# bibendovsky/oalsfxpp

Hardware: AMD Instinct MI355X
Metric: Msamples/sec EAX reverb, 256-frame buffers, batch=4096; % HBM roofline (higher is better)
Workload: dtype f32

## Files before the change

### include/oalsfx_hip.h

```cpp
#ifndef OALSFX_HIP_H
#define OALSFX_HIP_H

#include "oalsfx_desc.h"

#ifdef __cplusplus
extern "C" {
#endif

typedef struct oalsfx_batch oalsfx_batch;

typedef struct {
    int32_t type;
    unsigned char props[108];
} oalsfx_effect;

typedef struct { float gain, gain_hf, gain_lf; } oalsfx_send_props;

oalsfx_batch* oalsfx_batch_create(int n_instances, int channel_format, int sampling_rate, int effect_count, int device_id);
void oalsfx_batch_destroy(oalsfx_batch* b);
const char* oalsfx_batch_error(const oalsfx_batch* b);
const char* oalsfx_last_error(void);

int oalsfx_batch_instances(const oalsfx_batch* b);
int oalsfx_batch_channels(const oalsfx_batch* b);
int oalsfx_batch_sampling_rate(const oalsfx_batch* b);
int oalsfx_batch_effect_count(const oalsfx_batch* b);

int oalsfx_batch_set_effect(oalsfx_batch* b, int first, int count, int slot, const oalsfx_effect* effects, int stride_bytes);
int oalsfx_batch_set_effect_at(oalsfx_batch* b, const int* instances, int count, int slot, const oalsfx_effect* effects, int stride_bytes);
int oalsfx_batch_set_effect_type(oalsfx_batch* b, int first, int count, int slot, int effect_type);
int oalsfx_batch_set_effect_props(oalsfx_batch* b, int first, int count, int slot, const void* props, int stride_bytes);
int oalsfx_batch_set_send_props(oalsfx_batch* b, int first, int count, int slot, const oalsfx_send_props* props);
int oalsfx_batch_get_effect(const oalsfx_batch* b, int instance, int slot, int deferred, oalsfx_effect* out);
int oalsfx_batch_get_send_props(const oalsfx_batch* b, int instance, int slot, int deferred, oalsfx_send_props* out);
int oalsfx_batch_apply_changes(oalsfx_batch* b, int first, int count);

int oalsfx_batch_mix(oalsfx_batch* b, int frames, const float* src_host, float* dst_host);
int oalsfx_batch_mix_gather(oalsfx_batch* b, int frames, const float* const* src_per_instance, float* const* dst_per_instance);
int oalsfx_batch_mix_device(oalsfx_batch* b, int frames, const float* src_dev, float* dst_dev, void* hip_stream);
int oalsfx_batch_mix_device_multi(oalsfx_batch* b, int frames, int buffers, const float* const* src_dev, float* const* dst_dev, void* hip_stream);
int oalsfx_batch_synchronize(oalsfx_batch* b);
long long oalsfx_batch_chained_calls(const oalsfx_batch* b);
int oalsfx_batch_mix_async(oalsfx_batch* b, int frames, const float* src_host, float* dst_host);
int oalsfx_batch_wait(oalsfx_batch* b);
void* oalsfx_pinned_alloc(unsigned long long bytes);
void oalsfx_pinned_free(void* p);
void* oalsfx_batch_stream(oalsfx_batch* b);

typedef struct oalsfx_group oalsfx_group;
oalsfx_group* oalsfx_group_create(int n_total, const int* device_ids, int n_devices, int channel_format, int sampling_rate, int effect_count);
void oalsfx_group_destroy(oalsfx_group* g);
const char* oalsfx_group_error(const oalsfx_group* g);
const char* oalsfx_group_last_error(void);
int oalsfx_group_instances(const oalsfx_group* g);
int oalsfx_group_channels(const oalsfx_group* g);
int oalsfx_group_devices(const oalsfx_group* g);
int oalsfx_group_shard(const oalsfx_group* g, int k, int* device_id, int* first, int* count);
oalsfx_batch* oalsfx_group_batch(oalsfx_group* g, int k);
int oalsfx_group_set_effect(oalsfx_group* g, int first, int count, int slot, const oalsfx_effect* effects, int stride_bytes);
int oalsfx_group_set_effect_type(oalsfx_group* g, int first, int count, int slot, int effect_type);
int oalsfx_group_set_effect_props(oalsfx_group* g, int first, int count, int slot, const void* props, int stride_bytes);
int oalsfx_group_set_send_props(oalsfx_group* g, int first, int count, int slot, const oalsfx_send_props* props);
int oalsfx_group_apply_changes(oalsfx_group* g, int first, int count);
int oalsfx_group_mix(oalsfx_group* g, int frames, const float* src_host, float* dst_host);
int oalsfx_group_mix_device(oalsfx_group* g, int frames, const float* const* src_per_device, float* const* dst_per_device);
int oalsfx_group_mix_device_multi(oalsfx_group* g, int frames, int buffers, const float* const* src_dev, float* const* dst_dev);
int oalsfx_group_synchronize(oalsfx_group* g);
int oalsfx_group_set_routing(oalsfx_group* g, int first, int count, const int* bus, const float* gain);
int oalsfx_group_mix_downmix(oalsfx_group* g, int frames, const float* src_host, int n_buses, float* dst_bus_host);

unsigned long long oalsfx_trim_pools(void);
unsigned long long oalsfx_pools_waiting_bytes(void);

int oalsfx_batch_read_slot(oalsfx_batch* b, int instance, int slot, oalsfx_slot_params* params, oalsfx_slot_state* state);
int oalsfx_batch_read_ring(oalsfx_batch* b, int instance, int slot, float* out, int max_floats);
int oalsfx_batch_read_source(oalsfx_batch* b, int instance, oalsfx_source_params* params, oalsfx_source_state* state);

unsigned long long oalsfx_batch_snapshot_bytes(oalsfx_batch* b, const int* instances, int count);
int oalsfx_batch_snapshot(oalsfx_batch* b, const int* instances, int count, void* dst, unsigned long long bytes);
int oalsfx_batch_restore(oalsfx_batch* b, const int* instances, int count, const void* src, unsigned long long bytes);
int oalsfx_batch_reset(oalsfx_batch* b, const int* instances, int count);

#define OALSFX_DOWNMIX_CHUNK 32
int oalsfx_batch_set_routing(oalsfx_batch* b, int first, int count, const int* bus, const float* gain);
int oalsfx_batch_get_routing(const oalsfx_batch* b, int instance, int* bus, float* gain);
int oalsfx_batch_downmix_device(oalsfx_batch* b, int frames, const float* src_dev, int n_buses, float* dst_bus_dev, void* hip_stream);
int oalsfx_batch_mix_downmix(oalsfx_batch* b, int frames, const float* src_host, int n_buses, float* dst_bus_host);

#define OALSFX_METER_LANES 64
#define OALSFX_METER_CARRY 1
typedef struct {
    float    peak[OALSFX_MAX_CHANNELS];
    float    sumsq[OALSFX_MAX_CHANNELS];
    float    peak_hold;
    uint32_t quiet_run;
    uint32_t nonfinite;
    uint32_t frames;
} oalsfx_meter;
int oalsfx_batch_meter_device(oalsfx_batch* b, int rows, int frames, const float* src_dev, float threshold, int flags,
                              oalsfx_meter* meters_dev, void* hip_stream);
int oalsfx_batch_mix_downmix_meter(oalsfx_batch* b, int frames, const float* src_host, int n_buses, float* dst_bus_host,
                                   float threshold, int flags, oalsfx_meter* voice_meters_host, oalsfx_meter* bus_meters_host);
int oalsfx_group_mix_downmix_meter(oalsfx_group* g, int frames, const float* src_host, int n_buses, float* dst_bus_host,
                                   float threshold, int flags, oalsfx_meter* voice_meters_host);

#define OALSFX_SAMPLER_FRAC_BITS 12
#define OALSFX_PCM_U8  0
#define OALSFX_PCM_S16 1
#define OALSFX_PCM_F32 2
#define OALSFX_SAMPLER_PLAYING 1
#define OALSFX_SAMPLER_LOOP    2
#define OALSFX_SAMPLER_LINEAR  4
typedef struct {
    uint64_t data;
    uint64_t position;
    uint32_t frames;
    uint32_t loop_start;
    uint32_t loop_end;
    uint32_t step;
    uint32_t format;
    uint32_t channels;
    uint32_t flags;
// ... 32 lines not shown
```

### include/oalsfx_hip_debug.h

```cpp
#ifndef OALSFX_HIP_DEBUG_H
#define OALSFX_HIP_DEBUG_H

#include "oalsfx_hip.h"

#ifdef __cplusplus
extern "C" {
#endif

int oalsfx_batch_mix_timed(oalsfx_batch* b, int frames, const float* src_host, float* dst_host, double legs_us[3]);
long long oalsfx_debug_chain_same_cu(oalsfx_batch* b);
int oalsfx_batch_fill_synthetic(oalsfx_batch* b, int frames, unsigned buffer_index, float* dst_dev, void* hip_stream);

int oalsfx_batch_kernel_timing(oalsfx_batch* b, int enable);
int oalsfx_batch_kernel_timing_read(oalsfx_batch* b, int effect_type, int* launches, double* total_ms);
int oalsfx_batch_kernel_timing_samples(oalsfx_batch* b, int effect_type, double* out_us, int max_samples);
int oalsfx_batch_placement(const oalsfx_batch* b, int* chunks, int* candidates, double* best_us, double* worst_us);
int oalsfx_batch_event_overhead(oalsfx_batch* b, int repeats, double* avg_us);

int oalsfx_debug_hbm_sweep(int device_id, unsigned long long bytes, int write, int repeats);
void oalsfx_debug_set_flags(int flags);
unsigned long long oalsfx_debug_ring_address(oalsfx_batch* b, int instance, int slot);
int oalsfx_debug_move_rings(oalsfx_batch* b, int keep_old);
int oalsfx_debug_probe_rings(oalsfx_batch* b, int repeats, double* avg_us);
int oalsfx_debug_probe_pointer(void* slabs, int instances, int slab_floats, int repeats, double* avg_us);
int oalsfx_debug_stream_pattern(int device_id, int instances, int dwords_per_lane, int repeats, int slab_floats, int pos_skew, double* avg_us);

int oalsfx_debug_host_pipeline(oalsfx_batch* b, int* form, double* probe_us_three_streams, double* probe_us_one_stream);

void oalsfx_debug_gate_skew(oalsfx_batch* b, unsigned skew);
int oalsfx_debug_chain_given_up(const oalsfx_batch* b);
int oalsfx_debug_chain_started(oalsfx_batch* b, unsigned* host_total, unsigned* device_total);
int oalsfx_batch_multi_counts(const oalsfx_batch* b, long long* buffers_in_passes, long long* passes);

long long oalsfx_debug_downmix_uploads(const oalsfx_batch* b);
void oalsfx_debug_downmix_vector(int max_floats);

long long oalsfx_debug_sampler_uploads(const oalsfx_batch* b);

#ifdef __cplusplus
}
#endif

#endif
```

### oalsfxpp_amd/api.py

```python
import ctypes as C
import operator
import weakref

import numpy as np

from . import desc, lib

_fp = C.POINTER(C.c_float)
DOWNMIX_CHUNK = 32
METER_LANES = 64
METER_CARRY = 1
METER_DTYPE = np.dtype([("peak", np.float32, (desc.MAX_CHANNELS,)), ("sumsq", np.float32, (desc.MAX_CHANNELS,)), ("peak_hold", np.float32),
                        ("quiet_run", np.uint32), ("nonfinite", np.uint32), ("frames", np.uint32)])
assert METER_DTYPE.itemsize == C.sizeof(desc.Meter) == 80
SAMPLER_DTYPE = np.dtype([("data", np.uint64), ("position", np.uint64), ("frames", np.uint32), ("loop_start", np.uint32), ("loop_end", np.uint32),
                          ("step", np.uint32), ("format", np.uint32), ("channels", np.uint32), ("flags", np.uint32), ("reserved", np.uint32),
                          ("gain", np.float32, (desc.MAX_CHANNELS,))])
assert SAMPLER_DTYPE.itemsize == C.sizeof(desc.Sampler) == 80
SAMPLER_FRAC_BITS = desc.SAMPLER_FRAC_BITS
_PCM_BYTES = {desc.PCM_U8: 1, desc.PCM_S16: 2, desc.PCM_F32: 4}


class BatchError(RuntimeError):
    pass
# ... 48 lines not shown
    def _range(self, first, count):
        return first, (self.n - first if count is None else count)

    def set_effect(self, slot, effect, first=0, count=None):
        first, count = self._range(first, count)
        if isinstance(effect, desc.Effect):
            self._check(self._lib.oalsfx_batch_set_effect(self._h, first, count, slot, C.byref(effect), 0))
        else:
            arr = (desc.Effect * count)(*effect)
            self._check(self._lib.oalsfx_batch_set_effect(self._h, first, count, slot, arr, C.sizeof(desc.Effect)))

    def set_effect_at(self, slot, instances, effects):
        idx = (C.c_int * len(instances))(*instances)
        if isinstance(effects, desc.Effect):
            self._check(self._lib.oalsfx_batch_set_effect_at(self._h, idx, len(instances), slot, C.byref(effects), 0))
        else:
            arr = (desc.Effect * len(instances))(*effects)
            self._check(self._lib.oalsfx_batch_set_effect_at(self._h, idx, len(instances), slot, arr, C.sizeof(desc.Effect)))

    def set_effect_type(self, slot, effect_type, first=0, count=None):
        first, count = self._range(first, count)
        self._check(self._lib.oalsfx_batch_set_effect_type(self._h, first, count, slot, effect_type))

    def set_effect_props(self, slot, props, first=0, count=None):
        first, count = self._range(first, count)
        if isinstance(props, desc.EffectPropsU):
            self._check(self._lib.oalsfx_batch_set_effect_props(self._h, first, count, slot, C.byref(props), 0))
        else:
            arr = (desc.EffectPropsU * count)(*props)
            self._check(self._lib.oalsfx_batch_set_effect_props(self._h, first, count, slot, arr, C.sizeof(desc.EffectPropsU)))

    def set_send_props(self, slot, gain, gain_hf, gain_lf, first=0, count=None):
        first, count = self._range(first, count)
        p = desc.SendProps(gain, gain_hf, gain_lf)
        self._check(self._lib.oalsfx_batch_set_send_props(self._h, first, count, slot, C.byref(p)))

    def get_effect(self, instance, slot, deferred=False):
        e = desc.Effect()
        self._check(self._lib.oalsfx_batch_get_effect(self._h, instance, slot, 1 if deferred else 0, C.byref(e)))
        return e

    def get_send_props(self, instance, slot, deferred=False):
        p = desc.SendProps()
        self._check(self._lib.oalsfx_batch_get_send_props(self._h, instance, slot, 1 if deferred else 0, C.byref(p)))
        return p

    def apply_changes(self, first=0, count=None):
        first, count = self._range(first, count)
        self._check(self._lib.oalsfx_batch_apply_changes(self._h, first, count))

    def mix(self, src):
        src = np.ascontiguousarray(src, dtype=np.float32)
        assert src.ndim == 3 and src.shape[0] == self.n and src.shape[2] == self.channels, src.shape
        dst = np.empty_like(src)
        self._check(self._lib.oalsfx_batch_mix(self._h, src.shape[1], src.ctypes.data_as(_fp), dst.ctypes.data_as(_fp)))
        return dst

    def mix_async(self, src, dst):
        assert src.dtype == np.float32 and dst.dtype == np.float32 and src.flags.c_contiguous and dst.flags.c_contiguous and src.shape == dst.shape
        assert src.ndim == 3 and src.shape[0] == self.n and src.shape[2] == self.channels, src.shape
        self._check(self._lib.oalsfx_batch_mix_async(self._h, src.shape[1], src.ctypes.data_as(_fp), dst.ctypes.data_as(_fp)))

    def wait(self):
        self._check(self._lib.oalsfx_batch_wait(self._h))

    def pinned_array(self, frames):
        count = self.n * frames * self.channels
        p = self._lib.oalsfx_pinned_alloc(count * 4)
        if not p:
            raise BatchError("oalsfx_pinned_alloc failed")
        buf = (C.c_float * count).from_address(p)
        weakref.finalize(buf, self._lib.oalsfx_pinned_free, C.c_void_p(p))
        return np.frombuffer(buf, dtype=np.float32).reshape(self.n, frames, self.channels)

    def mix_device(self, frames, src_ptr, dst_ptr, stream=None):
        self._check(self._lib.oalsfx_batch_mix_device(self._h, frames, C.c_void_p(src_ptr), C.c_void_p(dst_ptr), C.c_void_p(stream or 0)))

    def mix_device_multi(self, frames, src_ptrs, dst_ptrs, stream=None):
        if len(src_ptrs) != len(dst_ptrs):
            raise BatchError("mix_device_multi: as many source as destination buffers")
        s = (C.c_void_p * max(1, len(src_ptrs)))(*src_ptrs)
        d = (C.c_void_p * max(1, len(dst_ptrs)))(*dst_ptrs)
        self._check(self._lib.oalsfx_batch_mix_device_multi(self._h, frames, len(src_ptrs), s, d, C.c_void_p(stream or 0)))

    def multi_counts(self):
        k, p = C.c_longlong(0), C.c_longlong(0)
        self._check(self._lib.oalsfx_batch_multi_counts(self._h, C.byref(k), C.byref(p)))
        return k.value, p.value

    def synchronize(self):
        self._check(self._lib.oalsfx_batch_synchronize(self._h))

    @property
    def stream(self):
        return self._lib.oalsfx_batch_stream(self._h)

    def fill_synthetic(self, frames, buffer_index, dst_ptr, stream=None):
        self._check(self._lib.oalsfx_batch_fill_synthetic(self._h, frames, buffer_index, C.c_void_p(dst_ptr), C.c_void_p(stream or 0)))

    def read_slot(self, instance, slot):
        p, s = desc.SlotParams(), desc.SlotState()
        self._check(self._lib.oalsfx_batch_read_slot(self._h, instance, slot, C.byref(p), C.byref(s)))
        return p, s

    def read_ring(self, instance, slot):
        n = self._lib.oalsfx_batch_read_ring(self._h, instance, slot, None, 0)
        out = np.zeros(n, dtype=np.float32)
        if n:
            self._lib.oalsfx_batch_read_ring(self._h, instance, slot, out.ctypes.data_as(_fp), n)
        return out

    def read_source(self, instance):
        p, s = desc.SourceParams(), desc.SourceState()
        self._check(self._lib.oalsfx_batch_read_source(self._h, instance, C.byref(p), C.byref(s)))
        return p, s

    def _instances(self, instances):
        if instances is None:
            return None, self.n
        try:
            idx = [operator.index(i) for i in instances]
        except TypeError:
            raise BatchError("Instances must be a sequence of integers.") from None
        bad = [i for i in idx if i < 0 or i >= self.n]
        if bad:
            raise BatchError(f"Instance range is out of bounds: {bad[:4]}")
        return (C.c_int * max(1, len(idx)))(*idx), len(idx)

    @staticmethod
    def _blob(ptr, nbytes):
        if not ptr:
            raise BatchError("No snapshot buffer.")
        if ptr % 16:
            raise BatchError("The snapshot buffer is not 16-byte aligned.")
        if operator.index(nbytes) < 0:
            raise BatchError("Snapshot bytes are negative.")

    def snapshot_bytes(self, instances=None):
        idx, count = self._instances(instances)
        nbytes = self._lib.oalsfx_batch_snapshot_bytes(self._h, idx, count)
        self._check(nbytes != 0)
        return nbytes

    def snapshot(self, instances, dst_ptr, nbytes):
        idx, count = self._instances(instances)
        self._blob(dst_ptr, nbytes)
        self._check(self._lib.oalsfx_batch_snapshot(self._h, idx, count, C.c_void_p(dst_ptr), nbytes))

    def restore(self, instances, src_ptr, nbytes):
        idx, count = self._instances(instances)
        if instances is not None and len(set(idx[:count])) != count:
            raise BatchError("An instance is listed twice as a restore target.")
        self._blob(src_ptr, nbytes)
        self._check(self._lib.oalsfx_batch_restore(self._h, idx, count, C.c_void_p(src_ptr), nbytes))

    def reset(self, instances=None):
        idx, count = self._instances(instances)
        self._check(self._lib.oalsfx_batch_reset(self._h, idx, count))

    @staticmethod
    def _routing(n, first, bus, gain):
        if bus is None and gain is None:
            raise BatchError("set_routing: give buses, gains or both.")
        try:
            buses = None if bus is None else [operator.index(v) for v in bus]
            gains = None if gain is None else [float(v) for v in gain]
# ... 428 lines not shown
```

### oalsfxpp_amd/csrc/hip/batch.cpp

```cpp
#include <hip/hip_runtime.h>

#include <algorithm>
#include <atomic>
#include <cstdio>
#include <chrono>
#include <cmath>
#include <cstdlib>
#include <cstring>
#include <map>
#include <mutex>
#include <new>
#include <string>
#include <type_traits>
#include <vector>

#include "../host/core.hpp"
#include "common.hpp"
#include "oalsfx_hip.h"
#include "state_io.hpp"
#include "downmix.hpp"
#include "meter.hpp"
#include "sampler.hpp"
#include "oalsfx_hip_debug.h"

// ... 75 lines not shown
    int* d_progress = nullptr;
    unsigned* d_hot = nullptr;
    unsigned* d_inst_epoch = nullptr;
    unsigned* d_exact = nullptr;
    unsigned* h_exact = nullptr;
    char fault_text[400] = {};
    long long host_prepare_ns = 0, host_stage_wait_ns = 0, host_derive_ns = 0, host_lists_ns = 0;
    unsigned* h_fault = nullptr;
    unsigned* d_fault = nullptr;
    bool chain_given_up = false;
    uint32_t gate_skew = 0;
    hipEvent_t ev_exact = nullptr;
    char* h_state_io = nullptr;
    char* d_state_io = nullptr;
    size_t state_io_capacity = 0;
    hipEvent_t ev_state_io = nullptr;
    bool state_io_pending = false;
    bool state_io_unordered = false;
    int list_offset[OALSFX_MAX_SLOTS][OALSFX_TYPE_COUNT] = {};
    int list_count[OALSFX_MAX_SLOTS][OALSFX_TYPE_COUNT] = {};
    int steady_offset[OALSFX_MAX_SLOTS] = {};
    int fast_count[OALSFX_MAX_SLOTS] = {};
    int kind_count[OALSFX_MAX_SLOTS][3] = {};
    int rest_tiles[OALSFX_MAX_SLOTS] = {};
    int fast_first[OALSFX_MAX_SLOTS] = {};
    int slow_count[OALSFX_MAX_SLOTS] = {};
    int general_offset[OALSFX_MAX_SLOTS] = {};
    int general_count[OALSFX_MAX_SLOTS] = {};
    std::map<size_t, RingPool> pools;
    std::vector<void*> chunks;
    struct RingChunk { char* base; size_t bytes; void* alloc; };
    std::vector<RingChunk> ring_chunks;
    int placed_chunks = 0, placement_candidates = 0;
    double placement_best_us = 0.0, placement_worst_us = 0.0;

    float* d_io_src = nullptr;
    float* d_io_dst = nullptr;
    size_t io_capacity = 0;
    float* h_io_src = nullptr;
    float* h_io_dst = nullptr;
    size_t h_io_capacity = 0;
    static constexpr int kPipeDepth = 3;
    struct PipeSlot { float* d_src = nullptr; float* d_dst = nullptr; hipEvent_t copied_in = nullptr, mixed = nullptr, copied_out = nullptr; bool busy = false; };
    PipeSlot pipe[kPipeDepth];
    size_t pipe_capacity = 0;
    long long pipe_turn = 0;
    hipStream_t h2d_stream = nullptr, d2h_stream = nullptr;
    int pipe_mode = 0;
    std::chrono::steady_clock::time_point pipe_probe_t0;
    double pipe_probe_us[2] = {0.0, 0.0};

    unsigned long long* d_timeline = nullptr;
    struct Stage { char* host = nullptr; char* dev = nullptr; size_t capacity = 0; hipEvent_t done = nullptr; bool pending = false; };
    Stage stage[4];
    int stage_turn = 0;
    hipEvent_t ev_uploaded = nullptr;
    hipEvent_t ev_mixed = nullptr;
    hipStream_t last_launch_stream = nullptr;
    const char* last_steady_kernel = "";

    hipStream_t stream = nullptr;
    hipStream_t chain_stream[kChainDepth] = {};
    hipEvent_t ev_chain[kChainDepth] = {};
    int chain_pos = 0;
    int chain_pos_last = -1, chain_pos_before = -1;
    bool chain_used[kChainDepth] = {};
    hipEvent_t ev_chain_start = nullptr;
    unsigned* d_turn = nullptr;
    uint32_t turn_counter = 0;
    uint32_t started_total = 0;
    int launched_groups = 0;
    uint32_t frames_total = 0;
    std::vector<uint32_t> started_at;
    bool off_grid_known = false;
    int off_grid[OALSFX_MAX_SLOTS] = {};
    bool poisoned = false;
    int chain_len = 0;
    std::vector<std::pair<const char*, const char*>> chain_dsts;
    bool uncached = false;
    bool chain_open = false;
    bool stream_handed_out = false;
    long long chained_calls = 0;
    long long multi_buffers = 0, multi_passes = 0;
    std::vector<int> route_bus;
    std::vector<float> route_gain;
    bool routing_dirty = true;
    int route_max = -1;
    int dm_buses = 0;
    oalsfx_hip::DownmixTable dm_table;
    oalsfx_hip::DownmixDevice dm_dev;
    char* h_dm_table = nullptr;
    char* d_dm_table = nullptr;
    size_t dm_table_capacity = 0;
    float* d_dm_partials = nullptr;
    size_t dm_partials_capacity = 0;
    float* d_dm_out = nullptr;
    size_t dm_out_capacity = 0;
    hipEvent_t ev_downmix = nullptr;
    hipEvent_t ev_dm_order = nullptr;
    hipStream_t dm_stream = nullptr;
    bool dm_pending = false;
    long long dm_uploads = 0;
    oalsfx_meter* d_meters = nullptr;
    size_t meters_capacity = 0;
    std::vector<oalsfx_sampler> h_samplers;
    std::vector<uint8_t> sampler_dirty;
    std::vector<int> sampler_dirty_list;
    bool samplers_ahead = false;
    oalsfx_sampler* d_samplers = nullptr;
    char* h_sampler_stage = nullptr;
    size_t sampler_stage_capacity = 0;
    hipEvent_t ev_sampler_staged = nullptr;
    bool sampler_stage_pending = false;
    hipEvent_t ev_sampler = nullptr;
    hipStream_t sampler_stream = nullptr;
    bool sampler_pending = false;
    long long sampler_uploads = 0;
    hipStream_t side_stream[kSideStreams] = {};
    hipEvent_t ev_fork = nullptr;
    hipEvent_t ev_join[kSideStreams] = {};
    const char* error = "";
    std::string error_store;

    bool timing = false;
    int timing_every = 0;
    long long mix_calls = 0;
    std::vector<TimedLaunch> timed;
    std::vector<hipEvent_t> event_pool;

    hipEvent_t take_event()
    {
        hipEvent_t e = nullptr;
        if (!event_pool.empty()) { e = event_pool.back(); event_pool.pop_back(); }
        else hipEventCreate(&e);
        return e;
    }
    bool fail(const char* msg) { error = msg; return false; }
    bool hip_ok(hipError_t e, const char* what)
    {
        if (e == hipSuccess) return true;
        error_store = std::string(what) + ": " + hipGetErrorString(e);
        error = error_store.c_str();
        return false;
    }
};

namespace {

constexpr const char* kErrRange = "Instance range is out of bounds.";
constexpr const char* kErrSlot = "Effect index is out of range.";
constexpr const char* kErrNoSrc = "No source samples.";
constexpr const char* kErrNoDst = "No destination samples.";

bool range_ok(oalsfx_batch* b, int first, int count)
{
    if (first < 0 || count < 0 || first + count > b->n) return b->fail(kErrRange);
    return true;
}

void mark_touched(oalsfx_batch* b, int first, int count)
{
    for (int i = first; i < first + count; ++i)
        if (!b->touched[i]) {
            b->touched[i] = 1;
            b->touched_list.push_back(i);
        }
}

void mark_dirty(oalsfx_batch* b, int i)
{
    if (!b->inst_dirty[i]) {
        b->inst_dirty[i] = 1;
        b->dirty_list.push_back(i);
    }
}

void release_slab(oalsfx_batch* b, size_t idx)
{
    if (b->h_rings[idx]) {
        b->pools[b->ring_floats[idx]].free_dirty.push_back(b->h_rings[idx]);
        b->h_rings[idx] = nullptr;
        b->ring_floats[idx] = 0;
    }
}

enum DebugFlag : int {
    kDbgAcquireAlways = 0x1,
    kDbgAcquireNever = 0x2,
    kDbgReadEarly = 0x4,
    kDbgGeneralOnly = 0x8,
    kDbgTapRound128 = 0x20,
    kDbgTapRound256 = 0x40,
    kDbgChainLight = 0x80,
    kDbgNoCuMajor = 0x100,
    kDbgNoChain = 0x400,
    kDbgGateSecondOnly = 0x800,
    kDbgChainAlways = 0x8000,
    kDbgForceProven = 0x2000000,
    kDbgHandOverBits = kDbgAcquireAlways | kDbgAcquireNever | kDbgReadEarly,
    kDbgKernelBits = 0xFF,
};
int debug_flags();

constexpr int kSettleFrames = OALSFX_RV_FADE_SAMPLES;

enum : uint8_t {
    kClassReverb = 1,
    kClassSteady = 2,
    kClassClose = 4,
    kClassShort = 8,
    kClassModulated = 16,
};

uint8_t classify_slot(const oalsfx_slot_params& sp)
{
    if (sp.type != OALSFX_REVERB && sp.type != OALSFX_EAX_REVERB) return 0;
    const oalsfx_reverb_params& p = sp.u.reverb;
    uint8_t cls = kClassReverb | kClassSteady;
    const int sway = p.mod_depth != 0.0F ? 1 + static_cast<int>(std::abs(p.mod_depth)) : 0;
    int lo = 1 << 30, lo_ahead = 1 << 30;
    for (int j = 0; j < 4; ++j) {
        if (p.early_tap[j] < 0 || p.early_ap_off[j] < 4 || p.early_line_off[j] < 0 || p.late_ap_off[j] < 4 ||
            p.late_line_off[j] < 64 + sway || p.late_tap[j] < p.late_feed_tap)
            cls &= static_cast<uint8_t>(~kClassSteady);
        lo = std::min({lo, p.early_tap[j], p.early_ap_off[j], p.early_line_off[j], p.late_tap[j] - p.late_feed_tap, p.late_ap_off[j], p.late_line_off[j]});
        lo_ahead = std::min({lo_ahead, p.early_tap[j], p.late_line_off[j]});
    }
    if (lo >= 64 && (lo < static_cast<int>(oalsfx_hip::kPlainMinTap) || lo_ahead < static_cast<int>(oalsfx_hip::kPlainMinTapAhead))) cls |= kClassClose;
    if (lo < 64) cls |= kClassShort;
    if (p.mod_depth != 0.0F) cls |= kClassModulated;
    return cls;
}

bool reverb_settled(const oalsfx_batch* b, size_t idx)
{
    return (b->slot_class[idx] & kClassSteady) != 0 && (b->since_update[idx] >= kSettleFrames || b->xf_ok[idx]);
}

bool crossfade_followable(const oalsfx_reverb_params& from, const oalsfx_reverb_params& to)
{
    const int sway = (from.mod_depth != 0.0F || to.mod_depth != 0.0F) ? 1 + static_cast<int>(std::max(std::abs(from.mod_depth), std::abs(to.mod_depth))) : 0;
    for (const oalsfx_reverb_params* p : {&from, &to})
        for (int j = 0; j < 4; ++j)
            if (p->early_tap[j] < 0 || p->early_ap_off[j] < 4 || p->early_line_off[j] < 0 || p->late_tap[j] < to.late_feed_tap ||
                p->late_ap_off[j] < 4 || p->late_line_off[j] < 64 + sway)
                return false;
    return true;
}

bool slot_in_transition(const oalsfx_batch* b, int slot)
{
    for (size_t idx : b->settling)
        if (static_cast<int>(idx % b->slots) == slot && b->xf_ok[idx]) return true;
    return false;
}

void reclassify_slot(oalsfx_batch* b, size_t idx, int slot)
{
    const uint8_t before = b->slot_class[idx], after = classify_slot(b->h_params[idx]);
    b->n_close[slot] += ((after & kClassClose) != 0) - ((before & kClassClose) != 0);
    b->n_short[slot] += ((after & kClassShort) != 0) - ((before & kClassShort) != 0);
    if (after & kClassModulated) b->modulated[slot] = true;
    b->slot_class[idx] = after;
}

void advance_settling(oalsfx_batch* b, int frames)
{
    size_t keep = 0;
    for (size_t k = 0; k < b->settling.size(); ++k) {
        const size_t idx = b->settling[k];
        b->since_update[idx] = std::min(b->since_update[idx] + frames, kSettleFrames);
        if (b->since_update[idx] < kSettleFrames) { b->settling[keep++] = idx; continue; }
        b->in_settling[idx] = 0;
        b->xf_ok[idx] = 0;
        if (b->slot_class[idx] & kClassSteady) { b->lists_dirty = true; b->exact_wanted = true; }
    }
    b->settling.resize(keep);
}

class UncachedPool {
public:
    static constexpr size_t kGranule = size_t(2) << 20;
// ... 868 lines not shown
            const char* lo = reinterpret_cast<const char*>(dsts[k]);
            bool known = false;
            for (const auto& d : b->chain_dsts) known |= d.first <= lo && lo < d.second;
            if (!known) return false;
        }
        const char* lo = reinterpret_cast<const char*>(srcs[k]);
        const char* hi = lo + buffer_bytes;
        if (b->chain_open)
            for (const auto& d : b->chain_dsts)
                if (lo < d.second && d.first < hi) return false;
    }
    if (stream != b->stream || b->stream_handed_out || (debug_flags() & (kDbgNoChain | kDbgGeneralOnly)) || b->timing_every > 0 || b->d_timeline) return false;
    if (!b->uncached) return false;
    for (const auto& kv : b->pools)
        if (kv.first % 32 != 0) return false;
    if (frames > OALSFX_MAX_CHUNK) return false;
    if (b->channels > 2) {
        const int last_block = frames - ((frames - 1) / OALSFX_RV_MAX_UPDATE) * OALSFX_RV_MAX_UPDATE;
        return b->slots == 1 && !uploading && (frames & 63) == 0 && b->n_filtered == 0 && b->general_count[0] == 0 && b->slow_count[0] == 0 &&
               b->fast_count[0] == b->n && last_block / 64 >= b->rest_tiles[0];
    }
    if (b->slots > 1) {
        const int last = b->slots - 1, run = reverb_free_run(b, 0);
        if (uploading || (frames & 63) != 0 || b->n_filtered > 0 || run < last) return false;
        if ((b->n + 3) / 4 < 1024 && !(debug_flags() & kDbgChainAlways)) return false;
        if (run == b->slots) return (debug_flags() & kDbgChainLight) != 0;
        if (b->fast_count[last] + b->slow_count[last] != b->n || b->general_count[last] != 0) return false;
        KernelCtx ctx{};
        ctx.frames = frames;
        const SlotPlan pl = plan_slot(b, ctx, last, frames, true);
        return pl.by_kind && !pl.mixed && pl.steady == b->n;
    }
    if ((b->n + 3) / 4 < 1024 && frames < 256 && !(debug_flags() & kDbgChainAlways)) return false;
    const int steady = b->fast_count[0] + b->slow_count[0];
    if (b->general_count[0] != 0) return false;
    if (steady != b->n) {
        if (uploading || (frames & 63) != 0 || b->n_filtered > 0) return false;
        KernelCtx ctx{};
        ctx.frames = frames;
        const SlotPlan pl = plan_slot(b, ctx, 0, frames, true);
        if (pl.light + pl.steady != b->n || pl.reverbs != pl.steady) return false;
        if (pl.steady == 0) return (debug_flags() & kDbgChainLight) != 0;
        if ((b->n + 3) / 4 <= 1024 && !(debug_flags() & kDbgChainAlways)) return false;
        return pl.mixed && mixed_grid_proven(b, 0, frames);
    }
    if ((frames & 63) != 0) {
        KernelCtx ctx{};
        ctx.frames = frames;
        if (!plan_slot(b, ctx, 0, frames, true).ragged_proven || b->n_filtered > 0) return false;
    }
    if (b->n_filtered > 0) {
        KernelCtx ctx{};
        ctx.frames = frames;
        const SlotPlan p0 = plan_slot(b, ctx, 0, frames, true);
        if (!p0.by_kind || p0.steady != b->n) return false;
        int counts[4];
        steady_kind_counts(b, 0, p0.proven_usable, counts);
        if (filters_inside_count(b, 0, counts) != b->n_filtered) return false;
    }
    return true;
}

bool chain_next_launch(oalsfx_batch* b, KernelCtx& ctx, int depth, PendingUpload* upload, hipStream_t* stream_out)
{
    b->chain_pos_before = b->chain_open ? b->chain_pos_last : -1;
    b->chain_pos_last = b->chain_open ? b->chain_pos : -1;
    b->chain_pos = b->chain_open ? (b->chain_pos + 1) % depth : 0;
    hipStream_t stream = b->chain_stream[b->chain_pos];
    const bool first_on_its_stream = b->chain_open && !b->chain_used[b->chain_pos];
    b->chain_used[b->chain_pos] = true;
    const size_t total = static_cast<size_t>(b->n) * b->slots;
    ctx.turn = b->d_turn;
    ctx.turn_cu = b->d_turn + total + 16;
    ctx.turn_cu2 = ctx.turn_cu + total;
    ctx.turn_slot = b->slots - 1;
    ctx.turn_two_back = (b->chain_pos_before >= 0 && b->chain_pos_before != b->chain_pos) ? 1u : 0u;
    ctx.turn_wait = b->chain_open ? b->turn_counter : 0u;
    if (++b->turn_counter == 0u) b->turn_counter = 1u;
    ctx.turn_set = b->turn_counter;
    unsigned* started = b->d_turn + total;
    if (!b->chain_open) {
        if (!b->hip_ok(hipEventRecord(b->ev_chain_start, b->stream), "hipEventRecord")) return false;
        b->chain_len = 1;
    } else {
        ++b->chain_len;
        if (first_on_its_stream && !b->hip_ok(hipStreamWaitEvent(stream, b->ev_chain_start, 0), "hipStreamWaitEvent")) return false;
        if (b->chain_len == 2 || !(debug_flags() & kDbgGateSecondOnly)) {
            const unsigned target = b->started_total - static_cast<uint32_t>(std::min(8, (b->n + 3) / 4 - 1));
            if (upload && upload->st) { upload->jobs.gate_started = started; upload->jobs.gate_target = target + b->gate_skew; }
            else oalsfx_hip::launch_chain_gate(started, target + b->gate_skew, b->d_fault + 1, stream);
        }
    }
    ctx.turn_started = started;
    b->chain_open = true;
    b->launched_groups = 0;
    *stream_out = stream;
    return true;
}

bool chain_launch_done(oalsfx_batch* b)
{
    if (b->launched_groups <= 0) return b->fail("Internal error: a chained call launched no grid that takes turns.");
    b->started_total += static_cast<uint32_t>(b->launched_groups);
    b->launched_groups = 0;
    return true;
}

bool pass_usable(oalsfx_batch* b, int frames, int total)
{
    if (total > OALSFX_MAX_CHUNK || frames > total) return false;
    if (b->slots != 1 || b->channels > 2 || (frames & 63) != 0 || b->n_filtered > 0 || b->d_timeline) return false;
    if (b->fast_count[0] != b->n || b->slow_count[0] != 0 || b->general_count[0] != 0) return false;
    for (const int n : {frames, total}) {
        KernelCtx ctx{};
        ctx.frames = n;
        const SlotPlan p = plan_slot(b, ctx, 0, n, true);
        if (!p.by_kind || p.mixed || p.steady != b->n || !p.proven_usable) return false;
    }
    return true;
}

bool buffers_apart(const oalsfx_batch* b, int frames, int buffers, const float* const* srcs, float* const* dsts)
{
    if (buffers < 2) return true;
    const uintptr_t bytes = static_cast<uintptr_t>(b->n) * frames * b->channels * sizeof(float);
    struct Range { uintptr_t lo; int call; bool out; };
    std::vector<Range> r;
    r.reserve(2 * static_cast<size_t>(buffers));
    for (int k = 0; k < buffers; ++k) {
        r.push_back({reinterpret_cast<uintptr_t>(srcs[k]), k, false});
        r.push_back({reinterpret_cast<uintptr_t>(dsts[k]), k, true});
    }
    std::sort(r.begin(), r.end(), [](const Range& x, const Range& y) { return x.lo < y.lo || (x.lo == y.lo && x.call < y.call); });
    const Range* last[2][2] = {};
    for (const Range& x : r) {
        for (int kind = 0; kind < 2; ++kind) {
            if (!x.out && kind == 0) continue;
            for (const Range* y : last[kind])
                if (y && y->call != x.call && y->lo + bytes > x.lo) return false;
        }
        const int kind = x.out ? 1 : 0;
        last[kind][1] = last[kind][0];
        last[kind][0] = &x;
    }
    return true;
}

bool mix_pass(oalsfx_batch* b, int frames, int buffers, const float* const* srcs, float* const* dsts, hipStream_t stream, bool may_chain,
              PendingUpload& upload, bool pass)
{
    const float* const src = srcs[0];
    float* const dst = dsts[0];
    const int total = frames * buffers;
    if (pass && total > OALSFX_MAX_CHUNK) return b->fail("Internal error: a multi-buffer pass longer than one chunk.");
    const bool chained = may_chain && (!upload.st || upload.chainable) && chain_eligible(b, total, buffers, srcs, dsts, stream, upload.st != nullptr);
    if (!chained && !chain_join(b)) return false;
    int depth = 2;
    if (chained) {
        const int rs = b->slots - 1;
        int populated = 0;
        for (int k = 0; k < 3; ++k) populated += b->kind_count[rs][k] > 0;
        depth = (populated > 1 || b->slow_count[rs] > 0 || upload.st) ? kChainDepth : 2;
    }
    if (!chained && !launch_params(b, upload, b->stream, stream)) return false;
    if (!ensure_mixbuf(b)) return false;
    b->timing = b->timing_every > 0 && (b->mix_calls % b->timing_every == 0 || b->mix_calls % b->timing_every + buffers > b->timing_every);
    b->mix_calls += buffers;
    const bool filtered = b->n_filtered > 0;
    const int chunk_max = std::min(total, OALSFX_MAX_CHUNK);
    const size_t plane = static_cast<size_t>(b->n) * chunk_max * b->channels;
    if (filtered && plane > b->filtered_capacity) {
        if (!b->hip_ok(hipStreamSynchronize(stream), "hipStreamSynchronize")) return false;
        for (int k = 1; k < kChainDepth && b->chain_open; ++k)
            if (!b->hip_ok(hipStreamSynchronize(b->chain_stream[k]), "hipStreamSynchronize")) return false;
        hipFree(b->d_filtered);
        b->d_filtered = nullptr;
        b->filtered_capacity = 0;
        if (!b->hip_ok(hipMalloc(reinterpret_cast<void**>(&b->d_filtered), plane * (1 + b->slots) * sizeof(float)), "hipMalloc(filtered sends)")) return false;
        b->filtered_capacity = plane;
    }
    KernelCtx ctx{};
    ctx.params = b->d_params;
    ctx.state = b->d_state;
    ctx.rings = b->d_rings;
    ctx.source = b->d_source;
    ctx.source_state = b->d_source_state;
    ctx.mixbuf = b->d_mixbuf;
    ctx.timeline = b->d_timeline;
    ctx.hot = b->d_hot;
    ctx.inst_epoch = b->d_inst_epoch;
    ctx.exact = b->d_exact;
    ctx.fault = b->d_fault;
    ctx.list_first = -1;
    ctx.no_follow_up = 0;
    if (chained) {
        if (!b->chain_open) b->chain_dsts.clear();
        for (int k = 0; k < buffers; ++k) {
            const char* lo = reinterpret_cast<const char*>(dsts[k]);
            const char* hi = lo + static_cast<size_t>(b->n) * frames * b->channels * sizeof(float);
            bool known = false;
            for (auto& d : b->chain_dsts) known |= d.first <= lo && hi <= d.second;
            if (!known) b->chain_dsts.push_back({lo, hi});
        }
        if (!chain_next_launch(b, ctx, depth, &upload, &stream)) return false;
        if (!launch_params(b, upload, stream, nullptr, b->d_turn, ctx.turn_wait)) return false;
        b->chained_calls += 1;
    }
    ctx.slots = b->slots;
    ctx.channels = b->channels;
    ctx.io_stride = static_cast<long long>(frames) * b->channels;
    struct EqualPlaces {
        bool on;
        explicit EqualPlaces(bool o) : on(o) { if (on) oalsfx_hip::set_lds_per_workgroup(40960); }
        ~EqualPlaces() { if (on) oalsfx_hip::set_lds_per_workgroup(0); }
    } equal_places(chained && b->slots > 1);
    oalsfx_hip::BufferTable table{};
    if (pass) {
        for (int k = 0; k < buffers; ++k) { table.src[k] = srcs[k]; table.dst[k] = dsts[k]; }
        table.frames = frames;
        table.buffers = buffers;
    }
    for (int done = 0; done < total;) {
        const int n = std::min(total - done, OALSFX_MAX_CHUNK);
        const float* chunk_src = src + static_cast<size_t>(done) * b->channels;
        ctx.raw_src = chunk_src;
        ctx.dst = dst + static_cast<size_t>(done) * b->channels;
        ctx.frames = n;
        bool planes = filtered;
        bool filters_inside = false;
        if (filtered && b->slots == 1) {
            const SlotPlan p0 = plan_slot(b, ctx, 0, n, true);
            if (p0.by_kind && p0.steady > 0) {
                int counts[4];
                steady_kind_counts(b, 0, p0.proven_usable, counts);
                const int inside = filters_inside_count(b, 0, counts);
                if (inside > 0) {
                    filters_inside = true;
                    ctx.src_stride = static_cast<long long>(n) * b->channels;
                    planes = inside < b->n_filtered;
                    if (planes) {
                        const int before = b->steady_offset[0], behind = before + counts[0] + counts[1];
                        oalsfx_hip::launch_send_filters(ctx, chunk_src, ctx.io_stride, b->d_filtered, b->filtered_capacity, b->d_lists, before, stream);
                        oalsfx_hip::launch_send_filters(ctx, chunk_src, ctx.io_stride, b->d_filtered, b->filtered_capacity, b->d_lists + behind, b->n - behind, stream);
                    }
                }
            }
        }
        if (filters_inside) {
            ctx.src = planes ? b->d_filtered : chunk_src;
            if (!planes) ctx.src_stride = ctx.io_stride;
        } else if (filtered) {
            ctx.src_stride = static_cast<long long>(n) * b->channels;
            oalsfx_hip::launch_send_filters(ctx, chunk_src, ctx.io_stride, b->d_filtered, b->filtered_capacity, nullptr, b->n, stream);
            ctx.src = b->d_filtered;
        } else {
            ctx.src_stride = ctx.io_stride;
            ctx.src = chunk_src;
        }
        ctx.wet_plane = planes ? static_cast<long long>(b->filtered_capacity) : 0;
        for (int s = 0; s < b->slots; ++s) {
            ctx.wet_src = planes ? b->d_filtered + static_cast<size_t>(1 + s) * b->filtered_capacity : ctx.src;
            const int run = reverb_free_run(b, s);
            if (run >= 2) {
                const int run_flags = (s == 0 ? oalsfx_hip::kFirst : 0) | (s + run == b->slots ? oalsfx_hip::kLast : 0) |
                                      (planes ? oalsfx_hip::kFiltered : 0);
                {
                    ScopedTiming timing(b, kTimedWaveEffects, stream);
                    const bool grid_order = chained && s + run < b->slots;
                    const int* every = grid_order ? b->d_lists + b->steady_offset[b->slots - 1] : b->d_lists + b->list_offset[s][OALSFX_NULL];
                    oalsfx_hip::launch_wave_effects(ctx, s, run, every, b->n, nullptr,
                                                    run_flags | (chained ? ((debug_flags() & kDbgHandOverBits) | (grid_order ? 0 : 8)) << 8 : 0), stream);
                }
                if (chained) b->launched_groups = (b->n + 3) / 4;
                s += run - 1;
                continue;
            }
            if (chained && s > 0 && (!chain_launch_done(b) || !chain_next_launch(b, ctx, depth, nullptr, &stream))) return false;
            const int flags = (s == 0 ? oalsfx_hip::kFirst : 0) | (s == b->slots - 1 ? oalsfx_hip::kLast : 0) |
                              (planes ? oalsfx_hip::kFiltered : 0);
            const bool null_has_duty = (flags & (oalsfx_hip::kFirst | oalsfx_hip::kLast)) != 0;
            const SlotPlan sp = plan_slot(b, ctx, s, n, null_has_duty);
            const int light = sp.light, steady = sp.steady, reverbs = sp.reverbs;
            const bool use_steady = sp.use_steady, mixed = sp.mixed, by_kind = sp.by_kind, proven_usable = sp.proven_usable;
            bool part_on[4] = {light > 0 && !mixed, false, steady > 0, reverbs - steady > 0};
            int parts = 0;
            for (bool on : part_on) parts += on;
            const bool fork = parts > 1;
            if (fork && !b->hip_ok(hipEventRecord(b->ev_fork, stream), "hipEventRecord")) return false;
            int main_part = -1;
            for (int g = 0; g < 4; ++g)
                if (part_on[g]) main_part = (main_part < 0 || g == 3) ? g : main_part;
            int side = 0;
            for (int g = 0; g < 4; ++g) {
                if (!part_on[g]) continue;
                hipStream_t gs = stream;
                if (fork && g != main_part) {
                    gs = b->side_stream[side];
                    if (!b->hip_ok(hipStreamWaitEvent(gs, b->ev_fork, 0), "hipStreamWaitEvent")) return false;
                }
                if (g == 0) {
                    launch_wave_group(b, ctx, s, flags, gs);
                } else if (g == 2 && mixed) {
                    launch_mixed_part(b, ctx, s, flags, gs);
                } else if (g == 2 && pass) {
                    launch_reverb_pass_part(b, ctx, s, flags, table, gs);
                } else if (g == 2 && by_kind) {
                    launch_reverb_kinds_part(b, ctx, s, flags, proven_usable, filters_inside, gs);
                } else if (g == 2) {
                    launch_reverb_steady_part(b, ctx, s, flags, b->steady_offset[s], steady, sp.ragged_proven, gs);
                } else {
                    launch_reverb_general_part(b, !use_steady, ctx, s, flags, gs);
                }
                if (gs != stream) {
                    if (!b->hip_ok(hipEventRecord(b->ev_join[side], gs), "hipEventRecord")) return false;
                    ++side;
                }
            }
            for (int k = 0; k < side; ++k)
                if (!b->hip_ok(hipStreamWaitEvent(stream, b->ev_join[k], 0), "hipStreamWaitEvent")) return false;
        }
        done += n;
    }
    if (chained && !chain_launch_done(b)) return false;
    if (pass) { b->multi_buffers += buffers; b->multi_passes += 1; }
    if ((total % OALSFX_MAX_CHUNK) & 63) {
        for (size_t idx : b->settling)
            if (b->xf_ok[idx]) { b->xf_ok[idx] = 0; b->lists_dirty = true; }
    }
    advance_settling(b, total);
    b->frames_total += static_cast<uint32_t>(total);
    if (total & 31) b->off_grid_known = false;
    if (b->exact_wanted && !b->exact_pending) {
        const size_t total = static_cast<size_t>(b->n) * b->slots;
        if (!b->hip_ok(hipMemcpyAsync(b->h_exact, b->d_exact, total * sizeof(unsigned), hipMemcpyDeviceToHost, stream), "hipMemcpyAsync(exact)")) return false;
        if (!b->hip_ok(hipEventRecord(b->ev_exact, stream), "hipEventRecord")) return false;
        b->exact_pending = true;
        b->exact_wanted = false;
        b->exact_gen = b->upload_gen;
    }
    b->last_launch_stream = chained ? b->stream : stream;
    if (!chained && stream != b->stream && !b->hip_ok(hipEventRecord(b->ev_mixed, stream), "hipEventRecord")) return false;
    return b->hip_ok(hipGetLastError(), "kernel launch");
}

bool mix_device(oalsfx_batch* b, int frames, int buffers, const float* const* srcs, float* const* dsts, hipStream_t stream, bool may_chain,
                bool multi)
{
    if (b->state_io_unordered && stream != b->stream) {
        if (!b->hip_ok(hipStreamWaitEvent(stream, b->ev_state_io, 0), "hipStreamWaitEvent")) return false;
        b->state_io_unordered = false;
    }
    const int per_pass = std::max(1, OALSFX_MAX_CHUNK / std::max(frames, 1));
    const bool apart = multi && buffers_apart(b, frames, buffers, srcs, dsts);
    for (int k = 0; k < buffers;) {
        if (b->poisoned) return b->fail(b->fault_text);
        poll_exact(b);
        b->launched_groups = 0;
        PendingUpload upload;
        const auto hp0 = std::chrono::steady_clock::now();
        if (!prepare_params(b, upload)) return false;
        b->host_prepare_ns += std::chrono::duration_cast<std::chrono::nanoseconds>(std::chrono::steady_clock::now() - hp0).count();
        const int take = std::min(buffers - k, per_pass);
        const bool pass = apart && !(debug_flags() & kDbgGeneralOnly) && pass_usable(b, frames, take * frames);
        const int step = pass ? take : 1;
        if (!mix_pass(b, frames, step, srcs + k, dsts + k, stream, may_chain, upload, pass)) return false;
        k += step;
    }
    return true;
}

bool mix_device(oalsfx_batch* b, int frames, const float* src, float* dst, hipStream_t stream, bool may_chain = false)
{
    float* out = dst;
    return mix_device(b, frames, 1, &src, &out, stream, may_chain, false);
}

}

extern "C" {

const char* oalsfx_last_error(void) { return g_last_error.c_str(); }

oalsfx_batch* oalsfx_batch_create(int n_instances, int channel_format, int sampling_rate, int effect_count, int device_id)
{
    g_last_error.clear();
    const int channels = channel_count_of(static_cast<oalsfxpp::ChannelFormat>(channel_format));
    if (channels == 0) { g_last_error = "Invalid channel format."; return nullptr; }
    if (sampling_rate < min_sampling_rate) { g_last_error = "Sampling rate is out of range."; return nullptr; }
    if (effect_count <= 0 || effect_count > OALSFX_MAX_SLOTS) { g_last_error = "Effect count is out of range."; return nullptr; }
    if (n_instances <= 0) { g_last_error = "Instance count is out of range."; return nullptr; }

    int device_count = 0;
    if (hipGetDeviceCount(&device_count) != hipSuccess || device_count <= 0) {
        g_last_error = "No HIP device available: the effect process path has no CPU fallback.";
        return nullptr;
    }
    if (device_id < 0 || device_id >= device_count) { g_last_error = "HIP device ordinal is out of range."; return nullptr; }
    if (hipSetDevice(device_id) != hipSuccess) { g_last_error = "hipSetDevice failed."; return nullptr; }

    auto* b = new (std::nothrow) oalsfx_batch{};
    if (!b) { g_last_error = "Failed to allocate the batch."; return nullptr; }
    b->n = n_instances;
    b->slots = effect_count;
    b->channels = channels;
    b->rate = sampling_rate;
    b->format = channel_format;
    b->device = device_id;
    b->dev.init(static_cast<oalsfxpp::ChannelFormat>(channel_format), sampling_rate);
    b->channels = b->dev.channels;
    const size_t total = static_cast<size_t>(n_instances) * effect_count;
    b->inst.resize(n_instances);
    b->h_params.assign(total, oalsfx_slot_params{});
    b->h_state_init.assign(total, oalsfx_slot_state{});
    b->started_at.assign(total, 0);
    b->h_source.assign(n_instances, oalsfx_source_params{});
    b->seq.assign(total, 0);
    b->h_rings.assign(total, nullptr);
    b->ring_floats.assign(total, 0);
    b->inst_dirty.assign(n_instances, 0);
    b->inst_filtered.assign(n_instances, 0);
    b->touched.assign(n_instances, 0);
    b->aux_written.assign(n_instances, 0);
    b->route_bus.assign(n_instances, 0);
    b->route_gain.assign(n_instances, 1.0F);
    b->h_samplers.assign(n_instances, oalsfx_sampler{});
    b->sampler_dirty.assign(n_instances, 0);
    b->since_update.assign(total, 0);
    b->slot_class.assign(total, 0);
    b->in_settling.assign(total, 0);
    b->xf_ok.assign(total, 0);
    b->mod_ever.assign(total, 0);
    b->proven.assign(total, 0);
    b->updated_gen.assign(total, 0);
    b->inst_epoch.assign(n_instances, 1);
    for (int i = 0; i < n_instances; ++i) {
        b->inst[i].initialize(effect_count);
        mark_dirty(b, i);
    }
    mark_touched(b, 0, n_instances);

    bool ok = b->hip_ok(hipStreamCreateWithFlags(&b->stream, hipStreamNonBlocking), "hipStreamCreate");
    b->chain_stream[0] = b->stream;
    for (int k = 1; k < kChainDepth; ++k) {
        ok = ok && b->hip_ok(hipStreamCreateWithFlags(&b->chain_stream[k], hipStreamNonBlocking), "hipStreamCreate");
        ok = ok && b->hip_ok(hipEventCreateWithFlags(&b->ev_chain[k], hipEventDisableTiming), "hipEventCreate");
    }
    {
        const char* kind = std::getenv("OALSFX_RING_MEMORY");
        b->uncached = (!kind || std::strcmp(kind, "uncached") == 0) && uncached_memory_available(b->device);
    }
    ok = ok && b->hip_ok(hipEventCreateWithFlags(&b->ev_chain_start, hipEventDisableTiming), "hipEventCreate");
    for (int k = 0; k < kSideStreams; ++k) {
        ok = ok && b->hip_ok(hipStreamCreateWithFlags(&b->side_stream[k], hipStreamNonBlocking), "hipStreamCreate");
        ok = ok && b->hip_ok(hipEventCreateWithFlags(&b->ev_join[k], hipEventDisableTiming), "hipEventCreate");
    }
    ok = ok && b->hip_ok(hipEventCreateWithFlags(&b->ev_fork, hipEventDisableTiming), "hipEventCreate");
    ok = ok && b->hip_ok(hipEventCreateWithFlags(&b->ev_uploaded, hipEventDisableTiming), "hipEventCreate");
    ok = ok && b->hip_ok(hipEventCreateWithFlags(&b->ev_mixed, hipEventDisableTiming), "hipEventCreate");
    ok = ok && b->hip_ok(hipEventCreateWithFlags(&b->ev_downmix, hipEventDisableTiming), "hipEventCreate");
    ok = ok && b->hip_ok(hipEventCreateWithFlags(&b->ev_dm_order, hipEventDisableTiming), "hipEventCreate");
    ok = ok && b->hip_ok(hipEventCreateWithFlags(&b->ev_sampler, hipEventDisableTiming), "hipEventCreate");
    ok = ok && b->hip_ok(hipEventCreateWithFlags(&b->ev_sampler_staged, hipEventDisableTiming), "hipEventCreate");
    ok = ok && b->hip_ok(hipMalloc(reinterpret_cast<void**>(&b->d_samplers), n_instances * sizeof(oalsfx_sampler)), "hipMalloc(samplers)");
    ok = ok && b->hip_ok(hipMemsetAsync(b->d_samplers, 0, n_instances * sizeof(oalsfx_sampler), b->stream), "hipMemsetAsync(samplers)");
    ok = ok && b->hip_ok(hipMalloc(reinterpret_cast<void**>(&b->d_params), total * sizeof(oalsfx_slot_params)), "hipMalloc(params)");
    ok = ok && b->hip_ok(handed_on_malloc(b, reinterpret_cast<void**>(&b->d_state), total * sizeof(oalsfx_hip::SlotStateLines)), "hipMalloc(state)");
    ok = ok && b->hip_ok(hipMalloc(reinterpret_cast<void**>(&b->d_source), n_instances * sizeof(oalsfx_source_params)), "hipMalloc(source)");
    ok = ok && b->hip_ok(hipMalloc(reinterpret_cast<void**>(&b->d_rings), total * sizeof(float*)), "hipMalloc(ring table)");
    ok = ok && b->hip_ok(handed_on_malloc(b, reinterpret_cast<void**>(&b->d_source_state), n_instances * sizeof(oalsfx_source_state)), "hipMalloc(source state)");
    ok = ok && b->hip_ok(hipMalloc(reinterpret_cast<void**>(&b->d_lists_buf[0]), (kChainDepth + 1) * total * sizeof(int)), "hipMalloc(lists)");
    if (ok) {
        for (int k = 1; k <= kChainDepth; ++k) b->d_lists_buf[k] = b->d_lists_buf[0] + k * total;
        b->d_lists = b->d_lists_buf[0];
    }
    ok = ok && b->hip_ok(hipMalloc(reinterpret_cast<void**>(&b->d_progress), total * sizeof(int)), "hipMalloc(progress)");
    ok = ok && b->hip_ok(hipMemsetAsync(b->d_progress, 0, total * sizeof(int), b->stream), "hipMemsetAsync(progress)");
    ok = ok && b->hip_ok(handed_on_malloc(b, reinterpret_cast<void**>(&b->d_hot), total * oalsfx_hip::hot::SIZE * sizeof(unsigned)), "hipMalloc(hot records)");
    ok = ok && b->hip_ok(hipMemsetAsync(b->d_hot, 0, total * oalsfx_hip::hot::SIZE * sizeof(unsigned), b->stream), "hipMemsetAsync(hot records)");
    ok = ok && b->hip_ok(hipMalloc(reinterpret_cast<void**>(&b->d_inst_epoch), n_instances * sizeof(unsigned)), "hipMalloc(epochs)");
    ok = ok && b->hip_ok(hipMemsetAsync(b->d_inst_epoch, 0, n_instances * sizeof(unsigned), b->stream), "hipMemsetAsync(epochs)");
    ok = ok && b->hip_ok(handed_on_malloc(b, reinterpret_cast<void**>(&b->d_turn), (3 * total + 16) * sizeof(unsigned)), "hipMalloc(turns)");
    ok = ok && b->hip_ok(hipMemsetAsync(b->d_turn, 0, (3 * total + 16) * sizeof(unsigned), b->stream), "hipMemsetAsync(turns)");
    ok = ok && b->hip_ok(handed_on_malloc(b, reinterpret_cast<void**>(&b->d_exact), total * sizeof(unsigned)), "hipMalloc(exact)");
    ok = ok && b->hip_ok(hipMemsetAsync(b->d_exact, 0, total * sizeof(unsigned), b->stream), "hipMemsetAsync(exact)");
    ok = ok && b->hip_ok(hipHostMalloc(reinterpret_cast<void**>(&b->h_exact), total * sizeof(unsigned)), "hipHostMalloc(exact)");
    ok = ok && b->hip_ok(hipHostMalloc(reinterpret_cast<void**>(&b->h_fault), 2 * sizeof(unsigned), hipHostMallocMapped), "hipHostMalloc(fault)");
    if (ok) b->h_fault[0] = b->h_fault[1] = 0;
    ok = ok && b->hip_ok(hipHostGetDevicePointer(reinterpret_cast<void**>(&b->d_fault), b->h_fault, 0), "hipHostGetDevicePointer");
    ok = ok && b->hip_ok(hipEventCreateWithFlags(&b->ev_exact, hipEventDisableTiming), "hipEventCreate");
    ok = ok && b->hip_ok(hipEventCreateWithFlags(&b->ev_state_io, hipEventDisableTiming), "hipEventCreate");
    ok = ok && b->hip_ok(hipMemsetAsync(b->d_state, 0, total * sizeof(oalsfx_hip::SlotStateLines), b->stream), "hipMemsetAsync(state)");
    ok = ok && b->hip_ok(hipMemsetAsync(b->d_source_state, 0, n_instances * sizeof(oalsfx_source_state), b->stream), "hipMemsetAsync(source state)");
    if (ok && std::getenv("OALSFX_DEBUG_TIMELINE")) {
        ok = b->hip_ok(hipMalloc(reinterpret_cast<void**>(&b->d_timeline), kTimelineBytes), "hipMalloc(timeline)");
        ok = ok && b->hip_ok(hipMemsetAsync(b->d_timeline, 0, kTimelineBytes, b->stream), "hipMemsetAsync(timeline)");
    }
    if (!ok) {
        g_last_error = b->error;
        oalsfx_batch_destroy(b);
        return nullptr;
    }
    return b;
}

void oalsfx_batch_destroy(oalsfx_batch* b)
{
    if (!b) return;
    hipSetDevice(b->device);
    for (int k = 1; k < kChainDepth; ++k)
        if (b->chain_stream[k]) hipStreamSynchronize(b->chain_stream[k]);
    if (b->stream) hipStreamSynchronize(b->stream);
    for (int k = 0; k < kSideStreams; ++k)
        if (b->side_stream[k]) hipStreamSynchronize(b->side_stream[k]);
    if (b->exact_pending) hipEventSynchronize(b->ev_exact);
    if (b->d_timeline) {
        std::vector<unsigned long long> h(kTimelineBytes / sizeof(unsigned long long));
        if (hipMemcpy(h.data(), b->d_timeline, kTimelineBytes, hipMemcpyDeviceToHost) == hipSuccess)
            if (FILE* f = std::fopen(std::getenv("OALSFX_DEBUG_TIMELINE"), "wb")) { std::fwrite(h.data(), 1, kTimelineBytes, f); std::fclose(f); }
        hipFree(b->d_timeline);
    }
    for (auto& t : b->timed) { hipEventDestroy(t.start); hipEventDestroy(t.stop); }
    for (hipEvent_t e : b->event_pool) hipEventDestroy(e);
    if (std::getenv("OALSFX_HOST_PROFILE"))
        std::fprintf(stderr, "host profile: prepare_params %.1f ms (of which waiting for a staging buffer %.1f ms), %lld mix_device calls chained\n",
                     b->host_prepare_ns * 1e-6, b->host_stage_wait_ns * 1e-6, b->chained_calls);
    for (void* c : b->chunks) handed_on_free(c);
    hipFree(b->d_params); handed_on_free(b->d_state); hipFree(b->d_source); hipFree(b->d_rings); handed_on_free(b->d_source_state); hipFree(b->d_filtered);
    handed_on_free(b->d_mixbuf); hipFree(b->d_lists_buf[0]); hipFree(b->d_progress); hipFree(b->d_io_src); hipFree(b->d_io_dst);
    handed_on_free(b->d_hot); hipFree(b->d_inst_epoch); handed_on_free(b->d_exact); handed_on_free(b->d_turn);
    for (int k = 1; k < kChainDepth; ++k)
        if (b->ev_chain[k]) hipEventDestroy(b->ev_chain[k]);
    if (b->ev_chain_start) hipEventDestroy(b->ev_chain_start);
    for (int k = 1; k < kChainDepth; ++k)
        if (b->chain_stream[k]) hipStreamDestroy(b->chain_stream[k]);
    if (b->h2d_stream) hipStreamSynchronize(b->h2d_stream);
    if (b->d2h_stream) hipStreamSynchronize(b->d2h_stream);
    for (auto& ps : b->pipe) {
        hipFree(ps.d_src); hipFree(ps.d_dst);
        if (ps.copied_in) hipEventDestroy(ps.copied_in);
        if (ps.mixed) hipEventDestroy(ps.mixed);
        if (ps.copied_out) hipEventDestroy(ps.copied_out);
    }
    if (b->h2d_stream) hipStreamDestroy(b->h2d_stream);
    if (b->d2h_stream) hipStreamDestroy(b->d2h_stream);
    if (b->h_io_src) (void)hipHostFree(b->h_io_src);
    if (b->h_io_dst) (void)hipHostFree(b->h_io_dst);
    if (b->h_exact) (void)hipHostFree(b->h_exact);
    if (b->h_fault) (void)hipHostFree(b->h_fault);
    if (b->ev_exact) hipEventDestroy(b->ev_exact);
    if (b->h_state_io) (void)hipHostFree(b->h_state_io);
    hipFree(b->d_state_io);
    if (b->ev_state_io) hipEventDestroy(b->ev_state_io);
    if (b->dm_pending) hipEventSynchronize(b->ev_downmix);
    if (b->h_dm_table) (void)hipHostFree(b->h_dm_table);
    hipFree(b->d_dm_table); hipFree(b->d_dm_partials); hipFree(b->d_dm_out);
    hipFree(b->d_meters);
    if (b->sampler_pending) hipEventSynchronize(b->ev_sampler);
    if (b->h_sampler_stage) (void)hipHostFree(b->h_sampler_stage);
    hipFree(b->d_samplers);
    if (b->ev_sampler) hipEventDestroy(b->ev_sampler);
    if (b->ev_sampler_staged) hipEventDestroy(b->ev_sampler_staged);
    if (b->ev_downmix) hipEventDestroy(b->ev_downmix);
    if (b->ev_dm_order) hipEventDestroy(b->ev_dm_order);
    for (int k = 0; k < kSideStreams; ++k) {
        if (b->side_stream[k]) hipStreamDestroy(b->side_stream[k]);
        if (b->ev_join[k]) hipEventDestroy(b->ev_join[k]);
    }
    if (b->ev_fork) hipEventDestroy(b->ev_fork);
    if (b->ev_uploaded) hipEventDestroy(b->ev_uploaded);
    if (b->ev_mixed) hipEventDestroy(b->ev_mixed);
    for (auto& st : b->stage) {
        if (st.host) (void)hipHostFree(st.host);
        if (st.dev) (void)hipFree(st.dev);
        if (st.done) hipEventDestroy(st.done);
    }
    if (b->stream) hipStreamDestroy(b->stream);
    delete b;
}

const char* oalsfx_batch_error(const oalsfx_batch* b) { return b ? b->error : g_last_error.c_str(); }
int oalsfx_batch_instances(const oalsfx_batch* b) { return b->n; }
int oalsfx_batch_channels(const oalsfx_batch* b) { return b->channels; }
int oalsfx_batch_sampling_rate(const oalsfx_batch* b) { return b->rate; }
int oalsfx_batch_effect_count(const oalsfx_batch* b) { return b->slots; }

int oalsfx_batch_set_effect(oalsfx_batch* b, int first, int count, int slot, const oalsfx_effect* effects, int stride_bytes)
{
    if (!range_ok(b, first, count)) return 0;
    if (slot < 0 || slot >= b->slots) return b->fail(kErrSlot) ? 1 : 0;
    const auto* base = reinterpret_cast<const unsigned char*>(effects);
    for (int i = 0; i < count; ++i)
        std::memcpy(&b->inst[first + i].deferred[slot], base + static_cast<size_t>(i) * stride_bytes, sizeof(oalsfx_effect));
    mark_touched(b, first, count);
    return 1;
}

int oalsfx_batch_set_effect_at(oalsfx_batch* b, const int* instances, int count, int slot, const oalsfx_effect* effects, int stride_bytes)
{
    if (count < 0 || (count > 0 && (!instances || !effects))) return b->fail(kErrRange) ? 1 : 0;
    if (slot < 0 || slot >= b->slots) return b->fail(kErrSlot) ? 1 : 0;
    for (int k = 0; k < count; ++k)
        if (instances[k] < 0 || instances[k] >= b->n) return b->fail(kErrRange) ? 1 : 0;
    const auto* base = reinterpret_cast<const unsigned char*>(effects);
    for (int k = 0; k < count; ++k) {
        std::memcpy(&b->inst[instances[k]].deferred[slot], base + static_cast<size_t>(k) * stride_bytes, sizeof(oalsfx_effect));
        mark_touched(b, instances[k], 1);
    }
    return 1;
}

int oalsfx_batch_set_effect_type(oalsfx_batch* b, int first, int count, int slot, int effect_type)
{
    if (!range_ok(b, first, count)) return 0;
    if (slot < 0 || slot >= b->slots) return b->fail(kErrSlot) ? 1 : 0;
    for (int i = 0; i < count; ++i) b->inst[first + i].deferred[slot].set_type_and_defaults(static_cast<oalsfxpp::EffectType>(effect_type));
    mark_touched(b, first, count);
    return 1;
}

int oalsfx_batch_set_effect_props(oalsfx_batch* b, int first, int count, int slot, const void* props, int stride_bytes)
{
    if (!range_ok(b, first, count)) return 0;
    if (slot < 0 || slot >= b->slots) return b->fail(kErrSlot) ? 1 : 0;
    const auto* base = static_cast<const unsigned char*>(props);
    for (int i = 0; i < count; ++i)
        std::memcpy(&b->inst[first + i].deferred[slot].props_, base + static_cast<size_t>(i) * stride_bytes, sizeof(oalsfxpp::EffectProps));
    mark_touched(b, first, count);
    return 1;
}

int oalsfx_batch_set_send_props(oalsfx_batch* b, int first, int count, int slot, const oalsfx_send_props* props)
{
    if (!range_ok(b, first, count)) return 0;
    if (slot >= b->slots) return b->fail(kErrSlot) ? 1 : 0;
    oalsfxpp::SendProps p;
    p.gain_ = props->gain; p.gain_hf_ = props->gain_hf; p.gain_lf_ = props->gain_lf;
    for (int i = 0; i < count; ++i) {
        InstanceHost& h = b->inst[first + i];
        if (slot < 0) h.direct_deferred = p;
        else { h.aux_props[slot] = p; b->aux_written[first + i] = 1; }
    }
    mark_touched(b, first, count);
    return 1;
}

int oalsfx_batch_get_effect(const oalsfx_batch* b, int instance, int slot, int deferred, oalsfx_effect* out)
{
    if (instance < 0 || instance >= b->n || slot < 0 || slot >= b->slots) return 0;
    const InstanceHost& h = b->inst[instance];
    std::memcpy(out, deferred ? &h.deferred[slot] : &h.active[slot], sizeof(oalsfx_effect));
    return 1;
}

int oalsfx_batch_get_send_props(const oalsfx_batch* b, int instance, int slot, int deferred, oalsfx_send_props* out)
{
    if (instance < 0 || instance >= b->n || slot >= b->slots) return 0;
    const InstanceHost& h = b->inst[instance];
    const oalsfxpp::SendProps& p = slot < 0 ? (deferred ? h.direct_deferred : h.direct_props) : (deferred ? h.aux_deferred[slot] : h.aux_props[slot]);
    out->gain = p.gain_; out->gain_hf = p.gain_hf_; out->gain_lf = p.gain_lf_;
    return 1;
}

int oalsfx_batch_apply_changes(oalsfx_batch* b, int first, int count)
{
    if (!range_ok(b, first, count)) return 0;
    size_t kept = 0;
    for (size_t k = 0; k < b->touched_list.size(); ++k) {
        const int i = b->touched_list[k];
        if (i < first || i >= first + count) { b->touched_list[kept++] = i; continue; }
        InstanceHost& h = b->inst[i];
        h.apply_changes();
        bool dirty = h.source_changed;
        for (int s = 0; s < b->slots; ++s) dirty |= h.slot_changed[s];
        if (dirty) mark_dirty(b, i);
        bool sticky = false;
        for (int s = 0; s < b->slots; ++s) sticky |= !oalsfxpp::SendProps::are_equal(h.aux_props[s], h.aux_deferred[s]);
        if (sticky) b->touched_list[kept++] = i;
        else b->touched[i] = 0;
    }
    b->touched_list.resize(kept);
    return 1;
}

int oalsfx_batch_mix_device(oalsfx_batch* b, int frames, const float* src_dev, float* dst_dev, void* hip_stream)
{
    if (frames == 0) return 1;
    if (frames < 0) return b->fail("Frame count is negative.") ? 1 : 0;
    if (!src_dev) return b->fail(kErrNoSrc) ? 1 : 0;
    if (!dst_dev) return b->fail(kErrNoDst) ? 1 : 0;
    if (!b->hip_ok(hipSetDevice(b->device), "hipSetDevice")) return 0;
    return mix_device(b, frames, src_dev, dst_dev, hip_stream ? static_cast<hipStream_t>(hip_stream) : b->stream, hip_stream == nullptr) ? 1 : 0;
}

int oalsfx_batch_mix_device_multi(oalsfx_batch* b, int frames, int buffers, const float* const* src_dev, float* const* dst_dev, void* hip_stream)
{
    if (!b) { g_last_error = "Null batch."; return 0; }
    if (frames < 0) return b->fail("Frame count is negative.") ? 1 : 0;
    if (buffers < 0) return b->fail("Buffer count is negative.") ? 1 : 0;
    if (frames == 0 || buffers == 0) return 1;
    if (!src_dev) return b->fail("Null source buffer table.") ? 1 : 0;
    if (!dst_dev) return b->fail("Null destination buffer table.") ? 1 : 0;
    for (int k = 0; k < buffers; ++k) {
        if (!src_dev[k]) return b->fail(kErrNoSrc) ? 1 : 0;
        if (!dst_dev[k]) return b->fail(kErrNoDst) ? 1 : 0;
    }
    if (!b->hip_ok(hipSetDevice(b->device), "hipSetDevice")) return 0;
    return mix_device(b, frames, buffers, src_dev, dst_dev, hip_stream ? static_cast<hipStream_t>(hip_stream) : b->stream, hip_stream == nullptr, true) ? 1 : 0;
}

namespace {

bool grow_io(oalsfx_batch* b, size_t floats)
{
    if (floats <= b->io_capacity) return true;
    hipFree(b->d_io_src); hipFree(b->d_io_dst);
    b->d_io_src = b->d_io_dst = nullptr;
    b->io_capacity = 0;
    if (!b->hip_ok(hipMalloc(reinterpret_cast<void**>(&b->d_io_src), floats * sizeof(float)), "hipMalloc(io)")) return false;
    if (!b->hip_ok(hipMalloc(reinterpret_cast<void**>(&b->d_io_dst), floats * sizeof(float)), "hipMalloc(io)")) return false;
    b->io_capacity = floats;
    return true;
}

int mix_host(oalsfx_batch* b, int frames, const float* src_host, float* dst_host, double* legs_us)
{
    if (legs_us) legs_us[0] = legs_us[1] = legs_us[2] = 0.0;
    if (frames == 0) return 1;
    if (frames < 0) return b->fail("Frame count is negative.") ? 1 : 0;
    if (!src_host) return b->fail(kErrNoSrc) ? 1 : 0;
    if (!dst_host) return b->fail(kErrNoDst) ? 1 : 0;
    if (!b->hip_ok(hipSetDevice(b->device), "hipSetDevice") || !chain_join(b)) return 0;
    const size_t floats = static_cast<size_t>(b->n) * frames * b->channels;
    if (!grow_io(b, floats)) return 0;
    hipEvent_t ev[4] = {};
    if (legs_us)
        for (auto& e : ev) e = b->take_event();
    if (legs_us) hipEventRecord(ev[0], b->stream);
    if (!b->hip_ok(hipMemcpyAsync(b->d_io_src, src_host, floats * sizeof(float), hipMemcpyHostToDevice, b->stream), "hipMemcpyAsync(src)")) return 0;
    if (legs_us) hipEventRecord(ev[1], b->stream);
    if (!mix_device(b, frames, b->d_io_src, b->d_io_dst, b->stream)) return 0;
    if (legs_us) hipEventRecord(ev[2], b->stream);
    if (!b->hip_ok(hipMemcpyAsync(dst_host, b->d_io_dst, floats * sizeof(float), hipMemcpyDeviceToHost, b->stream), "hipMemcpyAsync(dst)")) return 0;
    if (legs_us) hipEventRecord(ev[3], b->stream);
    if (!b->hip_ok(hipStreamSynchronize(b->stream), "hipStreamSynchronize")) return 0;
    if (legs_us) {
        for (int k = 0; k < 3; ++k) {
            float ms = 0.0F;
            if (hipEventElapsedTime(&ms, ev[k], ev[k + 1]) == hipSuccess) legs_us[k] = ms * 1e3;
        }
        for (auto& e : ev) b->event_pool.push_back(e);
    }
    poll_exact(b);
    return check_fault(b) ? 1 : 0;
}

}

int oalsfx_batch_mix(oalsfx_batch* b, int frames, const float* src_host, float* dst_host) { return mix_host(b, frames, src_host, dst_host, nullptr); }

int oalsfx_batch_mix_gather(oalsfx_batch* b, int frames, const float* const* src_per_instance, float* const* dst_per_instance)
{
    if (frames == 0) return 1;
    if (frames < 0) return b->fail("Frame count is negative.") ? 1 : 0;
    if (!src_per_instance) return b->fail(kErrNoSrc) ? 1 : 0;
    if (!dst_per_instance) return b->fail(kErrNoDst) ? 1 : 0;
    const size_t per = static_cast<size_t>(frames) * b->channels, floats = per * b->n;
    for (int i = 0; i < b->n; ++i) {
        if (!src_per_instance[i]) return b->fail(kErrNoSrc) ? 1 : 0;
        if (!dst_per_instance[i]) return b->fail(kErrNoDst) ? 1 : 0;
    }
    if (!b->hip_ok(hipSetDevice(b->device), "hipSetDevice")) return 0;
    if (floats > b->h_io_capacity) {
        if (b->h_io_src) (void)hipHostFree(b->h_io_src);
        if (b->h_io_dst) (void)hipHostFree(b->h_io_dst);
        b->h_io_src = b->h_io_dst = nullptr;
        b->h_io_capacity = 0;
        if (!b->hip_ok(hipHostMalloc(reinterpret_cast<void**>(&b->h_io_src), floats * sizeof(float), hipHostMallocDefault), "hipHostMalloc(io)")) return 0;
        if (!b->hip_ok(hipHostMalloc(reinterpret_cast<void**>(&b->h_io_dst), floats * sizeof(float), hipHostMallocDefault), "hipHostMalloc(io)")) return 0;
        b->h_io_capacity = floats;
    }
    for (int i = 0; i < b->n; ++i) std::memcpy(b->h_io_src + per * i, src_per_instance[i], per * sizeof(float));
    if (!mix_host(b, frames, b->h_io_src, b->h_io_dst, nullptr)) return 0;
    for (int i = 0; i < b->n; ++i) std::memcpy(dst_per_instance[i], b->h_io_dst + per * i, per * sizeof(float));
    return 1;
}

int oalsfx_batch_mix_timed(oalsfx_batch* b, int frames, const float* src_host, float* dst_host, double legs_us[3])
{
    return mix_host(b, frames, src_host, dst_host, legs_us);
}

namespace {

std::mutex g_pipe_mutex;
std::map<int, int> g_pipe_mode;

int pipe_form(oalsfx_batch* b)
{
    if (b->pipe_mode) return b->pipe_mode;
    if (const char* e = std::getenv("OALSFX_HOST_PIPELINE")) {
        const int m = std::atoi(e);
        if (m == 1 || m == 3) return b->pipe_mode = m;
    }
    {
        std::lock_guard<std::mutex> lock(g_pipe_mutex);
        auto it = g_pipe_mode.find(b->device);
        if (it != g_pipe_mode.end()) return b->pipe_mode = it->second;
    }
    const long long k = b->pipe_turn;
    const auto now = std::chrono::steady_clock::now();
    if ((k & 15) == 4) b->pipe_probe_t0 = now;
    if (k == 32 || k == 48) b->pipe_probe_us[k == 48 ? 0 : 1] = std::chrono::duration<double, std::micro>(now - b->pipe_probe_t0).count() / 12.0;
    if (k < 48) return (k >= 16 && k < 32) ? 1 : 3;
    b->pipe_mode = b->pipe_probe_us[1] < b->pipe_probe_us[0] * 0.9 ? 1 : 3;
    std::lock_guard<std::mutex> lock(g_pipe_mutex);
    g_pipe_mode[b->device] = b->pipe_mode;
    return b->pipe_mode;
}

}

int oalsfx_batch_mix_async(oalsfx_batch* b, int frames, const float* src_host, float* dst_host)
{
    if (frames == 0) return 1;
    if (frames < 0) return b->fail("Frame count is negative.") ? 1 : 0;
    if (!src_host) return b->fail(kErrNoSrc) ? 1 : 0;
    if (!dst_host) return b->fail(kErrNoDst) ? 1 : 0;
    if (!b->hip_ok(hipSetDevice(b->device), "hipSetDevice") || !chain_join(b)) return 0;
    const size_t floats = static_cast<size_t>(b->n) * frames * b->channels;
    if (!b->h2d_stream) {
        if (!b->hip_ok(hipStreamCreateWithFlags(&b->h2d_stream, hipStreamNonBlocking), "hipStreamCreate")) return 0;
        if (!b->hip_ok(hipStreamCreateWithFlags(&b->d2h_stream, hipStreamNonBlocking), "hipStreamCreate")) return 0;
        for (auto& ps : b->pipe) {
            if (!b->hip_ok(hipEventCreateWithFlags(&ps.copied_in, hipEventDisableTiming), "hipEventCreate")) return 0;
            if (!b->hip_ok(hipEventCreateWithFlags(&ps.mixed, hipEventDisableTiming), "hipEventCreate")) return 0;
            if (!b->hip_ok(hipEventCreateWithFlags(&ps.copied_out, hipEventDisableTiming), "hipEventCreate")) return 0;
        }
    }
    if (floats > b->pipe_capacity) {
        if (!b->hip_ok(hipStreamSynchronize(b->d2h_stream), "hipStreamSynchronize") || !b->hip_ok(hipStreamSynchronize(b->stream), "hipStreamSynchronize")) return 0;
        for (auto& ps : b->pipe) {
            hipFree(ps.d_src); hipFree(ps.d_dst);
            ps.d_src = ps.d_dst = nullptr;
            ps.busy = false;
        }
        b->pipe_capacity = 0;
        for (auto& ps : b->pipe) {
            if (!b->hip_ok(hipMalloc(reinterpret_cast<void**>(&ps.d_src), floats * sizeof(float)), "hipMalloc(io)")) return 0;
            if (!b->hip_ok(hipMalloc(reinterpret_cast<void**>(&ps.d_dst), floats * sizeof(float)), "hipMalloc(io)")) return 0;
        }
        b->pipe_capacity = floats;
    }
    const int form = pipe_form(b);
    oalsfx_batch::PipeSlot& ps = b->pipe[b->pipe_turn++ % oalsfx_batch::kPipeDepth];
    if (ps.busy && !b->hip_ok(hipEventSynchronize(ps.copied_out), "hipEventSynchronize")) return 0;
    ps.busy = true;
    if (form == 1) {
        if (!b->hip_ok(hipMemcpyAsync(ps.d_src, src_host, floats * sizeof(float), hipMemcpyHostToDevice, b->stream), "hipMemcpyAsync(src)")) return 0;
        if (!mix_device(b, frames, ps.d_src, ps.d_dst, b->stream)) return 0;
        if (!b->hip_ok(hipMemcpyAsync(dst_host, ps.d_dst, floats * sizeof(float), hipMemcpyDeviceToHost, b->stream), "hipMemcpyAsync(dst)")) return 0;
        return b->hip_ok(hipEventRecord(ps.copied_out, b->stream), "hipEventRecord") ? 1 : 0;
    }
    if (!b->hip_ok(hipMemcpyAsync(ps.d_src, src_host, floats * sizeof(float), hipMemcpyHostToDevice, b->h2d_stream), "hipMemcpyAsync(src)")) return 0;
    if (!b->hip_ok(hipEventRecord(ps.copied_in, b->h2d_stream), "hipEventRecord")) return 0;
    if (!b->hip_ok(hipStreamWaitEvent(b->stream, ps.copied_in, 0), "hipStreamWaitEvent")) return 0;
    if (!mix_device(b, frames, ps.d_src, ps.d_dst, b->stream)) return 0;
    if (!b->hip_ok(hipEventRecord(ps.mixed, b->stream), "hipEventRecord")) return 0;
    if (!b->hip_ok(hipStreamWaitEvent(b->d2h_stream, ps.mixed, 0), "hipStreamWaitEvent")) return 0;
    if (!b->hip_ok(hipMemcpyAsync(dst_host, ps.d_dst, floats * sizeof(float), hipMemcpyDeviceToHost, b->d2h_stream), "hipMemcpyAsync(dst)")) return 0;
    return b->hip_ok(hipEventRecord(ps.copied_out, b->d2h_stream), "hipEventRecord") ? 1 : 0;
}

int oalsfx_batch_wait(oalsfx_batch* b)
{
    if (!b->hip_ok(hipSetDevice(b->device), "hipSetDevice") || !chain_join(b)) return 0;
    if (b->d2h_stream && !b->hip_ok(hipStreamSynchronize(b->d2h_stream), "hipStreamSynchronize")) return 0;
    if (!b->hip_ok(hipStreamSynchronize(b->stream), "hipStreamSynchronize")) return 0;
    for (auto& ps : b->pipe) ps.busy = false;
    poll_exact(b);
    return check_fault(b) ? 1 : 0;
}

void* oalsfx_pinned_alloc(unsigned long long bytes)
{
    void* p = nullptr;
    return hipHostMalloc(&p, bytes, hipHostMallocDefault) == hipSuccess ? p : nullptr;
}

void oalsfx_pinned_free(void* p)
{
    if (p) (void)hipHostFree(p);
}

int oalsfx_batch_synchronize(oalsfx_batch* b)
{
    if (!b->hip_ok(hipSetDevice(b->device), "hipSetDevice") || !chain_join(b)) return 0;
    if (!b->hip_ok(hipStreamSynchronize(b->stream), "hipStreamSynchronize")) return 0;
    if (std::getenv("OALSFX_HOST_PROFILE")) {
        std::fprintf(stderr, "host profile since the last synchronize: prepare_params %.1f us, of which staging-buffer waits %.1f us, derive %.1f us, lists %.1f us; %lld calls chained so far\n",
                     b->host_prepare_ns * 1e-3, b->host_stage_wait_ns * 1e-3, b->host_derive_ns * 1e-3, b->host_lists_ns * 1e-3, b->chained_calls);
        b->host_prepare_ns = b->host_stage_wait_ns = b->host_derive_ns = b->host_lists_ns = 0;
    }
    poll_exact(b);
    return check_fault(b) ? 1 : 0;
}

void* oalsfx_batch_stream(oalsfx_batch* b)
{
    b->stream_handed_out = true;
    if (hipSetDevice(b->device) == hipSuccess) (void)chain_join(b);
    return b->stream;
}

int oalsfx_batch_read_slot(oalsfx_batch* b, int instance, int slot, oalsfx_slot_params* params, oalsfx_slot_state* state)
{
    if (instance < 0 || instance >= b->n || slot < 0 || slot >= b->slots) return b->fail(kErrRange) ? 1 : 0;
    if (!b->hip_ok(hipSetDevice(b->device), "hipSetDevice") || !chain_join(b)) return 0;
    if (!sync_params(b, nullptr)) return 0;
    const size_t idx = static_cast<size_t>(instance) * b->slots + slot;
    if (params) *params = b->h_params[idx];
    if (state) {
        if (!b->hip_ok(hipStreamSynchronize(b->stream), "hipStreamSynchronize")) return 0;
        if (!b->hip_ok(hipMemcpy(state, static_cast<const oalsfx_slot_state*>(b->d_state + idx), sizeof(*state), hipMemcpyDeviceToHost), "hipMemcpy(state)")) return 0;
    }
    return 1;
}

int oalsfx_batch_read_ring(oalsfx_batch* b, int instance, int slot, float* out, int max_floats)
{
    if (instance < 0 || instance >= b->n || slot < 0 || slot >= b->slots) return 0;
    if (hipSetDevice(b->device) != hipSuccess || !chain_join(b) || !sync_params(b, nullptr)) return 0;
    const size_t idx = static_cast<size_t>(instance) * b->slots + slot;
    const int floats = static_cast<int>(b->ring_floats[idx]);
    if (out && floats) {
        hipStreamSynchronize(b->stream);
        const int n = std::min(floats, max_floats);
        if (!b->hip_ok(hipMemcpy(out, b->h_rings[idx], static_cast<size_t>(n) * sizeof(float), hipMemcpyDeviceToHost), "hipMemcpy(ring)")) return 0;
    }
    return floats;
}

int oalsfx_batch_read_source(oalsfx_batch* b, int instance, oalsfx_source_params* params, oalsfx_source_state* state)
{
    if (instance < 0 || instance >= b->n) return b->fail(kErrRange) ? 1 : 0;
    if (!b->hip_ok(hipSetDevice(b->device), "hipSetDevice") || !chain_join(b)) return 0;
    if (!sync_params(b, nullptr)) return 0;
    if (params) *params = b->h_source[instance];
    if (state) {
        if (!b->hip_ok(hipStreamSynchronize(b->stream), "hipStreamSynchronize")) return 0;
        if (!b->hip_ok(hipMemcpy(state, b->d_source_state + instance, sizeof(*state), hipMemcpyDeviceToHost), "hipMemcpy(source state)")) return 0;
    }
    return 1;
}

namespace {

constexpr uint32_t kBlobMagic = 0x58465342u;
constexpr uint32_t kBlobVersion = 1;
constexpr size_t kBlobAlign = 256;

size_t blob_round(size_t v) { return (v + kBlobAlign - 1) / kBlobAlign * kBlobAlign; }

struct BlobHeader {
    uint32_t magic, version;
    int32_t format, rate, slots, count;
    uint64_t total_bytes;
    uint64_t table_offset;
    uint64_t prefix_bytes;
    uint64_t device_stride;
    uint64_t host_stride;
};
static_assert(sizeof(BlobHeader) <= kBlobAlign, "the header fits its section");

struct BlobEntry { uint64_t host, device, ring[OALSFX_MAX_SLOTS]; };

struct BlobSlot {
    int32_t type;
    uint32_t ring_floats;
    uint32_t update_seq;
    uint32_t frames_since_start;
    uint32_t mod_ever;
    uint32_t reserved[3];
};

struct BlobHost {
    oalsfxpp::Effect active[OALSFX_MAX_SLOTS], deferred[OALSFX_MAX_SLOTS];
    oalsfxpp::SendProps direct_props, direct_deferred, aux_props[OALSFX_MAX_SLOTS], aux_deferred[OALSFX_MAX_SLOTS];
    BlobSlot slot[OALSFX_MAX_SLOTS];
    uint32_t touched;
    uint32_t aux_written;
};
static_assert(std::is_trivially_copyable<oalsfxpp::Effect>::value && std::is_trivially_copyable<oalsfxpp::SendProps>::value, "records are bytes");

constexpr size_t kStateBytes = sizeof(oalsfx_hip::SlotStateLines);
constexpr size_t kSourceStateBytes = sizeof(oalsfx_source_state);
constexpr size_t kSourceParamsBytes = sizeof(oalsfx_source_params);
static_assert(kStateBytes % 16 == 0 && kSourceStateBytes % 16 == 0 && kSourceParamsBytes % 16 == 0, "records copy in 16-byte pieces");
size_t source_state_at(int slots) { return slots * kStateBytes; }
size_t source_params_at(int slots) { return source_state_at(slots) + kSourceStateBytes; }
size_t device_stride(int slots) { return blob_round(source_params_at(slots) + kSourceParamsBytes); }

int instance_at(const int* instances, int k) { return instances ? instances[k] : k; }

bool instances_ok(oalsfx_batch* b, const int* instances, int count)
{
    if (count < 0 || (!instances && count > b->n)) return b->fail(kErrRange);
    if (instances)
        for (int k = 0; k < count; ++k)
            if (instances[k] < 0 || instances[k] >= b->n) return b->fail(kErrRange);
    return true;
}

uint64_t blob_layout(const oalsfx_batch* b, const int* instances, int count, std::vector<BlobEntry>& entries, BlobHeader& h)
{
    h = BlobHeader{};
    h.magic = kBlobMagic;
    h.version = kBlobVersion;
    h.format = b->format;
    h.rate = b->rate;
    h.slots = b->slots;
    h.count = count;
    h.table_offset = kBlobAlign;
    h.host_stride = blob_round(sizeof(BlobHost));
    h.device_stride = device_stride(b->slots);
    const uint64_t host0 = h.table_offset + blob_round(static_cast<size_t>(count) * sizeof(BlobEntry));
    h.prefix_bytes = host0 + static_cast<uint64_t>(count) * h.host_stride;
// ... 95 lines not shown
            if (b->ring_floats[idx] == recs[k].slot[s].ring_floats) continue;
            release_slab(b, idx);
            b->rings_table_dirty = true;
            if (recs[k].slot[s].ring_floats) taking.push_back(idx);
        }
    for (int k = 0, t = 0; k < count; ++k)
        for (int s = 0; s < b->slots; ++s) {
            const size_t idx = static_cast<size_t>(instances[k]) * b->slots + s;
            if (t >= static_cast<int>(taking.size()) || taking[t] != idx) continue;
            ++t;
            const size_t floats = recs[k].slot[s].ring_floats;
            RingPool& pool = b->pools[floats];
            std::vector<float*>& from = pool.free_clean.empty() ? pool.free_dirty : pool.free_clean;
            b->h_rings[idx] = from.back();
            from.pop_back();
            b->ring_floats[idx] = floats;
        }
    for (int k = 0; k < count; ++k) {
        const int i = instances[k];
        const BlobHost& r = recs[k];
        InstanceHost& h = b->inst[i];
        h.effect_count = b->slots;
        for (int s = 0; s < OALSFX_MAX_SLOTS; ++s) {
            h.active[s] = r.active[s];
            h.deferred[s] = r.deferred[s];
            h.aux_props[s] = r.aux_props[s];
            h.aux_deferred[s] = r.aux_deferred[s];
            h.slot_changed[s] = s < b->slots;
            h.slot_retyped[s] = false;
        }
        h.direct_props = r.direct_props;
        h.direct_deferred = r.direct_deferred;
        h.source_changed = true;
        for (int s = 0; s < b->slots; ++s) b->started_at[static_cast<size_t>(i) * b->slots + s] = b->frames_total - r.slot[s].frames_since_start;
        mark_dirty(b, i);
    }
    b->off_grid_known = false;
    if (!sync_params(b, nullptr)) return false;
    std::vector<oalsfx_hip::StateSegment> segs;
    std::vector<oalsfx_hip::StateSeenFix> fixes;
    for (int k = 0; k < count; ++k) {
        const int i = instances[k];
        const BlobHost& r = recs[k];
        const char* dev = blob ? blob + entries[k].device : nullptr;
        for (int s = 0; s < b->slots; ++s) {
            const size_t idx = static_cast<size_t>(i) * b->slots + s;
            b->xf_ok[idx] = 0;
            b->mod_ever[idx] = r.slot[s].mod_ever ? 1 : 0;
            if (b->mod_ever[idx]) b->modulated[s] = true;
            segs.push_back({dev ? dev + s * kStateBytes : nullptr, b->d_state + idx, kStateBytes, 0});
            fixes.push_back({&b->d_state[idx].seen_seq, dev ? reinterpret_cast<const unsigned*>(dev + s * kStateBytes) : nullptr, r.slot[s].update_seq,
                             b->h_params[idx].update_seq});
            if (b->h_rings[idx]) segs.push_back({blob ? blob + entries[k].ring[s] : nullptr, b->h_rings[idx], b->ring_floats[idx] * sizeof(float), 0});
        }
        segs.push_back({dev ? dev + source_state_at(b->slots) : nullptr, b->d_source_state + i, kSourceStateBytes, 0});
        b->aux_written[i] = r.aux_written ? 1 : 0;
        if (r.aux_written && dev) {
            const oalsfx_source_params& sp = sends[k];
            auto has_filter = [&](const oalsfx_source_params& x) {
                int any = x.direct.filter_type;
                for (int s = 0; s < b->slots; ++s)
                    if (x.aux[s].out_channels != 0) any |= x.aux[s].filter_type;
                return any != OALSFX_AF_NONE;
            };
            b->n_filtered += static_cast<int>(has_filter(sp)) - static_cast<int>(has_filter(b->h_source[i]));
            b->inst_filtered[i] = has_filter(sp) ? 1 : 0;
            b->inside_version = ~0u;
            b->h_source[i] = sp;
            segs.push_back({dev + source_params_at(b->slots), b->d_source + i, kSourceParamsBytes, 0});
            b->lists_dirty = true;
        }
        if (r.touched && !b->touched[i]) { b->touched[i] = 1; b->touched_list.push_back(i); }
        if (!r.touched) b->touched[i] = 0;
    }
    b->lists_dirty = true;
    b->touched_list.erase(std::remove_if(b->touched_list.begin(), b->touched_list.end(), [&](int i) { return !b->touched[i]; }), b->touched_list.end());
    return state_io_launch(b, segs, fixes, {}, 0, false);
}

}

unsigned long long oalsfx_batch_snapshot_bytes(oalsfx_batch* b, const int* instances, int count)
{
    if (!b) { g_last_error = "Null batch."; return 0; }
    if (!instances_ok(b, instances, count)) return 0;
    std::vector<BlobEntry> entries;
    BlobHeader h;
    return blob_layout(b, instances, count, entries, h);
}

int oalsfx_batch_snapshot(oalsfx_batch* b, const int* instances, int count, void* dst, unsigned long long bytes)
{
    if (!b) { g_last_error = "Null batch."; return 0; }
    if (!instances_ok(b, instances, count)) return 0;
    if (!dst) return b->fail("No snapshot buffer.") ? 1 : 0;
    if (reinterpret_cast<uintptr_t>(dst) % 16 != 0) return b->fail("The snapshot buffer is not 16-byte aligned.") ? 1 : 0;
    if (b->poisoned) return b->fail(b->fault_text) ? 1 : 0;
    std::vector<BlobEntry> entries;
    BlobHeader h;
    if (blob_layout(b, instances, count, entries, h) > bytes) return b->fail("The snapshot buffer is too small (oalsfx_batch_snapshot_bytes).") ? 1 : 0;
    if (!state_io_begin(b) || !sync_params(b, nullptr)) return 0;
    std::vector<char> prefix(h.prefix_bytes, 0);
    std::memcpy(prefix.data(), &h, sizeof(h));
    std::memcpy(prefix.data() + h.table_offset, entries.data(), entries.size() * sizeof(BlobEntry));
    char* const out = static_cast<char*>(dst);
    std::vector<oalsfx_hip::StateSegment> segs;
    segs.push_back({nullptr, out, h.prefix_bytes, 0});
    for (int k = 0; k < count; ++k) {
        const int i = instance_at(instances, k);
        const InstanceHost& ih = b->inst[i];
        BlobHost r{};
        for (int s = 0; s < OALSFX_MAX_SLOTS; ++s) {
            r.active[s] = ih.active[s];
            r.deferred[s] = ih.deferred[s];
            r.aux_props[s] = ih.aux_props[s];
            r.aux_deferred[s] = ih.aux_deferred[s];
        }
        r.direct_props = ih.direct_props;
        r.direct_deferred = ih.direct_deferred;
        r.touched = b->touched[i];
        r.aux_written = b->aux_written[i];
        char* const dev = out + entries[k].device;
        for (int s = 0; s < b->slots; ++s) {
            const size_t idx = static_cast<size_t>(i) * b->slots + s;
            BlobSlot& sl = r.slot[s];
            sl.type = b->h_params[idx].type;
            sl.ring_floats = static_cast<uint32_t>(b->ring_floats[idx]);
            sl.update_seq = b->h_params[idx].update_seq;
            sl.frames_since_start = b->frames_total - b->started_at[idx];
            sl.mod_ever = b->mod_ever[idx];
            if (sl.ring_floats != static_cast<uint32_t>(ring_floats_for(sl.type, b->rate)) || (sl.ring_floats && !entries[k].ring[s]))
                return b->fail("Internal error: a slot's delay lines do not match its effect type.") ? 1 : 0;
            segs.push_back({b->d_state + idx, dev + s * kStateBytes, kStateBytes, 0});
            if (sl.ring_floats) segs.push_back({b->h_rings[idx], out + entries[k].ring[s], sl.ring_floats * sizeof(float), 0});
        }
        segs.push_back({b->d_source_state + i, dev + source_state_at(b->slots), kSourceStateBytes, 0});
        segs.push_back({b->d_source + i, dev + source_params_at(b->slots), kSourceParamsBytes, 0});
        std::memcpy(prefix.data() + entries[k].host, &r, sizeof(r));
    }
    return state_io_launch(b, segs, {}, prefix, 1, true) ? 1 : 0;
}

int oalsfx_batch_restore(oalsfx_batch* b, const int* instances, int count, const void* src, unsigned long long bytes)
{
    if (!b) { g_last_error = "Null batch."; return 0; }
    if (!instances_ok(b, instances, count)) return 0;
    if (!src) return b->fail("No snapshot buffer.") ? 1 : 0;
    if (reinterpret_cast<uintptr_t>(src) % 16 != 0) return b->fail("The snapshot buffer is not 16-byte aligned.") ? 1 : 0;
    if (b->poisoned) return b->fail(b->fault_text) ? 1 : 0;
    std::vector<int> targets(count);
    std::vector<uint8_t> taken(b->n, 0);
    for (int k = 0; k < count; ++k) {
        targets[k] = instance_at(instances, k);
        if (taken[targets[k]]) return b->fail("An instance is listed twice as a restore target.") ? 1 : 0;
        taken[targets[k]] = 1;
    }
    if (bytes < sizeof(BlobHeader)) return b->fail("The snapshot is shorter than its header.") ? 1 : 0;
    if (!state_io_begin(b) || !b->hip_ok(hipStreamSynchronize(b->stream), "hipStreamSynchronize")) return 0;
    const char* const blob = static_cast<const char*>(src);
    BlobHeader h;
    if (!b->hip_ok(hipMemcpy(&h, blob, sizeof(h), hipMemcpyDefault), "hipMemcpy(snapshot header)")) return 0;
    if (h.magic != kBlobMagic) return b->fail("Not a snapshot (bad magic value).") ? 1 : 0;
    if (h.version != kBlobVersion) return b->fail("Snapshot version is not supported.") ? 1 : 0;
    if (h.format != b->format || h.rate != b->rate || h.slots != b->slots)
        return b->fail("The snapshot's channel format, sampling rate or effect count differs from the batch's.") ? 1 : 0;
    if (h.count != count) return b->fail("The snapshot holds another number of instances than the target list.") ? 1 : 0;
    if (h.total_bytes > bytes) return b->fail("The snapshot is larger than the bytes given.") ? 1 : 0;
    if (h.table_offset != kBlobAlign || h.host_stride != blob_round(sizeof(BlobHost)) || h.device_stride != device_stride(b->slots) ||
        h.prefix_bytes > h.total_bytes || h.table_offset + static_cast<uint64_t>(count) * sizeof(BlobEntry) > h.prefix_bytes)
        return b->fail("The snapshot's layout is damaged.") ? 1 : 0;
    std::vector<char> prefix(h.prefix_bytes);
    if (!b->hip_ok(hipMemcpy(prefix.data(), blob, prefix.size(), hipMemcpyDefault), "hipMemcpy(snapshot records)")) return 0;
    std::vector<BlobEntry> entries(count);
    std::memcpy(entries.data(), prefix.data() + h.table_offset, count * sizeof(BlobEntry));
    std::vector<BlobHost> recs(count);
    auto within = [&](uint64_t off, uint64_t len, uint64_t lo, uint64_t hi) { return off % 16 == 0 && off >= lo && off <= hi && len <= hi - off; };
    for (int k = 0; k < count; ++k) {
        const BlobEntry& e = entries[k];
        if (!within(e.host, sizeof(BlobHost), h.table_offset, h.prefix_bytes) || !within(e.device, h.device_stride, h.prefix_bytes, h.total_bytes))
            return b->fail("The snapshot's layout is damaged.") ? 1 : 0;
        std::memcpy(&recs[k], prefix.data() + e.host, sizeof(BlobHost));
        for (int s = 0; s < b->slots; ++s) {
            const BlobSlot& sl = recs[k].slot[s];
            const bool type_ok = sl.type >= 0 && sl.type < OALSFX_TYPE_COUNT && static_cast<int>(recs[k].active[s].type_) == sl.type;
            if (!type_ok || sl.ring_floats != static_cast<uint32_t>(ring_floats_for(sl.type, b->rate)) ||
                (sl.ring_floats && !within(e.ring[s], sl.ring_floats * sizeof(float), h.prefix_bytes, h.total_bytes)))
                return b->fail("The snapshot's records are damaged.") ? 1 : 0;
        }
    }
    std::vector<oalsfx_source_params> sends(count);
    uint64_t lo = ~uint64_t(0), hi = 0;
    for (int k = 0; k < count; ++k)
        if (recs[k].aux_written) { lo = std::min(lo, entries[k].device); hi = std::max(hi, entries[k].device + h.device_stride); }
    if (hi > lo) {
        std::vector<char> span(hi - lo);
        if (!b->hip_ok(hipMemcpy(span.data(), blob + lo, span.size(), hipMemcpyDefault), "hipMemcpy(sends)")) return 0;
        for (int k = 0; k < count; ++k)
            if (recs[k].aux_written) std::memcpy(&sends[k], span.data() + (entries[k].device - lo) + source_params_at(b->slots), sizeof(oalsfx_source_params));
    }
    return put_images(b, targets.data(), count, recs, blob, entries, sends) ? 1 : 0;
}

int oalsfx_batch_reset(oalsfx_batch* b, const int* instances, int count)
{
    if (!b) { g_last_error = "Null batch."; return 0; }
    if (!instances_ok(b, instances, count)) return 0;
    if (b->poisoned) return b->fail(b->fault_text) ? 1 : 0;
    std::vector<int> targets(count);
    for (int k = 0; k < count; ++k) targets[k] = instance_at(instances, k);
    InstanceHost fresh;
    fresh.initialize(b->slots);
    BlobHost r{};
    for (int s = 0; s < OALSFX_MAX_SLOTS; ++s) {
        r.active[s] = fresh.active[s];
        r.deferred[s] = fresh.deferred[s];
        r.aux_props[s] = fresh.aux_props[s];
        r.aux_deferred[s] = fresh.aux_deferred[s];
        r.slot[s].type = static_cast<int32_t>(fresh.active[s].type_);
    }
    r.direct_props = fresh.direct_props;
    r.direct_deferred = fresh.direct_deferred;
    if (!state_io_begin(b)) return 0;
    return put_images(b, targets.data(), count, std::vector<BlobHost>(count, r), nullptr, std::vector<BlobEntry>(count, BlobEntry{}),
                      std::vector<oalsfx_source_params>()) ? 1 : 0;
}

namespace {

std::atomic<int> g_downmix_vector{4};

bool downmix_args_ok(oalsfx_batch* b, int frames, int n_buses)
{
    if (frames < 0) return b->fail("Frame count is negative.");
    if (n_buses < 1) return b->fail("Bus count is out of range.");
    if (b->poisoned) return b->fail(b->fault_text);
    if (static_cast<size_t>(frames) * b->channels > 0xFFFFFFFFull) return b->fail("Frame count is out of range.");
    if (b->routing_dirty) {
        b->route_max = -1;
        for (int v : b->route_bus) b->route_max = std::max(b->route_max, v);
    }
    if (b->route_max >= n_buses)
        for (int i = 0; i < b->n; ++i)
            if (b->route_bus[i] >= n_buses) {
                char text[96];
                std::snprintf(text, sizeof(text), "Instance %d is routed to bus %d; the call has %d.", i, b->route_bus[i], n_buses);
                b->error_store = text;
                return b->fail(b->error_store.c_str());
            }
    return true;
}

bool downmix_grow(oalsfx_batch* b, float** buffer, size_t* capacity, size_t floats, const char* what)
{
    if (floats <= *capacity) return true;
    hipFree(*buffer);
    *buffer = nullptr;
    *capacity = 0;
    if (!b->hip_ok(hipMalloc(reinterpret_cast<void**>(buffer), floats * sizeof(float)), what)) return false;
    *capacity = floats;
    return true;
}

bool queue_behind_batch(oalsfx_batch* b, hipStream_t stream)
{
    if (stream == b->stream) {
        if (b->last_launch_stream && b->last_launch_stream != b->stream && !b->hip_ok(hipStreamWaitEvent(b->stream, b->ev_mixed, 0), "hipStreamWaitEvent"))
            return false;
    } else {
        if (!b->hip_ok(hipEventRecord(b->ev_dm_order, b->stream), "hipEventRecord") || !b->hip_ok(hipStreamWaitEvent(stream, b->ev_dm_order, 0), "hipStreamWaitEvent"))
            return false;
        if (b->last_launch_stream && b->last_launch_stream != b->stream && b->last_launch_stream != stream &&
            !b->hip_ok(hipStreamWaitEvent(stream, b->ev_mixed, 0), "hipStreamWaitEvent"))
            return false;
    }
    return true;
}

bool downmix_queue(oalsfx_batch* b, size_t elements, const float* src, int n_buses, float* dst, hipStream_t stream)
{
    if (!queue_behind_batch(b, stream)) return false;
    if (b->dm_pending && b->dm_stream != stream && !b->hip_ok(hipStreamWaitEvent(stream, b->ev_downmix, 0), "hipStreamWaitEvent")) return false;
    if (b->routing_dirty || b->dm_buses != n_buses) {
        if (b->dm_pending && !b->hip_ok(hipEventSynchronize(b->ev_downmix), "hipEventSynchronize")) return false;
        b->dm_pending = false;
        b->dm_buses = 0;
        b->dm_table.build(b->route_bus.data(), b->route_gain.data(), b->n, n_buses);
        size_t at[4];
        const size_t bytes = std::max<size_t>(b->dm_table.packed_bytes(at), 16);
        if (bytes > b->dm_table_capacity) {
            if (b->h_dm_table) (void)hipHostFree(b->h_dm_table);
            hipFree(b->d_dm_table);
            b->h_dm_table = b->d_dm_table = nullptr;
            b->dm_table_capacity = 0;
            if (!b->hip_ok(hipHostMalloc(reinterpret_cast<void**>(&b->h_dm_table), bytes), "hipHostMalloc(downmix table)")) return false;
            if (!b->hip_ok(hipMalloc(reinterpret_cast<void**>(&b->d_dm_table), bytes), "hipMalloc(downmix table)")) return false;
            b->dm_table_capacity = bytes;
        }
        b->dm_table.pack(b->h_dm_table);
        if (!b->hip_ok(hipMemcpyAsync(b->d_dm_table, b->h_dm_table, bytes, hipMemcpyHostToDevice, stream), "hipMemcpyAsync(downmix table)")) return false;
        b->dm_dev.chunks = reinterpret_cast<const oalsfx_hip::DownmixChunk*>(b->d_dm_table + at[0]);
        b->dm_dev.sums = reinterpret_cast<const oalsfx_hip::DownmixSum*>(b->d_dm_table + at[1]);
        b->dm_dev.members = reinterpret_cast<const int*>(b->d_dm_table + at[2]);
        b->dm_dev.gains = reinterpret_cast<const float*>(b->d_dm_table + at[3]);
        b->dm_dev.n_chunks = static_cast<int>(b->dm_table.chunks.size());
        b->dm_dev.n_sums = static_cast<int>(b->dm_table.sums.size());
        b->dm_buses = n_buses;
        b->routing_dirty = false;
        ++b->dm_uploads;
        b->dm_pending = true;
        b->dm_stream = stream;
        if (!b->hip_ok(hipEventRecord(b->ev_downmix, stream), "hipEventRecord")) return false;
    }
    const int vector = oalsfx_hip::downmix_vector(src, dst, elements, g_downmix_vector.load(std::memory_order_relaxed));
    if (!oalsfx_hip::downmix_fits(b->dm_dev, elements, vector)) return b->fail("The downmix is too large for one launch.");
    if (!downmix_grow(b, &b->d_dm_partials, &b->dm_partials_capacity, static_cast<size_t>(b->dm_table.partial_rows) * elements, "hipMalloc(downmix partials)"))
        return false;
    oalsfx_hip::launch_downmix(b->dm_dev, src, dst, b->d_dm_partials, elements, vector, stream);
    if (!b->hip_ok(hipGetLastError(), "downmix launch")) return false;
    if (!b->hip_ok(hipEventRecord(b->ev_downmix, stream), "hipEventRecord")) return false;
    b->dm_pending = true;
    b->dm_stream = stream;
    return true;
}

}

int oalsfx_batch_set_routing(oalsfx_batch* b, int first, int count, const int* bus, const float* gain)
{
    if (!b) { g_last_error = "Null batch."; return 0; }
    if (!range_ok(b, first, count)) return 0;
    if (bus)
        for (int k = 0; k < count; ++k)
            if (bus[k] < -1) return b->fail("Bus number is out of range.") ? 1 : 0;
    if (!bus && !gain) return 1;
    for (int k = 0; k < count; ++k) {
        if (bus) b->route_bus[first + k] = bus[k];
        if (gain) b->route_gain[first + k] = gain[k];
    }
    if (count) b->routing_dirty = true;
    return 1;
}

int oalsfx_batch_get_routing(const oalsfx_batch* b, int instance, int* bus, float* gain)
{
    if (!b || instance < 0 || instance >= b->n) return 0;
    if (bus) *bus = b->route_bus[instance];
    if (gain) *gain = b->route_gain[instance];
    return 1;
}

int oalsfx_batch_downmix_device(oalsfx_batch* b, int frames, const float* src_dev, int n_buses, float* dst_bus_dev, void* hip_stream)
{
    if (!b) { g_last_error = "Null batch."; return 0; }
    if (!downmix_args_ok(b, frames, n_buses)) return 0;
    if (frames == 0) return 1;
    if (!src_dev) return b->fail(kErrNoSrc) ? 1 : 0;
    if (!dst_bus_dev) return b->fail(kErrNoDst) ? 1 : 0;
    const size_t elements = static_cast<size_t>(frames) * b->channels;
    if ((reinterpret_cast<uintptr_t>(src_dev) | reinterpret_cast<uintptr_t>(dst_bus_dev)) % sizeof(float) != 0)
        return b->fail("A downmix buffer is not 4-byte aligned.") ? 1 : 0;
    const char* const s0 = reinterpret_cast<const char*>(src_dev);
    const char* const d0 = reinterpret_cast<const char*>(dst_bus_dev);
    if (d0 < s0 + static_cast<size_t>(b->n) * elements * sizeof(float) && s0 < d0 + static_cast<size_t>(n_buses) * elements * sizeof(float))
        return b->fail("The bus buffer overlaps the source buffer.") ? 1 : 0;
    if (!b->hip_ok(hipSetDevice(b->device), "hipSetDevice") || !chain_join(b)) return 0;
    return downmix_queue(b, elements, src_dev, n_buses, dst_bus_dev, hip_stream ? static_cast<hipStream_t>(hip_stream) : b->stream) ? 1 : 0;
}

int oalsfx_batch_mix_downmix(oalsfx_batch* b, int frames, const float* src_host, int n_buses, float* dst_bus_host)
{
    if (!b) { g_last_error = "Null batch."; return 0; }
    if (!downmix_args_ok(b, frames, n_buses)) return 0;
    if (frames == 0) return 1;
    if (!src_host) return b->fail(kErrNoSrc) ? 1 : 0;
    if (!dst_bus_host) return b->fail(kErrNoDst) ? 1 : 0;
    if (!b->hip_ok(hipSetDevice(b->device), "hipSetDevice") || !chain_join(b)) return 0;
    const size_t elements = static_cast<size_t>(frames) * b->channels, floats = elements * b->n, bus_floats = elements * n_buses;
    if (!grow_io(b, floats) || !downmix_grow(b, &b->d_dm_out, &b->dm_out_capacity, bus_floats, "hipMalloc(bus output)")) return 0;
    if (!b->hip_ok(hipMemcpyAsync(b->d_io_src, src_host, floats * sizeof(float), hipMemcpyHostToDevice, b->stream), "hipMemcpyAsync(src)")) return 0;
    if (!mix_device(b, frames, b->d_io_src, b->d_io_dst, b->stream)) return 0;
    if (!downmix_queue(b, elements, b->d_io_dst, n_buses, b->d_dm_out, b->stream)) return 0;
    if (!b->hip_ok(hipMemcpyAsync(dst_bus_host, b->d_dm_out, bus_floats * sizeof(float), hipMemcpyDeviceToHost, b->stream), "hipMemcpyAsync(buses)")) return 0;
    if (!b->hip_ok(hipStreamSynchronize(b->stream), "hipStreamSynchronize")) return 0;
    b->dm_pending = false;
    poll_exact(b);
    return check_fault(b) ? 1 : 0;
}

namespace {

bool meter_args_ok(oalsfx_batch* b, int frames, float threshold, int flags)
{
    if (frames < 0) return b->fail("Frame count is negative.");
    if (!(threshold >= 0.0F)) return b->fail("The meter threshold is negative or not a number.");
    if (flags & ~OALSFX_METER_CARRY) return b->fail("Unknown meter flags.");
    if (b->poisoned) return b->fail(b->fault_text);
    if (static_cast<size_t>(frames) * b->channels > 0xFFFFFFFFull) return b->fail("Frame count is out of range.");
    return true;
}

bool meter_launch(oalsfx_batch* b, int rows, int frames, const float* src, float threshold, int flags, oalsfx_meter* meters, hipStream_t stream)
{
    if (!oalsfx_hip::meter_fits(rows)) return b->fail("The meter pass is too large for one launch.");
    if (!oalsfx_hip::launch_meter(src, rows, static_cast<unsigned>(frames), b->channels, threshold, (flags & OALSFX_METER_CARRY) != 0, meters, stream))
        return b->fail("No meter kernel for this channel count.");
    return b->hip_ok(hipGetLastError(), "meter launch");
}

}

int oalsfx_batch_meter_device(oalsfx_batch* b, int rows, int frames, const float* src_dev, float threshold, int flags, oalsfx_meter* meters_dev,
                              void* hip_stream)
{
    if (!b) { g_last_error = "Null batch."; return 0; }
    if (rows < 1) return b->fail("Row count is out of range.") ? 1 : 0;
    if (!meter_args_ok(b, frames, threshold, flags)) return 0;
    if (!oalsfx_hip::meter_fits(rows)) return b->fail("The meter pass is too large for one launch.") ? 1 : 0;
    if (frames == 0) return 1;
    if (!src_dev) return b->fail(kErrNoSrc) ? 1 : 0;
    if (!meters_dev) return b->fail("No meter records.") ? 1 : 0;
    if (reinterpret_cast<uintptr_t>(src_dev) % sizeof(float) != 0) return b->fail("The meter source is not 4-byte aligned.") ? 1 : 0;
    if (reinterpret_cast<uintptr_t>(meters_dev) % 16 != 0) return b->fail("The meter records are not 16-byte aligned.") ? 1 : 0;
    const char* const s0 = reinterpret_cast<const char*>(src_dev);
    const char* const m0 = reinterpret_cast<const char*>(meters_dev);
    if (m0 < s0 + static_cast<size_t>(rows) * frames * b->channels * sizeof(float) && s0 < m0 + static_cast<size_t>(rows) * sizeof(oalsfx_meter))
        return b->fail("The meter records overlap the source buffer.") ? 1 : 0;
    if (!b->hip_ok(hipSetDevice(b->device), "hipSetDevice") || !chain_join(b)) return 0;
    const hipStream_t stream = hip_stream ? static_cast<hipStream_t>(hip_stream) : b->stream;
    if (!queue_behind_batch(b, stream)) return 0;
    return meter_launch(b, rows, frames, src_dev, threshold, flags, meters_dev, stream) ? 1 : 0;
}

namespace {

bool sampler_queue(oalsfx_batch* b, int frames, float* dst, hipStream_t stream);

int downmix_meter_call(oalsfx_batch* b, int frames, const float* src_host, bool play, int n_buses, float* dst_bus_host, float threshold, int flags,
                       oalsfx_meter* voice_meters_host, oalsfx_meter* bus_meters_host)
{
    if (!meter_args_ok(b, frames, threshold, flags)) return 0;
    if (!play && !voice_meters_host && !bus_meters_host) return oalsfx_batch_mix_downmix(b, frames, src_host, n_buses, dst_bus_host);
    if (!downmix_args_ok(b, frames, n_buses)) return 0;
    if (!oalsfx_hip::meter_fits(std::max(b->n, n_buses))) return b->fail("The meter pass is too large for one launch.") ? 1 : 0;
    if (play && !oalsfx_hip::sampler_fits(b->n)) return b->fail("The sampler pass is too large for one launch.") ? 1 : 0;
    if (frames == 0) return 1;
    if (!play && !src_host) return b->fail(kErrNoSrc) ? 1 : 0;
    if (!dst_bus_host) return b->fail(kErrNoDst) ? 1 : 0;
    if (!b->hip_ok(hipSetDevice(b->device), "hipSetDevice") || !chain_join(b)) return 0;
    const size_t elements = static_cast<size_t>(frames) * b->channels, floats = elements * b->n, bus_floats = elements * n_buses;
    const size_t records = static_cast<size_t>(b->n) + n_buses;
    if (!grow_io(b, floats) || !downmix_grow(b, &b->d_dm_out, &b->dm_out_capacity, bus_floats, "hipMalloc(bus output)")) return 0;
    if ((voice_meters_host || bus_meters_host) && records > b->meters_capacity) {
        hipFree(b->d_meters);
        b->d_meters = nullptr;
        b->meters_capacity = 0;
        if (!b->hip_ok(hipMalloc(reinterpret_cast<void**>(&b->d_meters), records * sizeof(oalsfx_meter)), "hipMalloc(meters)")) return 0;
        b->meters_capacity = records;
    }
    oalsfx_meter* const d_voices = b->d_meters;
    oalsfx_meter* const d_buses = b->d_meters + b->n;
    if (flags & OALSFX_METER_CARRY) {
        if (voice_meters_host &&
            !b->hip_ok(hipMemcpyAsync(d_voices, voice_meters_host, b->n * sizeof(oalsfx_meter), hipMemcpyHostToDevice, b->stream), "hipMemcpyAsync(meters)"))
            return 0;
        if (bus_meters_host &&
            !b->hip_ok(hipMemcpyAsync(d_buses, bus_meters_host, n_buses * sizeof(oalsfx_meter), hipMemcpyHostToDevice, b->stream), "hipMemcpyAsync(meters)"))
            return 0;
    }
    if (play) {
        if (!sampler_queue(b, frames, b->d_io_src, b->stream)) return 0;
    } else if (!b->hip_ok(hipMemcpyAsync(b->d_io_src, src_host, floats * sizeof(float), hipMemcpyHostToDevice, b->stream), "hipMemcpyAsync(src)")) return 0;
    if (!mix_device(b, frames, b->d_io_src, b->d_io_dst, b->stream)) return 0;
    if (!downmix_queue(b, elements, b->d_io_dst, n_buses, b->d_dm_out, b->stream)) return 0;
    if (voice_meters_host && !meter_launch(b, b->n, frames, b->d_io_dst, threshold, flags, d_voices, b->stream)) return 0;
    if (bus_meters_host && !meter_launch(b, n_buses, frames, b->d_dm_out, threshold, flags, d_buses, b->stream)) return 0;
    if (!b->hip_ok(hipMemcpyAsync(dst_bus_host, b->d_dm_out, bus_floats * sizeof(float), hipMemcpyDeviceToHost, b->stream), "hipMemcpyAsync(buses)")) return 0;
    if (voice_meters_host && bus_meters_host && bus_meters_host == voice_meters_host + b->n) {
        if (!b->hip_ok(hipMemcpyAsync(voice_meters_host, d_voices, records * sizeof(oalsfx_meter), hipMemcpyDeviceToHost, b->stream), "hipMemcpyAsync(meters)"))
            return 0;
    } else {
        if (voice_meters_host &&
            !b->hip_ok(hipMemcpyAsync(voice_meters_host, d_voices, b->n * sizeof(oalsfx_meter), hipMemcpyDeviceToHost, b->stream), "hipMemcpyAsync(meters)"))
            return 0;
        if (bus_meters_host &&
            !b->hip_ok(hipMemcpyAsync(bus_meters_host, d_buses, n_buses * sizeof(oalsfx_meter), hipMemcpyDeviceToHost, b->stream), "hipMemcpyAsync(meters)"))
            return 0;
    }
    if (!b->hip_ok(hipStreamSynchronize(b->stream), "hipStreamSynchronize")) return 0;
    b->dm_pending = false;
    poll_exact(b);
    return check_fault(b) ? 1 : 0;
}

}

int oalsfx_batch_mix_downmix_meter(oalsfx_batch* b, int frames, const float* src_host, int n_buses, float* dst_bus_host, float threshold, int flags,
                                   oalsfx_meter* voice_meters_host, oalsfx_meter* bus_meters_host)
{
    if (!b) { g_last_error = "Null batch."; return 0; }
    return downmix_meter_call(b, frames, src_host, false, n_buses, dst_bus_host, threshold, flags, voice_meters_host, bus_meters_host);
}

long long oalsfx_debug_downmix_uploads(const oalsfx_batch* b) { return b ? b->dm_uploads : 0; }
void oalsfx_debug_downmix_vector(int max_floats) { g_downmix_vector.store(max_floats, std::memory_order_relaxed); }

namespace {

constexpr uint32_t kSamplerFlags = OALSFX_SAMPLER_PLAYING | OALSFX_SAMPLER_LOOP | OALSFX_SAMPLER_LINEAR;

size_t pcm_bytes(uint32_t format) { return format == OALSFX_PCM_F32 ? 4 : format == OALSFX_PCM_S16 ? 2 : 1; }

struct AssetRange { uintptr_t lo = 0, hi = 0; };

bool asset_resident(oalsfx_batch* b, uintptr_t data, uint64_t bytes, AssetRange& known)
{
    if (data >= known.lo && data <= known.hi && bytes <= known.hi - data) return true;
    hipPointerAttribute_t attr{};
    void* base = nullptr;
    size_t size = 0;
    if (hipPointerGetAttributes(&attr, reinterpret_cast<const void*>(data)) != hipSuccess || attr.type != hipMemoryTypeDevice || attr.device != b->device ||
        hipMemGetAddressRange(reinterpret_cast<hipDeviceptr_t*>(&base), &size, reinterpret_cast<hipDeviceptr_t>(data)) != hipSuccess) {
        (void)hipGetLastError();
// ... 2 lines not shown
    const uintptr_t lo = reinterpret_cast<uintptr_t>(base);
    if (data < lo || data - lo > size || bytes > size - (data - lo)) return false;
    known.lo = lo;
    known.hi = lo + size;
    return true;
}

bool sampler_ok(oalsfx_batch* b, const oalsfx_sampler& s, AssetRange& known)
{
    if (s.flags & ~kSamplerFlags) return b->fail("Unknown sampler flags.");
    if (s.format != OALSFX_PCM_U8 && s.format != OALSFX_PCM_S16 && s.format != OALSFX_PCM_F32) return b->fail("Unknown sampler format.");
    if (s.reserved != 0) return b->fail("The sampler's reserved field is not 0.");
    if (s.channels != 1 && s.channels != static_cast<uint32_t>(b->channels)) return b->fail("The sampler's channel count is neither 1 nor the batch's.");
    if (!(s.flags & OALSFX_SAMPLER_PLAYING)) return true;
    if (s.data == 0) return b->fail("A playing sampler has no data.");
    if (s.frames == 0 || s.frames >= 0x80000000U) return b->fail("The sampler's frame count is out of range.");
    if (s.data % pcm_bytes(s.format) != 0) return b->fail("The sampler's data is not aligned to its element size.");
    uint64_t end = static_cast<uint64_t>(s.frames) << OALSFX_SAMPLER_FRAC_BITS;
    if (s.flags & OALSFX_SAMPLER_LOOP) {
        if (s.loop_start >= s.loop_end || s.loop_end > s.frames) return b->fail("The sampler's loop region is out of range.");
        end = static_cast<uint64_t>(s.loop_end) << OALSFX_SAMPLER_FRAC_BITS;
    }
    if (s.position >= end) return b->fail("The sampler's position is past its end.");
    if (!asset_resident(b, static_cast<uintptr_t>(s.data), static_cast<uint64_t>(s.frames) * s.channels * pcm_bytes(s.format), known))
        return b->fail("The sampler's data does not lie inside one allocation on the batch's device.");
    return true;
}

bool sampler_args_ok(oalsfx_batch* b, int frames)
{
    if (frames < 0) return b->fail("Frame count is negative.");
    if (b->poisoned) return b->fail(b->fault_text);
    if (static_cast<size_t>(frames) * b->channels > 0xFFFFFFFFull) return b->fail("Frame count is out of range.");
    if (!oalsfx_hip::sampler_fits(b->n)) return b->fail("The sampler pass is too large for one launch.");
    return true;
}

bool sampler_queue(oalsfx_batch* b, int frames, float* dst, hipStream_t stream)
{
    if (!queue_behind_batch(b, stream)) return false;
    if (b->sampler_pending && b->sampler_stream != stream && !b->hip_ok(hipStreamWaitEvent(stream, b->ev_sampler, 0), "hipStreamWaitEvent")) return false;
    if (!b->sampler_dirty_list.empty()) {
        const size_t count = b->sampler_dirty_list.size();
        if (b->sampler_stage_pending && !b->hip_ok(hipEventSynchronize(b->ev_sampler_staged), "hipEventSynchronize")) return false;
        b->sampler_stage_pending = false;
        if (count > b->sampler_stage_capacity) {
            if (b->h_sampler_stage) (void)hipHostFree(b->h_sampler_stage);
            b->h_sampler_stage = nullptr;
            b->sampler_stage_capacity = 0;
            const size_t capacity = std::min<size_t>(b->n, std::max<size_t>(2 * count, 64));
            if (!b->hip_ok(hipHostMalloc(reinterpret_cast<void**>(&b->h_sampler_stage), capacity * (sizeof(oalsfx_sampler) + sizeof(int))), "hipHostMalloc(samplers)"))
                return false;
            b->sampler_stage_capacity = capacity;
        }
        oalsfx_sampler* const changed = reinterpret_cast<oalsfx_sampler*>(b->h_sampler_stage);
        int* const index = reinterpret_cast<int*>(changed + b->sampler_stage_capacity);
        for (size_t k = 0; k < count; ++k) {
            const int i = b->sampler_dirty_list[k];
            index[k] = i;
            changed[k] = b->h_samplers[i];
            b->sampler_dirty[i] = 0;
        }
        b->sampler_dirty_list.clear();
        oalsfx_hip::launch_sampler_upload(b->d_samplers, index, changed, static_cast<int>(count), stream);
        b->sampler_stage_pending = true;
        ++b->sampler_uploads;
        if (!b->hip_ok(hipGetLastError(), "sampler upload") || !b->hip_ok(hipEventRecord(b->ev_sampler_staged, stream), "hipEventRecord")) return false;
        b->sampler_pending = true;
        b->sampler_stream = stream;
        if (!b->hip_ok(hipEventRecord(b->ev_sampler, stream), "hipEventRecord")) return false;
    }
    if (!oalsfx_hip::launch_sampler(b->d_samplers, b->n, static_cast<unsigned>(frames), b->channels, dst, stream)) return b->fail("No sampler kernel for this channel count.");
    b->samplers_ahead = true;
    b->sampler_pending = true;
    b->sampler_stream = stream;
    if (!b->hip_ok(hipGetLastError(), "sampler launch")) return false;
    return b->hip_ok(hipEventRecord(b->ev_sampler, stream), "hipEventRecord");
}

}

int oalsfx_batch_set_samplers(oalsfx_batch* b, const int* instances, int count, const oalsfx_sampler* samplers)
{
    if (!b) { g_last_error = "Null batch."; return 0; }
    if (!instances_ok(b, instances, count)) return 0;
    if (b->poisoned) return b->fail(b->fault_text) ? 1 : 0;
    if (count == 0) return 1;
    if (!samplers) return b->fail("No sampler records.") ? 1 : 0;
    if (instances) {
        std::vector<uint8_t> taken(b->n, 0);
        for (int k = 0; k < count; ++k) {
            if (taken[instances[k]]) return b->fail("An instance is listed twice as a sampler target.") ? 1 : 0;
            taken[instances[k]] = 1;
        }
    }
    if (!b->hip_ok(hipSetDevice(b->device), "hipSetDevice")) return 0;
    AssetRange known;
    for (int k = 0; k < count; ++k)
        if (!sampler_ok(b, samplers[k], known)) return 0;
    for (int k = 0; k < count; ++k) {
        const int i = instance_at(instances, k);
        b->h_samplers[i] = samplers[k];
        if (!b->sampler_dirty[i]) {
            b->sampler_dirty[i] = 1;
            b->sampler_dirty_list.push_back(i);
        }
    }
    return 1;
}

int oalsfx_batch_get_samplers(oalsfx_batch* b, const int* instances, int count, oalsfx_sampler* out)
{
    if (!b) { g_last_error = "Null batch."; return 0; }
    if (!instances_ok(b, instances, count)) return 0;
    if (count == 0) return 1;
    if (!out) return b->fail("No sampler records.") ? 1 : 0;
    if (b->samplers_ahead) {
        std::vector<oalsfx_sampler> now(b->n);
        if (!b->hip_ok(hipSetDevice(b->device), "hipSetDevice")) return 0;
        if (b->sampler_pending && !b->hip_ok(hipEventSynchronize(b->ev_sampler), "hipEventSynchronize")) return 0;
        if (!b->hip_ok(hipMemcpy(now.data(), b->d_samplers, now.size() * sizeof(oalsfx_sampler), hipMemcpyDeviceToHost), "hipMemcpy(samplers)")) return 0;
        b->sampler_pending = false;
        for (int i = 0; i < b->n; ++i)
            if (!b->sampler_dirty[i]) b->h_samplers[i] = now[i];
        b->samplers_ahead = false;
    }
    for (int k = 0; k < count; ++k) out[k] = b->h_samplers[instance_at(instances, k)];
    return 1;
}

int oalsfx_batch_sample_device(oalsfx_batch* b, int frames, float* dst_dev, void* hip_stream)
{
    if (!b) { g_last_error = "Null batch."; return 0; }
    if (!sampler_args_ok(b, frames)) return 0;
    if (frames == 0) return 1;
    if (!dst_dev) return b->fail(kErrNoDst) ? 1 : 0;
    if (reinterpret_cast<uintptr_t>(dst_dev) % sizeof(float) != 0) return b->fail("The sampler destination is not 4-byte aligned.") ? 1 : 0;
    if (!b->hip_ok(hipSetDevice(b->device), "hipSetDevice") || !chain_join(b)) return 0;
    return sampler_queue(b, frames, dst_dev, hip_stream ? static_cast<hipStream_t>(hip_stream) : b->stream) ? 1 : 0;
}

int oalsfx_batch_play_downmix_meter(oalsfx_batch* b, int frames, int n_buses, float* dst_bus_host, float threshold, int flags,
                                    oalsfx_meter* voice_meters_host, oalsfx_meter* bus_meters_host)
{
    if (!b) { g_last_error = "Null batch."; return 0; }
    return downmix_meter_call(b, frames, nullptr, true, n_buses, dst_bus_host, threshold, flags, voice_meters_host, bus_meters_host);
}

long long oalsfx_debug_sampler_uploads(const oalsfx_batch* b) { return b ? b->sampler_uploads : 0; }

int oalsfx_batch_fill_synthetic(oalsfx_batch* b, int frames, unsigned buffer_index, float* dst_dev, void* hip_stream)
{
    if (!b->hip_ok(hipSetDevice(b->device), "hipSetDevice") || !chain_join(b)) return 0;
    oalsfx_hip::launch_fill_synthetic(dst_dev, b->n, frames * b->channels, buffer_index, hip_stream ? static_cast<hipStream_t>(hip_stream) : b->stream);
    return b->hip_ok(hipGetLastError(), "fill_synthetic") ? 1 : 0;
}

int oalsfx_batch_kernel_timing(oalsfx_batch* b, int enable)
{
    if (!b->hip_ok(hipSetDevice(b->device), "hipSetDevice") || !chain_join(b)) return 0;
    for (auto& t : b->timed) { b->event_pool.push_back(t.start); b->event_pool.push_back(t.stop); }
    b->timed.clear();
    b->timing_every = enable > 0 ? enable : 0;
    b->timing = false;
    b->mix_calls = 0;
    while (b->timing_every && b->event_pool.size() < 2048) {
        hipEvent_t e = nullptr;
        if (!b->hip_ok(hipEventCreate(&e), "hipEventCreate")) return 0;
        b->event_pool.push_back(e);
    }
    return 1;
}

int oalsfx_batch_kernel_timing_read(oalsfx_batch* b, int effect_type, int* launches, double* total_ms)
{
    if (!b->hip_ok(hipSetDevice(b->device), "hipSetDevice") || !chain_join(b)) return 0;
    int n = 0;
    double ms = 0.0;
    int key = (effect_type >= 0 && effect_type < OALSFX_REVERB) ? kTimedWaveEffects : effect_type;
    if (key == OALSFX_REVERB) key = OALSFX_EAX_REVERB;
    if (key == OALSFX_EAX_REVERB + kTimedGeneralOffset) key = OALSFX_REVERB + kTimedGeneralOffset;
    if (effect_type == 32) key = kTimedMixed;
    for (auto& t : b->timed) {
        if (t.type != key) continue;
        if (!b->hip_ok(hipEventSynchronize(t.stop), "hipEventSynchronize")) return 0;
        float e = 0.0F;
        if (!b->hip_ok(hipEventElapsedTime(&e, t.start, t.stop), "hipEventElapsedTime")) return 0;
        ms += e;
        ++n;
    }
    if (launches) *launches = n;
    if (total_ms) *total_ms = ms;
    return 1;
}

int oalsfx_batch_kernel_timing_samples(oalsfx_batch* b, int effect_type, double* out_us, int max_samples)
{
    if (!b->hip_ok(hipSetDevice(b->device), "hipSetDevice") || !chain_join(b)) return -1;
    int key = (effect_type >= 0 && effect_type < OALSFX_REVERB) ? kTimedWaveEffects : effect_type;
    if (key == OALSFX_REVERB) key = OALSFX_EAX_REVERB;
    if (key == OALSFX_EAX_REVERB + kTimedGeneralOffset) key = OALSFX_REVERB + kTimedGeneralOffset;
    if (effect_type == 32) key = kTimedMixed;
    int n = 0;
    for (auto& t : b->timed) {
        if (t.type != key) continue;
        if (out_us && n < max_samples) {
            if (!b->hip_ok(hipEventSynchronize(t.stop), "hipEventSynchronize")) return -1;
            float e = 0.0F;
            if (!b->hip_ok(hipEventElapsedTime(&e, t.start, t.stop), "hipEventElapsedTime")) return -1;
            out_us[n] = e * 1e3;
        }
        ++n;
    }
    return n;
}

int oalsfx_batch_plan(oalsfx_batch* b, int slot, int counts[4])
{
    if (slot < 0 || slot >= b->slots) return b->fail(kErrSlot) ? 1 : 0;
    if (!b->hip_ok(hipSetDevice(b->device), "hipSetDevice") || !chain_join(b)) return 0;
    poll_exact(b);
    if (!sync_params(b, nullptr)) return 0;
    int light = 0;
    for (int t = 0; t < OALSFX_REVERB; ++t) light += b->list_count[slot][t];
    counts[0] = light;
    counts[1] = b->fast_count[slot];
    counts[2] = b->slow_count[slot];
    counts[3] = b->general_count[slot];
    return 1;
}

const char* oalsfx_batch_last_reverb_kernel(const oalsfx_batch* b) { return b->last_steady_kernel; }

long long oalsfx_batch_chained_calls(const oalsfx_batch* b) { return b->chained_calls; }

int oalsfx_batch_multi_counts(const oalsfx_batch* b, long long* buffers_in_passes, long long* passes)
{
    if (!b) { g_last_error = "Null batch."; return 0; }
    if (buffers_in_passes) *buffers_in_passes = b->multi_buffers;
    if (passes) *passes = b->multi_passes;
    return 1;
}

long long oalsfx_debug_chain_same_cu(oalsfx_batch* b)
{
    unsigned v = 0;
    if (hipSetDevice(b->device) != hipSuccess || !chain_join(b) || hipStreamSynchronize(b->stream) != hipSuccess) return -1;
    if (hipMemcpy(&v, b->d_turn + static_cast<size_t>(b->n) * b->slots + 1, sizeof(v), hipMemcpyDeviceToHost) != hipSuccess) return -1;
    return v;
}

int oalsfx_debug_host_pipeline(oalsfx_batch* b, int* form, double* probe_us_three_streams, double* probe_us_one_stream)
{
    if (form) *form = b->pipe_mode;
    if (probe_us_three_streams) *probe_us_three_streams = b->pipe_probe_us[0];
    if (probe_us_one_stream) *probe_us_one_stream = b->pipe_probe_us[1];
    return 1;
}

unsigned long long oalsfx_trim_pools(void)
{
    return uncached_pool().trim(0);
}

unsigned long long oalsfx_pools_waiting_bytes(void) { return uncached_pool().bytes_waiting(); }

void oalsfx_debug_gate_skew(oalsfx_batch* b, unsigned skew) { if (b) b->gate_skew = skew; }
int oalsfx_debug_chain_given_up(const oalsfx_batch* b) { return b && b->chain_given_up ? 1 : 0; }

int oalsfx_debug_chain_started(oalsfx_batch* b, unsigned* host_total, unsigned* device_total)
{
    unsigned v = 0;
    if (!b->hip_ok(hipSetDevice(b->device), "hipSetDevice") || !chain_join(b) || !b->hip_ok(hipStreamSynchronize(b->stream), "hipStreamSynchronize")) return 0;
    if (b->d_turn && !b->hip_ok(hipMemcpy(&v, b->d_turn + static_cast<size_t>(b->n) * b->slots, sizeof(v), hipMemcpyDeviceToHost), "hipMemcpy")) return 0;
    if (host_total) *host_total = b->started_total;
    if (device_total) *device_total = v;
    return 1;
}

int oalsfx_device_pci_bus_id(int device_id, char* out, int len)
{
    if (!out || len < 16) return 0;
    return hipDeviceGetPCIBusId(out, len, device_id) == hipSuccess ? 1 : 0;
}

int oalsfx_batch_event_overhead(oalsfx_batch* b, int repeats, double* avg_us)
{
    if (repeats <= 0 || !b->hip_ok(hipSetDevice(b->device), "hipSetDevice") || !chain_join(b)) return 0;
    hipEvent_t e0 = b->take_event(), e1 = b->take_event();
    double total = 0.0;
    bool ok = true;
    for (int r = 0; r < repeats && ok; ++r) {
        oalsfx_hip::launch_null(b->stream);
        hipEventRecord(e0, b->stream);
        hipEventRecord(e1, b->stream);
        ok = hipEventSynchronize(e1) == hipSuccess;
        float ms = 0.0F;
        ok = ok && hipEventElapsedTime(&ms, e0, e1) == hipSuccess;
        total += ms;
    }
    b->event_pool.push_back(e0);
    b->event_pool.push_back(e1);
    if (avg_us) *avg_us = total * 1e3 / repeats;
    return ok ? 1 : 0;
}

int oalsfx_batch_placement(const oalsfx_batch* b, int* chunks, int* candidates, double* best_us, double* worst_us)
{
    if (chunks) *chunks = b->placed_chunks;
    if (candidates) *candidates = b->placement_candidates;
    if (best_us) *best_us = b->placement_best_us;
    if (worst_us) *worst_us = b->placement_worst_us;
    return 1;
}

int oalsfx_debug_probe_pointer(void* slabs, int instances, int slab_floats, int repeats, double* avg_us)
{
    if (!slabs || instances <= 0 || repeats <= 0 || slab_floats < 65536) return 0;
    const int wps = std::max(1, 4096 / instances);
    hipEvent_t e0, e1;
    hipEventCreate(&e0); hipEventCreate(&e1);
    for (int r = 0; r < 2; ++r) oalsfx_hip::launch_ring_probe(static_cast<float*>(slabs), instances, slab_floats, 256u * r, wps, nullptr);
    hipEventRecord(e0, nullptr);
    for (int r = 0; r < repeats; ++r) oalsfx_hip::launch_ring_probe(static_cast<float*>(slabs), instances, slab_floats, 256u * (2 + r), wps, nullptr);
    hipEventRecord(e1, nullptr);
    bool ok = hipEventSynchronize(e1) == hipSuccess;
    float ms = 0.0F;
    ok = ok && hipEventElapsedTime(&ms, e0, e1) == hipSuccess;
    if (avg_us) *avg_us = ms * 1e3 / repeats;
    hipEventDestroy(e0); hipEventDestroy(e1);
    return ok ? 1 : 0;
}

int oalsfx_debug_probe_rings(oalsfx_batch* b, int repeats, double* avg_us)
{
    if (hipSetDevice(b->device) != hipSuccess || !chain_join(b) || !sync_params(b, nullptr) || b->ring_chunks.empty() || repeats <= 0) return 0;
    if (!b->hip_ok(hipStreamSynchronize(b->stream), "hipStreamSynchronize")) return 0;
    const auto& rc = b->ring_chunks.front();
    const size_t slab_floats = static_cast<size_t>(ring_floats_for(OALSFX_EAX_REVERB, b->rate));
    const int instances = static_cast<int>(rc.bytes / (slab_floats * sizeof(float)));
    hipEvent_t e0, e1;
    hipEventCreate(&e0); hipEventCreate(&e1);
    for (int r = 0; r < 4; ++r) oalsfx_hip::launch_stream_pattern(reinterpret_cast<float*>(rc.base), instances, 1, 256u * r, slab_floats, 0, b->stream);
    hipEventRecord(e0, b->stream);
    for (int r = 0; r < repeats; ++r) oalsfx_hip::launch_stream_pattern(reinterpret_cast<float*>(rc.base), instances, 1, 256u * (4 + r), slab_floats, 0, b->stream);
    hipEventRecord(e1, b->stream);
    bool ok = hipEventSynchronize(e1) == hipSuccess;
    float ms = 0.0F;
    ok = ok && hipEventElapsedTime(&ms, e0, e1) == hipSuccess;
    if (avg_us) *avg_us = ms * 1e3 / repeats;
    hipEventDestroy(e0); hipEventDestroy(e1);
    return ok ? 1 : 0;
}

int oalsfx_debug_move_rings(oalsfx_batch* b, int keep_old)
{
    if (hipSetDevice(b->device) != hipSuccess || !chain_join(b) || !sync_params(b, nullptr)) return 0;
    if (!b->hip_ok(hipStreamSynchronize(b->stream), "hipStreamSynchronize")) return 0;
    const size_t total = static_cast<size_t>(b->n) * b->slots;
    for (auto& rc : b->ring_chunks) {
        void* fresh = nullptr;
        if (!b->hip_ok(handed_on_malloc(b, &fresh, rc.bytes), "hipMalloc(rings)")) return 0;
        if (!b->hip_ok(hipMemcpy(fresh, rc.base, rc.bytes, hipMemcpyDeviceToDevice), "hipMemcpy(rings)")) return 0;
        const ptrdiff_t delta = static_cast<char*>(fresh) - rc.base;
        auto inside = [&](float* p) { return reinterpret_cast<char*>(p) >= rc.base && reinterpret_cast<char*>(p) < rc.base + rc.bytes; };
        auto moved = [&](float* p) { return reinterpret_cast<float*>(reinterpret_cast<char*>(p) + delta); };
        for (size_t idx = 0; idx < total; ++idx)
            if (b->h_rings[idx] && inside(b->h_rings[idx])) b->h_rings[idx] = moved(b->h_rings[idx]);
        for (auto& kv : b->pools) {
            for (auto& p : kv.second.free_clean) if (inside(p)) p = moved(p);
            for (auto& p : kv.second.free_dirty) if (inside(p)) p = moved(p);
        }
        if (keep_old) {
        } else {
            for (auto& c : b->chunks) if (c == rc.alloc) c = nullptr;
            handed_on_free(rc.alloc);
        }
        b->chunks.push_back(fresh);
        rc.base = static_cast<char*>(fresh);
        rc.alloc = fresh;
    }
    return b->hip_ok(hipMemcpy(b->d_rings, b->h_rings.data(), total * sizeof(float*), hipMemcpyHostToDevice), "hipMemcpy(ring table)") ? 1 : 0;
}

unsigned long long oalsfx_debug_ring_address(oalsfx_batch* b, int instance, int slot)
{
    if (instance < 0 || instance >= b->n || slot < 0 || slot >= b->slots) return 0;
    if (hipSetDevice(b->device) != hipSuccess || !chain_join(b) || !sync_params(b, nullptr)) return 0;
    return reinterpret_cast<unsigned long long>(b->h_rings[static_cast<size_t>(instance) * b->slots + slot]);
}

void oalsfx_debug_set_flags(int flags) { g_debug_flags.store(flags < 0 ? 0 : flags, std::memory_order_relaxed); }

int oalsfx_debug_hbm_sweep(int device_id, unsigned long long bytes, int write, int repeats)
{
    if (hipSetDevice(device_id) != hipSuccess) return 0;
    float* buf = nullptr;
    float* sink = nullptr;
    if (hipMalloc(reinterpret_cast<void**>(&buf), bytes) != hipSuccess) return 0;
    if (hipMalloc(reinterpret_cast<void**>(&sink), 256) != hipSuccess) { (void)hipFree(buf); return 0; }
    (void)hipMemset(buf, 0, bytes);
    for (int r = 0; r < repeats; ++r) oalsfx_hip::launch_hbm_sweep(buf, bytes / sizeof(float), write, sink, nullptr);
    const bool ok = hipDeviceSynchronize() == hipSuccess;
    (void)hipFree(buf);
    (void)hipFree(sink);
    return ok ? 1 : 0;
}

int oalsfx_debug_stream_pattern(int device_id, int instances, int dwords_per_lane, int repeats, int slab_floats, int pos_skew, double* avg_us)
{
    if (hipSetDevice(device_id) != hipSuccess || instances <= 0 || repeats <= 0) return 0;
    if (dwords_per_lane != 1 && dwords_per_lane != 2 && dwords_per_lane != 4) return 0;
    float* slabs = nullptr;
    if (slab_floats < 235520) return 0;
    const size_t bytes = static_cast<size_t>(instances) * slab_floats * sizeof(float);
    if (hipMalloc(reinterpret_cast<void**>(&slabs), bytes) != hipSuccess) return 0;
    (void)hipMemset(slabs, 0, bytes);
    hipEvent_t e0, e1;
    hipEventCreate(&e0); hipEventCreate(&e1);
    for (int r = 0; r < 8; ++r) oalsfx_hip::launch_stream_pattern(slabs, instances, dwords_per_lane, 256u * r, slab_floats, pos_skew, nullptr);
    hipEventRecord(e0, nullptr);
    for (int r = 0; r < repeats; ++r) oalsfx_hip::launch_stream_pattern(slabs, instances, dwords_per_lane, 256u * (8 + r), slab_floats, pos_skew, nullptr);
    hipEventRecord(e1, nullptr);
    bool ok = hipEventSynchronize(e1) == hipSuccess;
    float ms = 0.0F;
    ok = ok && hipEventElapsedTime(&ms, e0, e1) == hipSuccess;
    if (avg_us) *avg_us = ms * 1e3 / repeats;
    hipEventDestroy(e0); hipEventDestroy(e1);
    (void)hipFree(slabs);
    return ok ? 1 : 0;
}

}
```

### oalsfxpp_amd/csrc/host/group.cpp

```cpp
#include <condition_variable>
#include <cstdio>
#include <cstring>
#include <functional>
#include <mutex>
#include <string>
#include <thread>
#include <vector>

#include "oalsfx_hip.h"

namespace {

struct Worker {
    std::thread thread;
    std::mutex m;
    std::condition_variable cv;
    std::function<int()> task;
    bool has_task = false, done = false, quit = false;
    int result = 1;

    void loop()
    {
        std::unique_lock<std::mutex> lock(m);
        for (;;) {
// ... 5 lines not shown
            const int r = t();
            lock.lock();
            result = r;
            done = true;
            cv.notify_all();
        }
    }
    void post(std::function<int()> t)
    {
        std::lock_guard<std::mutex> lock(m);
        task = std::move(t);
        has_task = true;
        done = false;
        cv.notify_all();
    }
    int join()
    {
        std::unique_lock<std::mutex> lock(m);
        cv.wait(lock, [&] { return done; });
        return result;
    }
};

}

struct oalsfx_group {
    int n = 0, channels = 0;
    std::vector<int> device, first, count;
    std::vector<oalsfx_batch*> batch;
    std::vector<Worker*> worker;
    std::vector<std::vector<float>> bus_part;
    std::string error;

    bool fail(const std::string& msg) { error = msg; return false; }
    bool shard_failed(size_t k, const char* what)
    {
        char head[96];
        std::snprintf(head, sizeof(head), "device %d (instances %d .. %d), %s: ", device[k], first[k], first[k] + count[k] - 1, what);
        error = std::string(head) + oalsfx_batch_error(batch[k]);
        return false;
    }
    int overlap(size_t k, int f, int c, int* local_first) const
    {
        const int lo = f > first[k] ? f : first[k], hi = (f + c < first[k] + count[k]) ? f + c : first[k] + count[k];
        *local_first = lo - first[k];
        return hi > lo ? hi - lo : 0;
    }
};

namespace {
std::string g_group_error;

void shard_range(int n_total, int k, int shards, int* first, int* count)
{
    const int base = n_total / shards, extra = n_total % shards;
    *first = k * base + (k < extra ? k : extra);
    *count = base + (k < extra ? 1 : 0);
}
}

extern "C" {

const char* oalsfx_group_last_error(void) { return g_group_error.c_str(); }

oalsfx_group* oalsfx_group_create(int n_total, const int* device_ids, int n_devices, int channel_format, int sampling_rate, int effect_count)
{
    g_group_error.clear();
    if (n_devices <= 0 || !device_ids) { g_group_error = "A group needs at least one device."; return nullptr; }
    if (n_total < n_devices) { g_group_error = "Instance count is out of range (fewer instances than devices)."; return nullptr; }
    oalsfx_group* g = new oalsfx_group;
    g->n = n_total;
    for (int k = 0; k < n_devices; ++k) {
        int f = 0, c = 0;
        shard_range(n_total, k, n_devices, &f, &c);
        oalsfx_batch* b = oalsfx_batch_create(c, channel_format, sampling_rate, effect_count, device_ids[k]);
        if (!b) {
            char head[64];
            std::snprintf(head, sizeof(head), "device %d: ", device_ids[k]);
            g_group_error = std::string(head) + oalsfx_last_error();
            for (oalsfx_batch* made : g->batch) oalsfx_batch_destroy(made);
            delete g;
            return nullptr;
        }
        g->device.push_back(device_ids[k]);
        g->first.push_back(f);
        g->count.push_back(c);
        g->batch.push_back(b);
    }
    g->channels = oalsfx_batch_channels(g->batch[0]);
    for (int k = 0; k < n_devices; ++k) {
        Worker* w = new Worker;
        w->thread = std::thread([w] { w->loop(); });
        g->worker.push_back(w);
    }
    return g;
}

void oalsfx_group_destroy(oalsfx_group* g)
{
    if (!g) return;
    for (Worker* w : g->worker) {
        { std::lock_guard<std::mutex> lock(w->m); w->quit = true; w->cv.notify_all(); }
        w->thread.join();
        delete w;
    }
    for (oalsfx_batch* b : g->batch) oalsfx_batch_destroy(b);
    delete g;
}

const char* oalsfx_group_error(const oalsfx_group* g) { return g ? g->error.c_str() : g_group_error.c_str(); }
int oalsfx_group_instances(const oalsfx_group* g) { return g->n; }
int oalsfx_group_channels(const oalsfx_group* g) { return g->channels; }
int oalsfx_group_devices(const oalsfx_group* g) { return static_cast<int>(g->batch.size()); }

int oalsfx_group_shard(const oalsfx_group* g, int k, int* device_id, int* first, int* count)
{
    if (k < 0 || k >= static_cast<int>(g->batch.size())) return 0;
    if (device_id) *device_id = g->device[k];
    if (first) *first = g->first[k];
    if (count) *count = g->count[k];
    return 1;
}

oalsfx_batch* oalsfx_group_batch(oalsfx_group* g, int k) { return (k < 0 || k >= static_cast<int>(g->batch.size())) ? nullptr : g->batch[k]; }

#define OALSFX_GROUP_RANGE_CHECK()                                                                          \
    if (first < 0 || count < 0 || first + count > g->n) return g->fail("Instance range is out of range.") ? 1 : 0

int oalsfx_group_set_effect(oalsfx_group* g, int first, int count, int slot, const oalsfx_effect* effects, int stride_bytes)
{
    OALSFX_GROUP_RANGE_CHECK();
    for (size_t k = 0; k < g->batch.size(); ++k) {
        int lf = 0;
        const int c = g->overlap(k, first, count, &lf);
        if (!c) continue;
        const auto* e = reinterpret_cast<const oalsfx_effect*>(reinterpret_cast<const char*>(effects) + static_cast<size_t>(g->first[k] + lf - first) * stride_bytes);
        if (!oalsfx_batch_set_effect(g->batch[k], lf, c, slot, e, stride_bytes)) return g->shard_failed(k, "set_effect") ? 1 : 0;
    }
    return 1;
}

int oalsfx_group_set_effect_type(oalsfx_group* g, int first, int count, int slot, int effect_type)
{
    OALSFX_GROUP_RANGE_CHECK();
    for (size_t k = 0; k < g->batch.size(); ++k) {
        int lf = 0;
        const int c = g->overlap(k, first, count, &lf);
        if (c && !oalsfx_batch_set_effect_type(g->batch[k], lf, c, slot, effect_type)) return g->shard_failed(k, "set_effect_type") ? 1 : 0;
    }
    return 1;
}

int oalsfx_group_set_effect_props(oalsfx_group* g, int first, int count, int slot, const void* props, int stride_bytes)
{
    OALSFX_GROUP_RANGE_CHECK();
    for (size_t k = 0; k < g->batch.size(); ++k) {
        int lf = 0;
        const int c = g->overlap(k, first, count, &lf);
        if (!c) continue;
        const void* p = static_cast<const char*>(props) + static_cast<size_t>(g->first[k] + lf - first) * stride_bytes;
        if (!oalsfx_batch_set_effect_props(g->batch[k], lf, c, slot, p, stride_bytes)) return g->shard_failed(k, "set_effect_props") ? 1 : 0;
    }
    return 1;
}

int oalsfx_group_set_send_props(oalsfx_group* g, int first, int count, int slot, const oalsfx_send_props* props)
// ... 140 lines not shown
```

### oalsfxpp_amd/lib.py

```python
import ctypes as C
import os

from . import desc

_HERE = os.path.dirname(os.path.abspath(__file__))
LIB_PATH = os.path.join(_HERE, "csrc", "liboalsfx_hip.so")

_fp = C.POINTER(C.c_float)
_lib = None

SIGNATURES = {
    "oalsfx_batch_create": (C.c_void_p, [C.c_int, C.c_int, C.c_int, C.c_int, C.c_int]),
    "oalsfx_batch_destroy": (None, [C.c_void_p]),
    "oalsfx_batch_error": (C.c_char_p, [C.c_void_p]),
    "oalsfx_last_error": (C.c_char_p, []),
    "oalsfx_batch_instances": (C.c_int, [C.c_void_p]),
    "oalsfx_batch_channels": (C.c_int, [C.c_void_p]),
    "oalsfx_batch_sampling_rate": (C.c_int, [C.c_void_p]),
    "oalsfx_batch_effect_count": (C.c_int, [C.c_void_p]),
    "oalsfx_batch_set_effect": (C.c_int, [C.c_void_p, C.c_int, C.c_int, C.c_int, C.c_void_p, C.c_int]),
    "oalsfx_batch_set_effect_at": (C.c_int, [C.c_void_p, C.c_void_p, C.c_int, C.c_int, C.c_void_p, C.c_int]),
    "oalsfx_batch_set_effect_type": (C.c_int, [C.c_void_p, C.c_int, C.c_int, C.c_int, C.c_int]),
    "oalsfx_batch_set_effect_props": (C.c_int, [C.c_void_p, C.c_int, C.c_int, C.c_int, C.c_void_p, C.c_int]),
    "oalsfx_batch_set_send_props": (C.c_int, [C.c_void_p, C.c_int, C.c_int, C.c_int, C.POINTER(desc.SendProps)]),
    "oalsfx_batch_get_effect": (C.c_int, [C.c_void_p, C.c_int, C.c_int, C.c_int, C.POINTER(desc.Effect)]),
    "oalsfx_batch_get_send_props": (C.c_int, [C.c_void_p, C.c_int, C.c_int, C.c_int, C.POINTER(desc.SendProps)]),
    "oalsfx_batch_apply_changes": (C.c_int, [C.c_void_p, C.c_int, C.c_int]),
    "oalsfx_batch_mix": (C.c_int, [C.c_void_p, C.c_int, _fp, _fp]),
    "oalsfx_batch_mix_timed": (C.c_int, [C.c_void_p, C.c_int, _fp, _fp, C.POINTER(C.c_double)]),
    "oalsfx_batch_mix_device": (C.c_int, [C.c_void_p, C.c_int, C.c_void_p, C.c_void_p, C.c_void_p]),
    "oalsfx_batch_mix_device_multi": (C.c_int, [C.c_void_p, C.c_int, C.c_int, C.POINTER(C.c_void_p), C.POINTER(C.c_void_p), C.c_void_p]),
    "oalsfx_batch_synchronize": (C.c_int, [C.c_void_p]),
    "oalsfx_batch_mix_async": (C.c_int, [C.c_void_p, C.c_int, _fp, _fp]),
    "oalsfx_batch_wait": (C.c_int, [C.c_void_p]),
    "oalsfx_pinned_alloc": (C.c_void_p, [C.c_ulonglong]),
    "oalsfx_pinned_free": (None, [C.c_void_p]),
    "oalsfx_batch_stream": (C.c_void_p, [C.c_void_p]),
    "oalsfx_batch_read_slot": (C.c_int, [C.c_void_p, C.c_int, C.c_int, C.POINTER(desc.SlotParams), C.POINTER(desc.SlotState)]),
    "oalsfx_batch_read_ring": (C.c_int, [C.c_void_p, C.c_int, C.c_int, _fp, C.c_int]),
    "oalsfx_batch_read_source": (C.c_int, [C.c_void_p, C.c_int, C.POINTER(desc.SourceParams), C.POINTER(desc.SourceState)]),
    "oalsfx_batch_snapshot_bytes": (C.c_ulonglong, [C.c_void_p, C.POINTER(C.c_int), C.c_int]),
    "oalsfx_batch_snapshot": (C.c_int, [C.c_void_p, C.POINTER(C.c_int), C.c_int, C.c_void_p, C.c_ulonglong]),
    "oalsfx_batch_restore": (C.c_int, [C.c_void_p, C.POINTER(C.c_int), C.c_int, C.c_void_p, C.c_ulonglong]),
    "oalsfx_batch_reset": (C.c_int, [C.c_void_p, C.POINTER(C.c_int), C.c_int]),
    "oalsfx_batch_set_routing": (C.c_int, [C.c_void_p, C.c_int, C.c_int, C.POINTER(C.c_int), _fp]),
    "oalsfx_batch_get_routing": (C.c_int, [C.c_void_p, C.c_int, C.POINTER(C.c_int), _fp]),
    "oalsfx_batch_downmix_device": (C.c_int, [C.c_void_p, C.c_int, C.c_void_p, C.c_int, C.c_void_p, C.c_void_p]),
    "oalsfx_batch_mix_downmix": (C.c_int, [C.c_void_p, C.c_int, _fp, C.c_int, _fp]),
    "oalsfx_batch_meter_device": (C.c_int, [C.c_void_p, C.c_int, C.c_int, C.c_void_p, C.c_float, C.c_int, C.c_void_p, C.c_void_p]),
    "oalsfx_batch_mix_downmix_meter": (C.c_int, [C.c_void_p, C.c_int, _fp, C.c_int, _fp, C.c_float, C.c_int, C.c_void_p, C.c_void_p]),
    "oalsfx_batch_set_samplers": (C.c_int, [C.c_void_p, C.POINTER(C.c_int), C.c_int, C.c_void_p]),
    "oalsfx_batch_get_samplers": (C.c_int, [C.c_void_p, C.POINTER(C.c_int), C.c_int, C.c_void_p]),
    "oalsfx_batch_sample_device": (C.c_int, [C.c_void_p, C.c_int, C.c_void_p, C.c_void_p]),
    "oalsfx_batch_play_downmix_meter": (C.c_int, [C.c_void_p, C.c_int, C.c_int, _fp, C.c_float, C.c_int, C.c_void_p, C.c_void_p]),
    "oalsfx_batch_fill_synthetic": (C.c_int, [C.c_void_p, C.c_int, C.c_uint, C.c_void_p, C.c_void_p]),
    "oalsfx_batch_kernel_timing": (C.c_int, [C.c_void_p, C.c_int]),
    "oalsfx_batch_kernel_timing_read": (C.c_int, [C.c_void_p, C.c_int, C.POINTER(C.c_int), C.POINTER(C.c_double)]),
    "oalsfx_batch_event_overhead": (C.c_int, [C.c_void_p, C.c_int, C.POINTER(C.c_double)]),
    "oalsfx_batch_kernel_timing_samples": (C.c_int, [C.c_void_p, C.c_int, C.POINTER(C.c_double), C.c_int]),
    "oalsfx_batch_plan": (C.c_int, [C.c_void_p, C.c_int, C.POINTER(C.c_int)]),
    "oalsfx_batch_placement": (C.c_int, [C.c_void_p, C.POINTER(C.c_int), C.POINTER(C.c_int), C.POINTER(C.c_double), C.POINTER(C.c_double)]),
    "oalsfx_batch_last_reverb_kernel": (C.c_char_p, [C.c_void_p]),
    "oalsfx_batch_mix_gather": (C.c_int, [C.c_void_p, C.c_int, C.POINTER(C.c_void_p), C.POINTER(C.c_void_p)]),
    "oalsfx_batch_chained_calls": (C.c_longlong, [C.c_void_p]),
    "oalsfx_group_create": (C.c_void_p, [C.c_int, C.POINTER(C.c_int), C.c_int, C.c_int, C.c_int, C.c_int]),
    "oalsfx_group_destroy": (None, [C.c_void_p]),
    "oalsfx_group_error": (C.c_char_p, [C.c_void_p]),
    "oalsfx_group_last_error": (C.c_char_p, []),
    "oalsfx_group_instances": (C.c_int, [C.c_void_p]),
    "oalsfx_group_channels": (C.c_int, [C.c_void_p]),
    "oalsfx_group_devices": (C.c_int, [C.c_void_p]),
    "oalsfx_group_shard": (C.c_int, [C.c_void_p, C.c_int, C.POINTER(C.c_int), C.POINTER(C.c_int), C.POINTER(C.c_int)]),
    "oalsfx_group_batch": (C.c_void_p, [C.c_void_p, C.c_int]),
    "oalsfx_group_set_effect": (C.c_int, [C.c_void_p, C.c_int, C.c_int, C.c_int, C.c_void_p, C.c_int]),
    "oalsfx_group_set_effect_type": (C.c_int, [C.c_void_p, C.c_int, C.c_int, C.c_int, C.c_int]),
    "oalsfx_group_set_effect_props": (C.c_int, [C.c_void_p, C.c_int, C.c_int, C.c_int, C.c_void_p, C.c_int]),
    "oalsfx_group_set_send_props": (C.c_int, [C.c_void_p, C.c_int, C.c_int, C.c_int, C.POINTER(desc.SendProps)]),
    "oalsfx_group_apply_changes": (C.c_int, [C.c_void_p, C.c_int, C.c_int]),
    "oalsfx_group_mix": (C.c_int, [C.c_void_p, C.c_int, C.c_void_p, C.c_void_p]),
    "oalsfx_group_mix_device": (C.c_int, [C.c_void_p, C.c_int, C.POINTER(C.c_void_p), C.POINTER(C.c_void_p)]),
    "oalsfx_group_mix_device_multi": (C.c_int, [C.c_void_p, C.c_int, C.c_int, C.POINTER(C.c_void_p), C.POINTER(C.c_void_p)]),
    "oalsfx_group_set_routing": (C.c_int, [C.c_void_p, C.c_int, C.c_int, C.POINTER(C.c_int), _fp]),
    "oalsfx_group_mix_downmix": (C.c_int, [C.c_void_p, C.c_int, _fp, C.c_int, _fp]),
    "oalsfx_group_mix_downmix_meter": (C.c_int, [C.c_void_p, C.c_int, _fp, C.c_int, _fp, C.c_float, C.c_int, C.c_void_p]),
    "oalsfx_group_synchronize": (C.c_int, [C.c_void_p]),
    "oalsfx_trim_pools": (C.c_ulonglong, []),
    "oalsfx_pools_waiting_bytes": (C.c_ulonglong, []),
    "oalsfx_debug_chain_same_cu": (C.c_longlong, [C.c_void_p]),
    "oalsfx_debug_chain_started": (C.c_int, [C.c_void_p, C.POINTER(C.c_uint), C.POINTER(C.c_uint)]),
    "oalsfx_batch_multi_counts": (C.c_int, [C.c_void_p, C.POINTER(C.c_longlong), C.POINTER(C.c_longlong)]),
    "oalsfx_debug_downmix_uploads": (C.c_longlong, [C.c_void_p]),
    "oalsfx_debug_downmix_vector": (None, [C.c_int]),
    "oalsfx_debug_sampler_uploads": (C.c_longlong, [C.c_void_p]),
    "oalsfx_debug_gate_skew": (None, [C.c_void_p, C.c_uint]),
    "oalsfx_debug_chain_given_up": (C.c_int, [C.c_void_p]),
    "oalsfx_debug_host_pipeline": (C.c_int, [C.c_void_p, C.POINTER(C.c_int), C.POINTER(C.c_double), C.POINTER(C.c_double)]),
    "oalsfx_device_pci_bus_id": (C.c_int, [C.c_int, C.c_char_p, C.c_int]),
    "oalsfx_debug_set_flags": (None, [C.c_int]),
    "oalsfx_debug_ring_address": (C.c_ulonglong, [C.c_void_p, C.c_int, C.c_int]),
    "oalsfx_debug_move_rings": (C.c_int, [C.c_void_p, C.c_int]),
    "oalsfx_debug_probe_rings": (C.c_int, [C.c_void_p, C.c_int, C.POINTER(C.c_double)]),
    "oalsfx_debug_probe_pointer": (C.c_int, [C.c_void_p, C.c_int, C.c_int, C.c_int, C.POINTER(C.c_double)]),
    "oalsfx_debug_hbm_sweep": (C.c_int, [C.c_int, C.c_ulonglong, C.c_int, C.c_int]),
    "oalsfx_debug_stream_pattern": (C.c_int, [C.c_int, C.c_int, C.c_int, C.c_int, C.c_int, C.c_int, C.POINTER(C.c_double)]),
    "oalsfx_host_effect_defaults": (None, [C.c_int, C.POINTER(desc.Effect)]),
    "oalsfx_host_effect_normalize": (None, [C.POINTER(desc.Effect)]),
    "oalsfx_host_derive_slot": (C.c_int, [C.c_int, C.c_int, C.POINTER(desc.Effect), C.POINTER(desc.SlotParams)]),
    "oalsfx_host_derive_source": (C.c_int, [C.c_int, C.c_int, C.c_int, C.POINTER(desc.SendProps), C.POINTER(desc.SendProps),
                                            C.POINTER(C.c_int), C.POINTER(desc.SourceParams)]),
    "oalsfx_host_ring_floats": (C.c_int, [C.c_int, C.c_int]),
    "oalsfx_host_channel_count": (C.c_int, [C.c_int]),
    "oalsfx_host_preset_count": (C.c_int, []),
    "oalsfx_host_preset_name": (C.c_char_p, [C.c_int]),
    "oalsfx_host_preset": (C.c_int, [C.c_int, C.c_void_p]),
}


def load(path=None):
    global _lib
    if _lib is not None and path is None:
        return _lib
    path = path or os.environ.get("OALSFX_LIB") or LIB_PATH
    if not os.path.exists(path):
        raise FileNotFoundError(
            f"{path} is missing: build it with `python -c 'import __graft_entry__ as g; g.build()'` "
            "(hipcc --offload-arch=gfx950).  There is no CPU fallback for the process path.")
    lib = C.CDLL(path)
    for name, (restype, argtypes) in SIGNATURES.items():
        try:
            fn = getattr(lib, name)
        except AttributeError:
            if name.startswith("oalsfx_host_") or os.environ.get("OALSFX_LIB") is None:
                raise
            continue
        fn.restype = restype
        fn.argtypes = argtypes
    _lib = lib
    return lib


def effect_defaults(effect_type):
    e = desc.Effect()
    load().oalsfx_host_effect_defaults(effect_type, C.byref(e))
    return e


def effect_normalized(effect):
    e = desc.Effect.from_buffer_copy(bytes(effect))
    load().oalsfx_host_effect_normalize(C.byref(e))
    return e


def derive_slot(channel_format, rate, normalized_effect):
    p = desc.SlotParams()
    if not load().oalsfx_host_derive_slot(channel_format, rate, C.byref(normalized_effect), C.byref(p)):
        raise ValueError("bad channel format")
    return p


def derive_source(channel_format, rate, direct, aux, slot_types):
    n = len(slot_types)
    aux_arr = (desc.SendProps * n)(*aux)
    types = (C.c_int * n)(*slot_types)
    out = desc.SourceParams()
    if not load().oalsfx_host_derive_source(channel_format, rate, n, C.byref(direct), aux_arr, types, C.byref(out)):
        raise ValueError("bad arguments")
    return out


def preset(index):
    p = desc.ReverbProps()
    if not load().oalsfx_host_preset(index, C.byref(p)):
        raise IndexError(index)
    return load().oalsfx_host_preset_name(index).decode(), p


def preset_count():
    return load().oalsfx_host_preset_count()
```

Measured before the change: 25490.

## Coalesce back-to-back device mix calls into one multi-buffer pass while GPU is backlogged

Consecutive single-buffer device mix calls can now be held on the host instead of launched at once. While the chained run is still backlogged (an event recorded two launches back has not completed), later calls with compatible, non-overlapping buffers are queued and then launched together as one multi-buffer pass. The aim is to cut per-call launch and chain-setup overhead for small 256-frame buffers. Every other API entry point now flushes held calls first, and the overlap check is extended to allow a shared output buffer. The cost is extra host bookkeeping, event queries per call and more complex error and flush handling.

```diff
diff --git a/include/oalsfx_hip.h b/include/oalsfx_hip.h
--- a/include/oalsfx_hip.h
+++ b/include/oalsfx_hip.h
@@ -38,6 +38,7 @@
 int oalsfx_batch_mix(oalsfx_batch* b, int frames, const float* src_host, float* dst_host);
 int oalsfx_batch_mix_gather(oalsfx_batch* b, int frames, const float* const* src_per_instance, float* const* dst_per_instance);
 int oalsfx_batch_mix_device(oalsfx_batch* b, int frames, const float* src_dev, float* dst_dev, void* hip_stream);
+int oalsfx_batch_set_coalescing(oalsfx_batch* b, int enable);
 int oalsfx_batch_mix_device_multi(oalsfx_batch* b, int frames, int buffers, const float* const* src_dev, float* const* dst_dev, void* hip_stream);
 int oalsfx_batch_synchronize(oalsfx_batch* b);
 long long oalsfx_batch_chained_calls(const oalsfx_batch* b);
diff --git a/include/oalsfx_hip_debug.h b/include/oalsfx_hip_debug.h
--- a/include/oalsfx_hip_debug.h
+++ b/include/oalsfx_hip_debug.h
@@ -32,6 +32,10 @@
 int oalsfx_debug_chain_started(oalsfx_batch* b, unsigned* host_total, unsigned* device_total);
 int oalsfx_batch_multi_counts(const oalsfx_batch* b, long long* buffers_in_passes, long long* passes);
 
+int oalsfx_host_buffers_apart(unsigned long long bytes, int buffers, const unsigned long long* srcs, const unsigned long long* dsts, int shared_out_ok);
+int oalsfx_host_joins_held(unsigned long long bytes, int held, const unsigned long long* srcs, const unsigned long long* dsts, unsigned long long src,
+                           unsigned long long dst);
+
 long long oalsfx_debug_downmix_uploads(const oalsfx_batch* b);
 void oalsfx_debug_downmix_vector(int max_floats);
 
diff --git a/oalsfxpp_amd/api.py b/oalsfxpp_amd/api.py
--- a/oalsfxpp_amd/api.py
+++ b/oalsfxpp_amd/api.py
@@ -154,6 +154,9 @@
         s = (C.c_void_p * max(1, len(src_ptrs)))(*src_ptrs)
         d = (C.c_void_p * max(1, len(dst_ptrs)))(*dst_ptrs)
         self._check(self._lib.oalsfx_batch_mix_device_multi(self._h, frames, len(src_ptrs), s, d, C.c_void_p(stream or 0)))
+
+    def set_coalescing(self, enable):
+        self._check(self._lib.oalsfx_batch_set_coalescing(self._h, 1 if enable else 0))
 
     def multi_counts(self):
         k, p = C.c_longlong(0), C.c_longlong(0)
diff --git a/oalsfxpp_amd/csrc/hip/batch.cpp b/oalsfxpp_amd/csrc/hip/batch.cpp
--- a/oalsfxpp_amd/csrc/hip/batch.cpp
+++ b/oalsfxpp_amd/csrc/hip/batch.cpp
@@ -181,6 +181,12 @@
     bool stream_handed_out = false;
     long long chained_calls = 0;
     long long multi_buffers = 0, multi_passes = 0;
+    bool coalesce = true;
+    int held_frames = 0;
+    std::vector<const float*> held_srcs;
+    std::vector<float*> held_dsts;
+    hipEvent_t ev_launched[2] = {};
+    int launched_no[2] = {0, 0};
     std::vector<int> route_bus;
     std::vector<float> route_gain;
     bool routing_dirty = true;
@@ -294,9 +300,12 @@
     kDbgNoCuMajor = 0x100,
     kDbgNoChain = 0x400,
     kDbgGateSecondOnly = 0x800,
+    kDbgNoCoalesce = 0x1000,
+    kDbgMultiSharedDst = 0x2000,
     kDbgChainAlways = 0x8000,
     kDbgForceProven = 0x2000000,
     kDbgHandOverBits = kDbgAcquireAlways | kDbgAcquireNever | kDbgReadEarly,
+    kDbgLaunchPerCall = kDbgNoCoalesce | kDbgChainAlways | kDbgGateSecondOnly | kDbgHandOverBits,
     kDbgKernelBits = 0xFF,
 };
 int debug_flags();
@@ -1331,6 +1340,7 @@
     if (!b->chain_open) {
         if (!b->hip_ok(hipEventRecord(b->ev_chain_start, b->stream), "hipEventRecord")) return false;
         b->chain_len = 1;
+        b->launched_no[0] = b->launched_no[1] = 0;
     } else {
         ++b->chain_len;
         if (first_on_its_stream && !b->hip_ok(hipStreamWaitEvent(stream, b->ev_chain_start, 0), "hipStreamWaitEvent")) return false;
@@ -1369,10 +1379,9 @@
     return true;
 }
 
-bool buffers_apart(const oalsfx_batch* b, int frames, int buffers, const float* const* srcs, float* const* dsts)
+bool ranges_apart(uintptr_t bytes, int buffers, const float* const* srcs, float* const* dsts, bool shared_out_ok)
 {
     if (buffers < 2) return true;
-    const uintptr_t bytes = static_cast<uintptr_t>(b->n) * frames * b->channels * sizeof(float);
     struct Range { uintptr_t lo; int call; bool out; };
     std::vector<Range> r;
     r.reserve(2 * static_cast<size_t>(buffers));
@@ -1381,28 +1390,58 @@
         r.push_back({reinterpret_cast<uintptr_t>(dsts[k]), k, true});
     }
     std::sort(r.begin(), r.end(), [](const Range& x, const Range& y) { return x.lo < y.lo || (x.lo == y.lo && x.call < y.call); });
-    const Range* last[2][2] = {};
+    struct Seen { uintptr_t lo; int call; bool set; };
+    Seen last[2][2] = {};
     for (const Range& x : r) {
         for (int kind = 0; kind < 2; ++kind) {
             if (!x.out && kind == 0) continue;
-            for (const Range* y : last[kind])
-                if (y && y->call != x.call && y->lo + bytes > x.lo) return false;
+            for (const Seen& y : last[kind]) {
+                if (!y.set || y.call == x.call || y.lo + bytes <= x.lo) continue;
+                if (shared_out_ok && x.out && kind == 1 && y.lo == x.lo) continue;
+                return false;
+            }
         }
         const int kind = x.out ? 1 : 0;
+        if (shared_out_ok && x.out && last[1][0].set && last[1][0].lo == x.lo) {
+            if (last[1][0].call != x.call) last[1][0].call = -1;
+            continue;
+        }
         last[kind][1] = last[kind][0];
-        last[kind][0] = &x;
+        last[kind][0] = Seen{x.lo, x.call, true};
     }
     return true;
 }
 
+bool buffers_apart(const oalsfx_batch* b, int frames, int buffers, const float* const* srcs, float* const* dsts, bool shared_out_ok)
+{
+    return ranges_apart(static_cast<uintptr_t>(b->n) * frames * b->channels * sizeof(float), buffers, srcs, dsts, shared_out_ok);
+}
+
+bool may_hold_behind(oalsfx_batch* b, int frames)
+{
+    if (!b->coalesce || (debug_flags() & (kDbgLaunchPerCall | kDbgNoChain | kDbgGeneralOnly))) return false;
+    return pass_usable(b, frames, 2 * frames);
+}
+
+bool run_backlogged(oalsfx_batch* b)
+{
+    if (!b->chain_open || b->chain_len < 2) return false;
+    const int two_back = b->chain_len - 1;
+    if (b->launched_no[two_back & 1] != two_back) return false;
+    if (hipEventQuery(b->ev_launched[two_back & 1]) != hipErrorNotReady) return false;
+    (void)hipGetLastError();
+    return true;
+}
+
 bool mix_pass(oalsfx_batch* b, int frames, int buffers, const float* const* srcs, float* const* dsts, hipStream_t stream, bool may_chain,
-              PendingUpload& upload, bool pass)
+              PendingUpload& upload, bool pass, bool held = false)
 {
     const float* const src = srcs[0];
     float* const dst = dsts[0];
     const int total = frames * buffers;
     if (pass && total > OALSFX_MAX_CHUNK) return b->fail("Internal error: a multi-buffer pass longer than one chunk.");
     const bool chained = may_chain && (!upload.st || upload.chainable) && chain_eligible(b, total, buffers, srcs, dsts, stream, upload.st != nullptr);
+    if (held && !chained) b->chained_calls -= buffers;
     if (!chained && !chain_join(b)) return false;
     int depth = 2;
     if (chained) {
@@ -1453,7 +1492,7 @@
         }
         if (!chain_next_launch(b, ctx, depth, &upload, &stream)) return false;
         if (!launch_params(b, upload, stream, nullptr, b->d_turn, ctx.turn_wait)) return false;
-        b->chained_calls += 1;
+        if (!held) b->chained_calls += 1;
     }
     ctx.slots = b->slots;
     ctx.channels = b->channels;
@@ -1571,6 +1610,11 @@
         done += n;
     }
     if (chained && !chain_launch_done(b)) return false;
+    if (chained && may_hold_behind(b, frames)) {
+        const int at = b->chain_len & 1;
+        if (!b->hip_ok(hipEventRecord(b->ev_launched[at], stream), "hipEventRecord")) return false;
+        b->launched_no[at] = b->chain_len;
+    }
     if (pass) { b->multi_buffers += buffers; b->multi_passes += 1; }
     if ((total % OALSFX_MAX_CHUNK) & 63) {
         for (size_t idx : b->settling)
@@ -1593,14 +1637,14 @@
 }
 
 bool mix_device(oalsfx_batch* b, int frames, int buffers, const float* const* srcs, float* const* dsts, hipStream_t stream, bool may_chain,
-                bool multi)
+                bool multi, bool held = false)
 {
     if (b->state_io_unordered && stream != b->stream) {
         if (!b->hip_ok(hipStreamWaitEvent(stream, b->ev_state_io, 0), "hipStreamWaitEvent")) return false;
         b->state_io_unordered = false;
     }
     const int per_pass = std::max(1, OALSFX_MAX_CHUNK / std::max(frames, 1));
-    const bool apart = multi && buffers_apart(b, frames, buffers, srcs, dsts);
+    const bool apart = multi && buffers_apart(b, frames, buffers, srcs, dsts, held || (debug_flags() & kDbgMultiSharedDst) != 0);
     for (int k = 0; k < buffers;) {
         if (b->poisoned) return b->fail(b->fault_text);
         poll_exact(b);
@@ -1612,7 +1656,7 @@
         const int take = std::min(buffers - k, per_pass);
         const bool pass = apart && !(debug_flags() & kDbgGeneralOnly) && pass_usable(b, frames, take * frames);
         const int step = pass ? take : 1;
-        if (!mix_pass(b, frames, step, srcs + k, dsts + k, stream, may_chain, upload, pass)) return false;
+        if (!mix_pass(b, frames, step, srcs + k, dsts + k, stream, may_chain, upload, pass, held)) return false;
         k += step;
     }
     return true;
@@ -1624,11 +1668,105 @@
     return mix_device(b, frames, 1, &src, &out, stream, may_chain, false);
 }
 
+
+bool flush_held(oalsfx_batch* b)
+{
+    if (b->held_srcs.empty()) return true;
+    std::vector<const float*> srcs;
+    std::vector<float*> dsts;
+    srcs.swap(b->held_srcs);
+    dsts.swap(b->held_dsts);
+    const int held = static_cast<int>(srcs.size());
+    bool ok = b->hip_ok(hipSetDevice(b->device), "hipSetDevice");
+    if (ok) ok = mix_device(b, b->held_frames, held, srcs.data(), dsts.data(), b->stream, true, held > 1, true);
+    else b->chained_calls -= held;
+    srcs.clear();
+    dsts.clear();
+    srcs.swap(b->held_srcs);
+    dsts.swap(b->held_dsts);
+    if (!ok && !b->poisoned) {
+        char text[sizeof(b->fault_text)];
+        std::snprintf(text, sizeof(text), "Held calls could not be launched: %s", b->error);
+        std::memcpy(b->fault_text, text, sizeof(text));
+        b->poisoned = true;
+        return b->fail(b->fault_text);
+    }
+    return ok;
+}
+
+bool entered(oalsfx_batch* b) { return !b || b->held_srcs.empty() || flush_held(b); }
+
+bool holdable(oalsfx_batch* b, int frames, int held, const float* src, float* dst)
+{
+    if (!may_hold_behind(b, frames) || !pass_usable(b, frames, (held + 1) * frames)) return false;
+    poll_exact(b);
+    if (!b->dirty_list.empty() || b->lists_dirty || b->rings_table_dirty) return false;
+    return chain_eligible(b, frames, 1, &src, &dst, b->stream, false);
+}
+
+bool range_joins(uintptr_t bytes, int held, const float* const* held_srcs, float* const* held_dsts, const float* src, const float* dst)
+{
+    const auto overlap = [bytes](const void* x, const void* y) {
+        const uintptr_t a = reinterpret_cast<uintptr_t>(x), c = reinterpret_cast<uintptr_t>(y);
+        return a < c + bytes && c < a + bytes;
+    };
+    for (int k = 0; k < held; ++k) {
+        if (overlap(dst, held_dsts[k]) && dst != held_dsts[k]) return false;
+        if (overlap(dst, held_srcs[k]) || overlap(src, held_dsts[k])) return false;
+    }
+    return true;
+}
+
+bool joins_held(const oalsfx_batch* b, int frames, const float* src, const float* dst)
+{
+    return range_joins(static_cast<uintptr_t>(b->n) * frames * b->channels * sizeof(float), static_cast<int>(b->held_srcs.size()),
+                       b->held_srcs.data(), b->held_dsts.data(), src, dst);
+}
+
+bool hold_or_launch(oalsfx_batch* b, int frames, const float* src, float* dst)
+{
+    if (b->poisoned) return b->fail(b->fault_text);
+    int held = static_cast<int>(b->held_srcs.size());
+    bool joins = holdable(b, frames, held, src, dst);
+    if (held > 0 && !(joins && frames == b->held_frames && joins_held(b, frames, src, dst))) {
+        if (!flush_held(b)) return false;
+        held = 0;
+        joins = holdable(b, frames, 0, src, dst);
+    }
+    if (!joins) return mix_device(b, frames, src, dst, b->stream, true);
+    b->held_frames = frames;
+    b->held_srcs.push_back(src);
+    b->held_dsts.push_back(dst);
+    b->chained_calls += 1;
+    ++held;
+    const bool full = !pass_usable(b, frames, (held + 1) * frames);
+    if (full || !run_backlogged(b)) return flush_held(b);
+    return true;
+}
+
 }
 
 extern "C" {
 
 const char* oalsfx_last_error(void) { return g_last_error.c_str(); }
+
+int oalsfx_host_buffers_apart(unsigned long long bytes, int buffers, const unsigned long long* srcs, const unsigned long long* dsts, int shared_out_ok)
+{
+    std::vector<const float*> s(buffers);
+    std::vector<float*> d(buffers);
+    for (int k = 0; k < buffers; ++k) { s[k] = reinterpret_cast<const float*>(static_cast<uintptr_t>(srcs[k])); d[k] = reinterpret_cast<float*>(static_cast<uintptr_t>(dsts[k])); }
+    return ranges_apart(static_cast<uintptr_t>(bytes), buffers, s.data(), d.data(), shared_out_ok != 0) ? 1 : 0;
+}
+
+int oalsfx_host_joins_held(unsigned long long bytes, int held, const unsigned long long* srcs, const unsigned long long* dsts, unsigned long long src,
+                           unsigned long long dst)
+{
+    std::vector<const float*> s(held);
+    std::vector<float*> d(held);
+    for (int k = 0; k < held; ++k) { s[k] = reinterpret_cast<const float*>(static_cast<uintptr_t>(srcs[k])); d[k] = reinterpret_cast<float*>(static_cast<uintptr_t>(dsts[k])); }
+    return range_joins(static_cast<uintptr_t>(bytes), held, s.data(), d.data(), reinterpret_cast<const float*>(static_cast<uintptr_t>(src)),
+                       reinterpret_cast<const float*>(static_cast<uintptr_t>(dst))) ? 1 : 0;
+}
 
 oalsfx_batch* oalsfx_batch_create(int n_instances, int channel_format, int sampling_rate, int effect_count, int device_id)
 {
@@ -1699,6 +1837,7 @@
         b->uncached = (!kind || std::strcmp(kind, "uncached") == 0) && uncached_memory_available(b->device);
     }
     ok = ok && b->hip_ok(hipEventCreateWithFlags(&b->ev_chain_start, hipEventDisableTiming), "hipEventCreate");
+    for (auto& e : b->ev_launched) ok = ok && b->hip_ok(hipEventCreateWithFlags(&e, hipEventDisableTiming), "hipEventCreate");
     for (int k = 0; k < kSideStreams; ++k) {
         ok = ok && b->hip_ok(hipStreamCreateWithFlags(&b->side_stream[k], hipStreamNonBlocking), "hipStreamCreate");
         ok = ok && b->hip_ok(hipEventCreateWithFlags(&b->ev_join[k], hipEventDisableTiming), "hipEventCreate");
@@ -1756,6 +1895,7 @@
 {
     if (!b) return;
     hipSetDevice(b->device);
+    (void)entered(b);
     for (int k = 1; k < kChainDepth; ++k)
         if (b->chain_stream[k]) hipStreamSynchronize(b->chain_stream[k]);
     if (b->stream) hipStreamSynchronize(b->stream);
@@ -1780,6 +1920,8 @@
     for (int k = 1; k < kChainDepth; ++k)
         if (b->ev_chain[k]) hipEventDestroy(b->ev_chain[k]);
     if (b->ev_chain_start) hipEventDestroy(b->ev_chain_start);
+    for (hipEvent_t e : b->ev_launched)
+        if (e) hipEventDestroy(e);
     for (int k = 1; k < kChainDepth; ++k)
         if (b->chain_stream[k]) hipStreamDestroy(b->chain_stream[k]);
     if (b->h2d_stream) hipStreamSynchronize(b->h2d_stream);
@@ -1835,6 +1977,7 @@
 
 int oalsfx_batch_set_effect(oalsfx_batch* b, int first, int count, int slot, const oalsfx_effect* effects, int stride_bytes)
 {
+    if (!entered(b)) return 0;
     if (!range_ok(b, first, count)) return 0;
     if (slot < 0 || slot >= b->slots) return b->fail(kErrSlot) ? 1 : 0;
     const auto* base = reinterpret_cast<const unsigned char*>(effects);
@@ -1846,6 +1989,7 @@
 
 int oalsfx_batch_set_effect_at(oalsfx_batch* b, const int* instances, int count, int slot, const oalsfx_effect* effects, int stride_bytes)
 {
+    if (!entered(b)) return 0;
     if (count < 0 || (count > 0 && (!instances || !effects))) return b->fail(kErrRange) ? 1 : 0;
     if (slot < 0 || slot >= b->slots) return b->fail(kErrSlot) ? 1 : 0;
     for (int k = 0; k < count; ++k)
@@ -1860,6 +2004,7 @@
 
 int oalsfx_batch_set_effect_type(oalsfx_batch* b, int first, int count, int slot, int effect_type)
 {
+    if (!entered(b)) return 0;
     if (!range_ok(b, first, count)) return 0;
     if (slot < 0 || slot >= b->slots) return b->fail(kErrSlot) ? 1 : 0;
     for (int i = 0; i < count; ++i) b->inst[first + i].deferred[slot].set_type_and_defaults(static_cast<oalsfxpp::EffectType>(effect_type));
@@ -1869,6 +2014,7 @@
 
 int oalsfx_batch_set_effect_props(oalsfx_batch* b, int first, int count, int slot, const void* props, int stride_bytes)
 {
+    if (!entered(b)) return 0;
     if (!range_ok(b, first, count)) return 0;
     if (slot < 0 || slot >= b->slots) return b->fail(kErrSlot) ? 1 : 0;
     const auto* base = static_cast<const unsigned char*>(props);
@@ -1880,6 +2026,7 @@
 
 int oalsfx_batch_set_send_props(oalsfx_batch* b, int first, int count, int slot, const oalsfx_send_props* props)
 {
+    if (!entered(b)) return 0;
     if (!range_ok(b, first, count)) return 0;
     if (slot >= b->slots) return b->fail(kErrSlot) ? 1 : 0;
     oalsfxpp::SendProps p;
@@ -1912,6 +2059,7 @@
 
 int oalsfx_batch_apply_changes(oalsfx_batch* b, int first, int count)
 {
+    if (!entered(b)) return 0;
     if (!range_ok(b, first, count)) return 0;
     size_t kept = 0;
     for (size_t k = 0; k < b->touched_list.size(); ++k) {
@@ -1938,11 +2086,22 @@
     if (!src_dev) return b->fail(kErrNoSrc) ? 1 : 0;
     if (!dst_dev) return b->fail(kErrNoDst) ? 1 : 0;
     if (!b->hip_ok(hipSetDevice(b->device), "hipSetDevice")) return 0;
-    return mix_device(b, frames, src_dev, dst_dev, hip_stream ? static_cast<hipStream_t>(hip_stream) : b->stream, hip_stream == nullptr) ? 1 : 0;
+    if (!hip_stream) return hold_or_launch(b, frames, src_dev, dst_dev) ? 1 : 0;
+    if (!entered(b)) return 0;
+    return mix_device(b, frames, src_dev, dst_dev, static_cast<hipStream_t>(hip_stream), false) ? 1 : 0;
+}
+
+int oalsfx_batch_set_coalescing(oalsfx_batch* b, int enable)
+{
+    if (!b) { g_last_error = "Null batch."; return 0; }
+    if (!entered(b)) return 0;
+    b->coalesce = enable != 0;
+    return 1;
 }
 
 int oalsfx_batch_mix_device_multi(oalsfx_batch* b, int frames, int buffers, const float* const* src_dev, float* const* dst_dev, void* hip_stream)
 {
+    if (!entered(b)) return 0;
     if (!b) { g_last_error = "Null batch."; return 0; }
     if (frames < 0) return b->fail("Frame count is negative.") ? 1 : 0;
     if (buffers < 0) return b->fail("Buffer count is negative.") ? 1 : 0;
@@ -1973,6 +2132,7 @@
 
 int mix_host(oalsfx_batch* b, int frames, const float* src_host, float* dst_host, double* legs_us)
 {
+    if (!entered(b)) return 0;
     if (legs_us) legs_us[0] = legs_us[1] = legs_us[2] = 0.0;
     if (frames == 0) return 1;
     if (frames < 0) return b->fail("Frame count is negative.") ? 1 : 0;
@@ -2071,6 +2231,7 @@
 
 int oalsfx_batch_mix_async(oalsfx_batch* b, int frames, const float* src_host, float* dst_host)
 {
+    if (!entered(b)) return 0;
     if (frames == 0) return 1;
     if (frames < 0) return b->fail("Frame count is negative.") ? 1 : 0;
     if (!src_host) return b->fail(kErrNoSrc) ? 1 : 0;
@@ -2122,6 +2283,7 @@
 
 int oalsfx_batch_wait(oalsfx_batch* b)
 {
+    if (!entered(b)) return 0;
     if (!b->hip_ok(hipSetDevice(b->device), "hipSetDevice") || !chain_join(b)) return 0;
     if (b->d2h_stream && !b->hip_ok(hipStreamSynchronize(b->d2h_stream), "hipStreamSynchronize")) return 0;
     if (!b->hip_ok(hipStreamSynchronize(b->stream), "hipStreamSynchronize")) return 0;
@@ -2143,6 +2305,7 @@
 
 int oalsfx_batch_synchronize(oalsfx_batch* b)
 {
+    if (!entered(b)) return 0;
     if (!b->hip_ok(hipSetDevice(b->device), "hipSetDevice") || !chain_join(b)) return 0;
     if (!b->hip_ok(hipStreamSynchronize(b->stream), "hipStreamSynchronize")) return 0;
     if (std::getenv("OALSFX_HOST_PROFILE")) {
@@ -2156,6 +2319,7 @@
 
 void* oalsfx_batch_stream(oalsfx_batch* b)
 {
+    (void)entered(b);
     b->stream_handed_out = true;
     if (hipSetDevice(b->device) == hipSuccess) (void)chain_join(b);
     return b->stream;
@@ -2163,6 +2327,7 @@
 
 int oalsfx_batch_read_slot(oalsfx_batch* b, int instance, int slot, oalsfx_slot_params* params, oalsfx_slot_state* state)
 {
+    if (!entered(b)) return 0;
     if (instance < 0 || instance >= b->n || slot < 0 || slot >= b->slots) return b->fail(kErrRange) ? 1 : 0;
     if (!b->hip_ok(hipSetDevice(b->device), "hipSetDevice") || !chain_join(b)) return 0;
     if (!sync_params(b, nullptr)) return 0;
@@ -2177,6 +2342,7 @@
 
 int oalsfx_batch_read_ring(oalsfx_batch* b, int instance, int slot, float* out, int max_floats)
 {
+    if (!entered(b)) return 0;
     if (instance < 0 || instance >= b->n || slot < 0 || slot >= b->slots) return 0;
     if (hipSetDevice(b->device) != hipSuccess || !chain_join(b) || !sync_params(b, nullptr)) return 0;
     const size_t idx = static_cast<size_t>(instance) * b->slots + slot;
@@ -2191,6 +2357,7 @@
 
 int oalsfx_batch_read_source(oalsfx_batch* b, int instance, oalsfx_source_params* params, oalsfx_source_state* state)
 {
+    if (!entered(b)) return 0;
     if (instance < 0 || instance >= b->n) return b->fail(kErrRange) ? 1 : 0;
     if (!b->hip_ok(hipSetDevice(b->device), "hipSetDevice") || !chain_join(b)) return 0;
     if (!sync_params(b, nullptr)) return 0;
@@ -2452,6 +2619,7 @@
 
 unsigned long long oalsfx_batch_snapshot_bytes(oalsfx_batch* b, const int* instances, int count)
 {
+    if (!entered(b)) return 0;
     if (!b) { g_last_error = "Null batch."; return 0; }
     if (!instances_ok(b, instances, count)) return 0;
     std::vector<BlobEntry> entries;
@@ -2461,6 +2629,7 @@
 
 int oalsfx_batch_snapshot(oalsfx_batch* b, const int* instances, int count, void* dst, unsigned long long bytes)
 {
+    if (!entered(b)) return 0;
     if (!b) { g_last_error = "Null batch."; return 0; }
     if (!instances_ok(b, instances, count)) return 0;
     if (!dst) return b->fail("No snapshot buffer.") ? 1 : 0;
@@ -2513,6 +2682,7 @@
 
 int oalsfx_batch_restore(oalsfx_batch* b, const int* instances, int count, const void* src, unsigned long long bytes)
 {
+    if (!entered(b)) return 0;
     if (!b) { g_last_error = "Null batch."; return 0; }
     if (!instances_ok(b, instances, count)) return 0;
     if (!src) return b->fail("No snapshot buffer.") ? 1 : 0;
@@ -2573,6 +2743,7 @@
 
 int oalsfx_batch_reset(oalsfx_batch* b, const int* instances, int count)
 {
+    if (!entered(b)) return 0;
     if (!b) { g_last_error = "Null batch."; return 0; }
     if (!instances_ok(b, instances, count)) return 0;
     if (b->poisoned) return b->fail(b->fault_text) ? 1 : 0;
@@ -2697,6 +2868,7 @@
 
 int oalsfx_batch_set_routing(oalsfx_batch* b, int first, int count, const int* bus, const float* gain)
 {
+    if (!entered(b)) return 0;
     if (!b) { g_last_error = "Null batch."; return 0; }
     if (!range_ok(b, first, count)) return 0;
     if (bus)
@@ -2721,6 +2893,7 @@
 
 int oalsfx_batch_downmix_device(oalsfx_batch* b, int frames, const float* src_dev, int n_buses, float* dst_bus_dev, void* hip_stream)
 {
+    if (!entered(b)) return 0;
     if (!b) { g_last_error = "Null batch."; return 0; }
     if (!downmix_args_ok(b, frames, n_buses)) return 0;
     if (frames == 0) return 1;
@@ -2739,6 +2912,7 @@
 
 int oalsfx_batch_mix_downmix(oalsfx_batch* b, int frames, const float* src_host, int n_buses, float* dst_bus_host)
 {
+    if (!entered(b)) return 0;
     if (!b) { g_last_error = "Null batch."; return 0; }
     if (!downmix_args_ok(b, frames, n_buses)) return 0;
     if (frames == 0) return 1;
@@ -2782,6 +2956,7 @@
 int oalsfx_batch_meter_device(oalsfx_batch* b, int rows, int frames, const float* src_dev, float threshold, int flags, oalsfx_meter* meters_dev,
                               void* hip_stream)
 {
+    if (!entered(b)) return 0;
     if (!b) { g_last_error = "Null batch."; return 0; }
     if (rows < 1) return b->fail("Row count is out of range.") ? 1 : 0;
     if (!meter_args_ok(b, frames, threshold, flags)) return 0;
@@ -2808,6 +2983,7 @@
 int downmix_meter_call(oalsfx_batch* b, int frames, const float* src_host, bool play, int n_buses, float* dst_bus_host, float threshold, int flags,
                        oalsfx_meter* voice_meters_host, oalsfx_meter* bus_meters_host)
 {
+    if (!entered(b)) return 0;
     if (!meter_args_ok(b, frames, threshold, flags)) return 0;
     if (!play && !voice_meters_host && !bus_meters_host) return oalsfx_batch_mix_downmix(b, frames, src_host, n_buses, dst_bus_host);
     if (!downmix_args_ok(b, frames, n_buses)) return 0;
@@ -2976,6 +3152,7 @@
 
 int oalsfx_batch_set_samplers(oalsfx_batch* b, const int* instances, int count, const oalsfx_sampler* samplers)
 {
+    if (!entered(b)) return 0;
     if (!b) { g_last_error = "Null batch."; return 0; }
     if (!instances_ok(b, instances, count)) return 0;
     if (b->poisoned) return b->fail(b->fault_text) ? 1 : 0;
@@ -3005,6 +3182,7 @@
 
 int oalsfx_batch_get_samplers(oalsfx_batch* b, const int* instances, int count, oalsfx_sampler* out)
 {
+    if (!entered(b)) return 0;
     if (!b) { g_last_error = "Null batch."; return 0; }
     if (!instances_ok(b, instances, count)) return 0;
     if (count == 0) return 1;
@@ -3025,6 +3203,7 @@
 
 int oalsfx_batch_sample_device(oalsfx_batch* b, int frames, float* dst_dev, void* hip_stream)
 {
+    if (!entered(b)) return 0;
     if (!b) { g_last_error = "Null batch."; return 0; }
     if (!sampler_args_ok(b, frames)) return 0;
     if (frames == 0) return 1;
@@ -3045,6 +3224,7 @@
 
 int oalsfx_batch_fill_synthetic(oalsfx_batch* b, int frames, unsigned buffer_index, float* dst_dev, void* hip_stream)
 {
+    if (!entered(b)) return 0;
     if (!b->hip_ok(hipSetDevice(b->device), "hipSetDevice") || !chain_join(b)) return 0;
     oalsfx_hip::launch_fill_synthetic(dst_dev, b->n, frames * b->channels, buffer_index, hip_stream ? static_cast<hipStream_t>(hip_stream) : b->stream);
     return b->hip_ok(hipGetLastError(), "fill_synthetic") ? 1 : 0;
@@ -3052,6 +3232,7 @@
 
 int oalsfx_batch_kernel_timing(oalsfx_batch* b, int enable)
 {
+    if (!entered(b)) return 0;
     if (!b->hip_ok(hipSetDevice(b->device), "hipSetDevice") || !chain_join(b)) return 0;
     for (auto& t : b->timed) { b->event_pool.push_back(t.start); b->event_pool.push_back(t.stop); }
     b->timed.clear();
@@ -3068,6 +3249,7 @@
 
 int oalsfx_batch_kernel_timing_read(oalsfx_batch* b, int effect_type, int* launches, double* total_ms)
 {
+    if (!entered(b)) return 0;
     if (!b->hip_ok(hipSetDevice(b->device), "hipSetDevice") || !chain_join(b)) return 0;
     int n = 0;
     double ms = 0.0;
@@ -3090,6 +3272,7 @@
 
 int oalsfx_batch_kernel_timing_samples(oalsfx_batch* b, int effect_type, double* out_us, int max_samples)
 {
+    if (!entered(b)) return 0;
     if (!b->hip_ok(hipSetDevice(b->device), "hipSetDevice") || !chain_join(b)) return -1;
     int key = (effect_type >= 0 && effect_type < OALSFX_REVERB) ? kTimedWaveEffects : effect_type;
     if (key == OALSFX_REVERB) key = OALSFX_EAX_REVERB;
@@ -3111,6 +3294,7 @@
 
 int oalsfx_batch_plan(oalsfx_batch* b, int slot, int counts[4])
 {
+    if (!entered(b)) return 0;
     if (slot < 0 || slot >= b->slots) return b->fail(kErrSlot) ? 1 : 0;
     if (!b->hip_ok(hipSetDevice(b->device), "hipSetDevice") || !chain_join(b)) return 0;
     poll_exact(b);
@@ -3138,6 +3322,7 @@
 
 long long oalsfx_debug_chain_same_cu(oalsfx_batch* b)
 {
+    if (!entered(b)) return -1;
     unsigned v = 0;
     if (hipSetDevice(b->device) != hipSuccess || !chain_join(b) || hipStreamSynchronize(b->stream) != hipSuccess) return -1;
     if (hipMemcpy(&v, b->d_turn + static_cast<size_t>(b->n) * b->slots + 1, sizeof(v), hipMemcpyDeviceToHost) != hipSuccess) return -1;
@@ -3146,6 +3331,7 @@
 
 int oalsfx_debug_host_pipeline(oalsfx_batch* b, int* form, double* probe_us_three_streams, double* probe_us_one_stream)
 {
+    if (!entered(b)) return 0;
     if (form) *form = b->pipe_mode;
     if (probe_us_three_streams) *probe_us_three_streams = b->pipe_probe_us[0];
     if (probe_us_one_stream) *probe_us_one_stream = b->pipe_probe_us[1];
@@ -3159,11 +3345,12 @@
 
 unsigned long long oalsfx_pools_waiting_bytes(void) { return uncached_pool().bytes_waiting(); }
 
-void oalsfx_debug_gate_skew(oalsfx_batch* b, unsigned skew) { if (b) b->gate_skew = skew; }
+void oalsfx_debug_gate_skew(oalsfx_batch* b, unsigned skew) { if (b && entered(b)) b->gate_skew = skew; }
 int oalsfx_debug_chain_given_up(const oalsfx_batch* b) { return b && b->chain_given_up ? 1 : 0; }
 
 int oalsfx_debug_chain_started(oalsfx_batch* b, unsigned* host_total, unsigned* device_total)
 {
+    if (!entered(b)) return 0;
     unsigned v = 0;
     if (!b->hip_ok(hipSetDevice(b->device), "hipSetDevice") || !chain_join(b) || !b->hip_ok(hipStreamSynchronize(b->stream), "hipStreamSynchronize")) return 0;
     if (b->d_turn && !b->hip_ok(hipMemcpy(&v, b->d_turn + static_cast<size_t>(b->n) * b->slots, sizeof(v), hipMemcpyDeviceToHost), "hipMemcpy")) return 0;
@@ -3180,6 +3367,7 @@
 
 int oalsfx_batch_event_overhead(oalsfx_batch* b, int repeats, double* avg_us)
 {
+    if (!entered(b)) return 0;
     if (repeats <= 0 || !b->hip_ok(hipSetDevice(b->device), "hipSetDevice") || !chain_join(b)) return 0;
     hipEvent_t e0 = b->take_event(), e1 = b->take_event();
     double total = 0.0;
@@ -3228,6 +3416,7 @@
 
 int oalsfx_debug_probe_rings(oalsfx_batch* b, int repeats, double* avg_us)
 {
+    if (!entered(b)) return 0;
     if (hipSetDevice(b->device) != hipSuccess || !chain_join(b) || !sync_params(b, nullptr) || b->ring_chunks.empty() || repeats <= 0) return 0;
     if (!b->hip_ok(hipStreamSynchronize(b->stream), "hipStreamSynchronize")) return 0;
     const auto& rc = b->ring_chunks.front();
@@ -3249,6 +3438,7 @@
 
 int oalsfx_debug_move_rings(oalsfx_batch* b, int keep_old)
 {
+    if (!entered(b)) return 0;
     if (hipSetDevice(b->device) != hipSuccess || !chain_join(b) || !sync_params(b, nullptr)) return 0;
     if (!b->hip_ok(hipStreamSynchronize(b->stream), "hipStreamSynchronize")) return 0;
     const size_t total = static_cast<size_t>(b->n) * b->slots;
@@ -3279,6 +3469,7 @@
 
 unsigned long long oalsfx_debug_ring_address(oalsfx_batch* b, int instance, int slot)
 {
+    if (!entered(b)) return 0;
     if (instance < 0 || instance >= b->n || slot < 0 || slot >= b->slots) return 0;
     if (hipSetDevice(b->device) != hipSuccess || !chain_join(b) || !sync_params(b, nullptr)) return 0;
     return reinterpret_cast<unsigned long long>(b->h_rings[static_cast<size_t>(instance) * b->slots + slot]);
diff --git a/oalsfxpp_amd/csrc/host/group.cpp b/oalsfxpp_amd/csrc/host/group.cpp
--- a/oalsfxpp_amd/csrc/host/group.cpp
+++ b/oalsfxpp_amd/csrc/host/group.cpp
@@ -111,6 +111,7 @@
             delete g;
             return nullptr;
         }
+        oalsfx_batch_set_coalescing(b, 0);
         g->device.push_back(device_ids[k]);
         g->first.push_back(f);
         g->count.push_back(c);
diff --git a/oalsfxpp_amd/lib.py b/oalsfxpp_amd/lib.py
--- a/oalsfxpp_amd/lib.py
+++ b/oalsfxpp_amd/lib.py
@@ -88,6 +88,7 @@
     "oalsfx_pools_waiting_bytes": (C.c_ulonglong, []),
     "oalsfx_debug_chain_same_cu": (C.c_longlong, [C.c_void_p]),
     "oalsfx_debug_chain_started": (C.c_int, [C.c_void_p, C.POINTER(C.c_uint), C.POINTER(C.c_uint)]),
+    "oalsfx_batch_set_coalescing": (C.c_int, [C.c_void_p, C.c_int]),
     "oalsfx_batch_multi_counts": (C.c_int, [C.c_void_p, C.POINTER(C.c_longlong), C.POINTER(C.c_longlong)]),
     "oalsfx_debug_downmix_uploads": (C.c_longlong, [C.c_void_p]),
     "oalsfx_debug_downmix_vector": (None, [C.c_int]),
@@ -109,6 +110,8 @@
     "oalsfx_host_derive_source": (C.c_int, [C.c_int, C.c_int, C.c_int, C.POINTER(desc.SendProps), C.POINTER(desc.SendProps),
                                             C.POINTER(C.c_int), C.POINTER(desc.SourceParams)]),
     "oalsfx_host_ring_floats": (C.c_int, [C.c_int, C.c_int]),
+    "oalsfx_host_buffers_apart": (C.c_int, [C.c_ulonglong, C.c_int, C.POINTER(C.c_ulonglong), C.POINTER(C.c_ulonglong), C.c_int]),
+    "oalsfx_host_joins_held": (C.c_int, [C.c_ulonglong, C.c_int, C.POINTER(C.c_ulonglong), C.POINTER(C.c_ulonglong), C.c_ulonglong, C.c_ulonglong]),
     "oalsfx_host_channel_count": (C.c_int, [C.c_int]),
     "oalsfx_host_preset_count": (C.c_int, []),
     "oalsfx_host_preset_name": (C.c_char_p, [C.c_int]),
```

Result: faster. 28700, median of 6 (+12.6%).
